# reuk/wayverb

Measured on AMD Instinct MI355X. Metric: Gnode-updates/s, fp64 box mesh, higher is better.
Workload: dtype f64

## Files before the change

include/wayverb_amd.h:

```cpp
#ifndef WAYVERB_AMD_H
#define WAYVERB_AMD_H

#include <stddef.h>
#include <stdint.h>

#ifdef __cplusplus
extern "C" {
#endif

enum {
    WV_OK = 0,
    WV_E_INVALID_ARGUMENT = -1,
    WV_E_INVALID_MESH = -2,
    WV_E_HIP = -3,
    WV_E_NO_DEVICE = -4,
    WV_E_COMM = -5,
    WV_E_STATE = -6
};


enum {
    WV_ID_NONE = 0,
    WV_ID_INSIDE = 1 << 0,
    WV_ID_NX = 1 << 1,
    WV_ID_PX = 1 << 2,
    WV_ID_NY = 1 << 3,
    WV_ID_PY = 1 << 4,
    WV_ID_NZ = 1 << 5,
    WV_ID_PZ = 1 << 6,
    WV_ID_REENTRANT = 1 << 7
};

enum {
    WV_FLAG_SUCCESS = 0,
    WV_FLAG_INF = 1 << 0,
    WV_FLAG_NAN = 1 << 1,
    WV_FLAG_OUTSIDE_RANGE = 1 << 2,
    WV_FLAG_OUTSIDE_MESH = 1 << 3,
    WV_FLAG_SUSPICIOUS_BOUNDARY = 1 << 4
};

typedef struct wv_condensed_node {
    int32_t boundary_type;
    uint32_t boundary_index;
} wv_condensed_node;

typedef struct wv_coefficients_canonical {
    double b[7];
    double a[7];
} wv_coefficients_canonical;

typedef struct wv_boundary_data {
    double filter_memory[6];
    uint32_t coefficient_index;
    uint32_t reserved_;
} wv_boundary_data;

typedef struct wv_mesh {
    int32_t nx, ny, nz;
    const wv_condensed_node* nodes;
    const wv_coefficients_canonical* coefficients;
    uint32_t num_coefficients;
    const uint32_t* boundary_indices_1;
    const uint32_t* boundary_indices_2;
    const uint32_t* boundary_indices_3;
    uint64_t num_boundary_1, num_boundary_2, num_boundary_3;
} wv_mesh;

enum { WV_PRECISION_F32 = 0,
       WV_PRECISION_F64 = 1   };

typedef struct wv_tuning {
    int32_t pair;
    int32_t pair_chunks;
    int32_t pair_inner_fix;
    int32_t pair_wide;
    int32_t pair_unit_waves;
    int32_t pair_unit_planes;
    int32_t pair_units_by_chunk;
    int32_t tile_lists;
    int32_t fuse_pre_post;
    int32_t graph;
    int32_t boundary_lds;
    int32_t boundary_order;
    int32_t boundary_xwall;
    int32_t stream_ry, stream_nwx, stream_nwy, stream_zchunks;
    int32_t slab_early;
    int32_t pair_split_rows;
    int32_t fuse_planes;
    int32_t whole_step;
    int32_t triple;
    int32_t triple_chunks;
    int32_t triple_lanes;
} wv_tuning;

typedef struct wv_options {
    int32_t struct_size;
    int32_t precision;
    int32_t device;
    int32_t ghost_lo, ghost_hi;
    int32_t flag_interval;
    int32_t stream_variant;
    int32_t all_tiles;
    int32_t nodes_on_device;
    int32_t comm_timeout_s;
    int32_t transport;
    int32_t reserved_[5];
    wv_tuning tuning;
} wv_options;

enum { WV_TRANSPORT_RCCL = 0, WV_TRANSPORT_IPC = 1 };

typedef struct wv_engine wv_engine;


int wv_create(const wv_mesh* mesh, const wv_options* options, wv_engine** out);
void wv_destroy(wv_engine* e);
const char* wv_last_error(void);
void wv_default_options(wv_options* options);

enum { WV_BUF_CURRENT = 0, WV_BUF_PREVIOUS = 1 };

int wv_read_value(wv_engine* e, int buffer, uint64_t index, double* value);
int wv_write_value(wv_engine* e, int buffer, uint64_t index, double value);
int wv_read_field(wv_engine* e, int buffer, void* dst, int elem_size);
int wv_write_field(wv_engine* e, int buffer, const void* src, int elem_size);
int wv_read_planes(wv_engine* e, int buffer, int32_t z_begin, int32_t z_count, void* dst, int elem_size);
int wv_write_planes(wv_engine* e, int buffer, int32_t z_begin, int32_t z_count, const void* src, int elem_size);
int wv_read_boundary_data(wv_engine* e, int dimensionality, wv_boundary_data* dst);
int wv_write_boundary_data(wv_engine* e, int dimensionality, const wv_boundary_data* src);
int wv_set_coefficients(wv_engine* e, const wv_coefficients_canonical* c, uint32_t n);
int wv_host_register(void* p, uint64_t bytes);
int wv_host_unregister(void* p);
int wv_device_buffer(wv_engine* e, int buffer, void** device_ptr);

int wv_checkpoint(wv_engine* e);
int wv_rollback(wv_engine* e);
int wv_drop_checkpoint(wv_engine* e);


int wv_step(wv_engine* e, int32_t* flag);
int wv_swap(wv_engine* e);

enum { WV_SOURCE_NONE = 0,
       WV_SOURCE_HARD = 1,
       WV_SOURCE_SOFT = 2   };

int wv_set_source(wv_engine* e, int kind, uint64_t node, const double* signal, uint64_t n);
int wv_set_receivers(wv_engine* e, const uint64_t* nodes, uint32_t n);
int wv_run(wv_engine* e, uint64_t n_steps, uint64_t* steps_done, int32_t* flag);
int wv_fetch_receivers(wv_engine* e, uint64_t first, uint64_t n, double* dst);
int wv_step_count(wv_engine* e, uint64_t* steps);

int wv_kernel_time_ms(wv_engine* e, double* mean_ms, uint64_t* launches);
int wv_enable_kernel_timing(wv_engine* e, int enable);
int wv_kernel_time_detail(wv_engine* e, double* mean_ms, uint64_t* launches, uint64_t* steps);
enum { WV_QUERY_PASSES = 0, WV_QUERY_XWALL_ENTRIES = 1, WV_QUERY_FIELDS = 2, WV_QUERY_MARCH_LIVE_PERMILLE = 3,
       WV_QUERY_SWEEP_LIVE_PERMILLE = 4, WV_QUERY_MARCH_ROUNDS = 5, WV_QUERY_HALO_WAIT_NS = 6, WV_QUERY_HALO_WAITS = 7,
       WV_QUERY_HALO_EXCHANGES = 8, WV_QUERY_HALO_BYTES_SENT = 9, WV_QUERY_EARLY_PASSES = 10,
       WV_QUERY_BOUNDARY1_NS = 11, WV_QUERY_BOUNDARY2_NS = 12, WV_QUERY_BOUNDARY_TIMED = 13,
       WV_QUERY_WHOLE_STEPS = 14 ,
       WV_QUERY_TRIPLE_PASSES = 15,
       WV_QUERY_TRIPLE_MARCH_NS = 16, WV_QUERY_TRIPLE_MARCH_TIMED = 17, WV_QUERY_BOUNDARY3_NS = 18, WV_QUERY_FIXUP3_NS = 19,
       WV_QUERY_TRIPLE_PARTS_TIMED = 20 };
int wv_query(wv_engine* e, int what, uint64_t* value);
int wv_synchronize(wv_engine* e);
int wv_set_stream_tuning(wv_engine* e, int variant, int rows_per_wave, int waves_x, int waves_y, int knob);

#define WV_UNIQUE_ID_BYTES 128
int wv_comm_use_library(const char* path);
int wv_comm_unique_id(void* id_bytes );
int wv_comm_init(wv_engine* e, const void* id_bytes, int rank, int nranks);
int wv_comm_destroy(wv_engine* e);
int wv_comm_init_local(wv_engine* const* engines, int32_t n);
int wv_run_group(wv_engine* const* engines, int32_t n, uint64_t n_steps, uint64_t* steps_done, int32_t* flag);

int wv_measure_triad(int32_t device, uint64_t n_doubles, int32_t iters, double* gb_per_s);

int wv_compressed_waveguide_run(int32_t device, uint64_t steps, int32_t source_kind, const float* input,
                                uint64_t n_input, float* output );
int wv_make_transparent(const float* input, uint64_t n, const float* response, uint32_t taps,
                        float* out );

int wv_filter_test_2(const float* input, float* output, double* memory,
                     const wv_coefficients_canonical* coeffs, uint32_t n_filters, uint32_t n_samples);
int wv_field_pitch(wv_engine* e, uint64_t* pitch_elements);

int wv_make_box_nodes(int32_t nx, int32_t ny, int32_t nz_global, int32_t z_begin, int32_t z_count,
                      int32_t number_from, int32_t number_to, wv_condensed_node* nodes,
                      uint64_t counts[3]);

int wv_classify_nodes(int32_t nx, int32_t ny, int32_t nz, const uint8_t* inside, wv_condensed_node* nodes,
                      uint64_t counts[3]);

int wv_voxelise(const float* vertices, uint32_t n_vertices, const uint32_t* triangles, uint32_t n_triangles,
                const float aabb_min[3], const float aabb_max[3], uint32_t side, uint32_t* out, uint64_t capacity,
                uint64_t* needed);
int wv_nodes_inside(int32_t nx, int32_t ny, int32_t nz, const float min_corner[3], float spacing,
                    const uint32_t* voxel_index, uint64_t n_voxel_words, const float aabb_min[3],
                    const float aabb_max[3], uint32_t side, const uint32_t* triangles, uint32_t n_triangles,
                    const float* vertices, uint32_t n_vertices, uint8_t* inside);

int wv_boundary_index_data(int32_t nx, int32_t ny, int32_t nz, const float min_corner[3], float spacing,
                           wv_condensed_node* nodes, const uint32_t* triangles, uint32_t n_triangles,
                           const float* vertices, uint32_t n_vertices, uint32_t* b1, uint64_t capacity_1,
                           uint32_t* b2, uint64_t capacity_2, uint32_t* b3, uint64_t capacity_3,
                           uint64_t counts[3]);

typedef struct wv_scene_mesh wv_scene_mesh;
int wv_scene_mesh_create(int32_t nx, int32_t ny, int32_t nz, const float min_corner[3], float spacing,
                         const uint32_t* voxel_index, uint64_t n_voxel_words, const float aabb_min[3],
                         const float aabb_max[3], uint32_t side, const uint32_t* triangles, uint32_t n_triangles,
                         const float* vertices, uint32_t n_vertices, int32_t device, wv_scene_mesh** out,
                         uint64_t counts[3]);
int wv_scene_mesh_fetch(const wv_scene_mesh* sm, wv_condensed_node* nodes, uint32_t* b1, uint32_t* b2, uint32_t* b3);
int wv_scene_mesh_create_engine(const wv_scene_mesh* sm, const wv_coefficients_canonical* coefficients,
                                uint32_t num_coefficients, const wv_options* options, wv_engine** out);
void wv_scene_mesh_destroy(wv_scene_mesh* sm);

int wv_arbitrary_magnitude_filter(const double* frequency, const double* amplitude, uint32_t n_points,
                                  double b[7], double a[7]);
int wv_is_stable(const double* a, uint32_t n, int32_t* stable);
int wv_band_centres(double sample_rate, double centres[8]);
int wv_reflectance_filter(const double absorption[8], double sample_rate, wv_coefficients_canonical* out);
int wv_impedance_coefficients(const wv_coefficients_canonical* reflectance, wv_coefficients_canonical* impedance);

typedef struct wv_directional_output {
    float intensity[3];
    float pressure;
} wv_directional_output;
typedef struct wv_waveguide_band {
    const wv_directional_output* directional;
    uint64_t n;
    double sample_rate;
    double valid_hz_min, valid_hz_max;
} wv_waveguide_band;
enum { WV_ATTENUATOR_NULL = 0,
       WV_ATTENUATOR_MICROPHONE = 1
        };
enum { WV_FILTER_LOPASS = 0, WV_FILTER_HIPASS = 1, WV_FILTER_BANDPASS = 2 };

int wv_attenuate(int32_t method, const float pointing[3], float shape, float acoustic_impedance,
                 const wv_directional_output* in, uint64_t n, float* out);
int wv_adjust_sampling_rate(const float* in, uint64_t n, double in_sample_rate, double out_sample_rate, float* out,
                            uint64_t capacity, uint64_t* n_out);
int wv_frequency_domain_filter(float* signal, uint64_t n, int32_t kind, double edge_lo, double edge_hi,
                               double width_factor, uint32_t steepness);
int wv_postprocess_waveguide(const wv_waveguide_band* bands, uint32_t n_bands, int32_t method, const float pointing[3],
                             float shape, float acoustic_impedance, double output_sample_rate, float* out,
                             uint64_t capacity, uint64_t* n_out);

typedef struct wv_hrtf_table {
    const double* energy;
    uint32_t az_num, el_num;
} wv_hrtf_table;
int wv_hrtf_attenuation(const wv_hrtf_table* table, const float pointing[3], const float up[3], int32_t channel,
                        const float incident[3], float bands[8]);
int wv_hrtf_ear_position(const float pointing[3], const float up[3], int32_t channel, float radius,
                         const float base_position[3], float ear[3]);
int wv_attenuate_hrtf(const wv_hrtf_table* table, const float pointing[3], const float up[3], int32_t channel,
                      float acoustic_impedance, const wv_directional_output* in, uint64_t n, float* out);
int wv_multiband_filter_and_mixdown(float* bands, uint64_t n, double sample_rate, float* out);
int wv_postprocess_waveguide_hrtf(const wv_waveguide_band* bands, uint32_t n_bands, const wv_hrtf_table* table,
                                  const float pointing[3], const float up[3], int32_t channel, float acoustic_impedance,
                                  double output_sample_rate, float* out, uint64_t capacity, uint64_t* n_out);

#ifdef __cplusplus
}
#endif
#endif
```

wayverb_amd/csrc/boundary_kernels.hip.h:

```cpp
#pragma once
#include "device_common.hip.h"

namespace wv {

__device__ __forceinline__ void filter_step_6(double in, double m[6], const double* __restrict__ cb,
                                              const double* __restrict__ ca) {
    const double out = (in * cb[0] + m[0]) / ca[0];
#pragma unroll
    for (int i = 0; i < 5; ++i) {
        const double b = cb[i + 1] == 0 ? 0 : cb[i + 1] * in;
        const double a = ca[i + 1] == 0 ? 0 : ca[i + 1] * out;
        m[i] = b - a + m[i + 1];
    }
    const double b = cb[6] == 0 ? 0 : cb[6] * in;
    const double a = ca[6] == 0 ? 0 : ca[6] * out;
    m[5] = b - a;
}

__global__ void __launch_bounds__(64) filter_test_2_kernel(const float* input, float* output, double* memory,
                                                           const double* coeffs, uint32_t n_filters,
                                                           uint32_t n_samples) {
    const uint32_t f = blockIdx.x * blockDim.x + threadIdx.x;
    if (f >= n_filters) return;
    double m[6], cb[7], ca[7];
// ... 287 lines not shown
    if (LEVEL == 2) {
        g2c = a.next[gn];
        h2c = a.next[gn + (h_off ? 0 : step)];
    }
    Real nb[3][2];
    bool off[3][2];
    off[0][0] = x - 1 < 0;
    off[0][1] = x + 1 >= a.nx;
    nb[0][0] = nb[0][1] = f_nb[pos_e];
    bool any_field = false;
#pragma unroll
    for (int k = 0; k < 4; ++k) {
        const int ax = 1 + (k >> 1), s = k & 1;
        const int c = pos[ax] + (s ? 1 : -1);
        off[ax][s] = c < 0 || c >= lim[ax];
        const bool mirrored = ref[k] != XW_FIELD;
        nb[ax][s] = own_nb[mirrored ? (ref[k] & ~XW_SAME_FACING) : pos_e];
        any_field = any_field || !mirrored;
    }
    const Real prev = own_prev[pos_e];
    double m[1][6];
    const double* cf[1];
    cf[0] = coeffs + (size_t)a.cidx[pos_e] * 14;
#pragma unroll
    for (int j = 0; j < 6; ++j) m[0][j] = __builtin_nontemporal_load(a.fmem + (size_t)j * a.n_slots + pos_e);
    Real f1 = 0, far1 = 0;
    Real fnb[3][2], fprev = 0;
    bool any_lateral_field = false;
    if (LEVEL == 1) {
        f1 = a.next[fn];
        far1 = a.next[fn + (far_off ? 0 : step)];
        far1 = far_off ? Real(0) : far1;
    } else {
        const Real own_at = own_nb[pos_e];
        Real far = LEVEL == 2 ? a.xw_g[pos_e] : *(gok ? a.xw_g2 + pos_e : a.cur + gn);
        far = (LEVEL == 3 && far_off) ? Real(0) : far;
        fnb[0][0] = step > 0 ? own_at : far;
        fnb[0][1] = step > 0 ? far : own_at;
#pragma unroll
        for (int k = 0; k < 4; ++k) {
            const int ax = 1 + (k >> 1), s = k & 1;
            const bool regular = ref[k] != XW_FIELD && (ref[k] & XW_SAME_FACING);
            const Real v = f_nb[regular ? (ref[k] & ~XW_SAME_FACING) : pos_e];
            fnb[ax][s] = off[ax][s] ? Real(0) : v;
            any_lateral_field = any_lateral_field || (!regular && !off[ax][s]);
        }
        fprev = LEVEL == 2 ? a.xw_f[pos_e] : a.xw_f1[pos_e];
    }
    Real gnb[3][2], gprev = 0;
    uint32_t g_from_field = 0;
    if (LEVEL == 3) {
        const Real f2 = nb[0][0], h2 = a.xw_h2[pos_e];
        gnb[0][0] = step > 0 ? f2 : h2;
        gnb[0][1] = step > 0 ? h2 : f2;
#pragma unroll
        for (int k = 0; k < 4; ++k) {
            const int ax = 1 + (k >> 1), s = k & 1;
            const bool regular = ref[k] != XW_FIELD && (ref[k] & XW_SAME_FACING);
            const uint32_t other = regular ? (ref[k] & ~XW_SAME_FACING) : pos_e;
            const bool copy = regular && a.xw_gok[other] != 0;
            const Real v = a.xw_g2[other];
            gnb[ax][s] = off[ax][s] ? Real(0) : v;
            if (!copy && !off[ax][s]) g_from_field |= 1u << k;
        }
        gprev = a.xw_g[pos_e];
        if (gok && g_from_field) {
#pragma unroll
            for (int k = 0; k < 4; ++k) {
                const int ax = 1 + (k >> 1), s = k & 1;
                if ((g_from_field >> k) & 1u) gnb[ax][s] = a.cur[gn + (s ? stride[ax] : -stride[ax])];
            }
        }
    }
    if (any_field) {
#pragma unroll
        for (int k = 0; k < 4; ++k) {
            const int ax = 1 + (k >> 1), s = k & 1;
            if (ref[k] == XW_FIELD) nb[ax][s] = a.cur[(int64_t)idx + (off[ax][s] ? 0 : (s ? stride[ax] : -stride[ax]))];
        }
    }
    if (LEVEL != 1 && any_lateral_field) {
#pragma unroll
        for (int k = 0; k < 4; ++k) {
            const int ax = 1 + (k >> 1), s = k & 1;
            const bool regular = ref[k] != XW_FIELD && (ref[k] & XW_SAME_FACING);
            if (!regular && !off[ax][s]) fnb[ax][s] = a.cur[fn + (s ? stride[ax] : -stride[ax])];
        }
    }

    const Real next = boundary_value<Real, 1>(a.courant, a.courant_sq, dirs, nb, off, prev, m, cf);
#pragma unroll
    for (int j = 0; j < 6; ++j) __builtin_nontemporal_store(m[0][j], a.fmem + (size_t)j * a.n_slots + pos_e);
    bad |= bad_bits(next);
    a.next[idx] = next;
    own_out[pos_e] = next;
    if (LEVEL == 1) {
        a.xw_f1[pos_e] = f1;
        a.xw_g[pos_e] = far1;
    } else {
        const Real sf = faced_value<Real>(fnb, fprev);
        bad |= bad_bits(sf);
        a.next[fn] = sf;
        (LEVEL == 2 ? a.xw_f2 : a.xw_f)[pos_e] = sf;
        if (LEVEL == 2) {
            a.xw_g2[pos_e] = g2c;
            a.xw_h2[pos_e] = h_off ? Real(0) : h2c;
        } else {
            const Real sg = faced_value<Real>(gnb, gprev);
            if (gok) {
                bad |= bad_bits(sg);
                a.next[gn] = sg;
            }
        }
    }
}

template <typename Real, bool FIX>
__device__ __forceinline__ void boundary_entry(const BoundaryArgs<Real>& a, const double* coeffs, uint32_t e, int& bad) {
    if (e < a.n1) {
        boundary_node<Real, 1, FIX>(a, coeffs, e, e, 0u, a.n1, bad);
    } else if (e < a.n1 + a.n2) {
        boundary_node<Real, 2, FIX>(a, coeffs, e - a.n1, e, a.n1, a.n2, bad);
    } else if (e < a.n1 + a.n2 + a.n3) {
        boundary_node<Real, 3, FIX>(a, coeffs, e - a.n1 - a.n2, e, a.n1 + 2u * a.n2, a.n3, bad);
    }
}

constexpr uint32_t kMaxLdsCoefficientSets = 256;

template <typename Real>
__device__ __forceinline__ void pre_post_body(const PrePostArgs<Real>& a, uint32_t t, uint32_t width);

template <typename Real, bool LDSC, bool FIX, int XW3 = 0>
__device__ __forceinline__ void boundary_body(const BoundaryArgs<Real>& a, const PrePostArgs<Real>& next, uint32_t block, uint32_t blocks) {
    __shared__ double s_coeffs[LDSC ? kMaxLdsCoefficientSets * 14 : 1];
    if (LDSC) {
        for (uint32_t w = threadIdx.x; w < a.n_coeffs * 14u; w += 256) s_coeffs[w] = a.coeffs[w];
        __syncthreads();
    }
    const double* coeffs = LDSC ? s_coeffs : a.coeffs;
    const uint32_t t = block * blockDim.x + threadIdx.x;
    int bad = 0;
    if (a.xw_n) {
        if (t < a.xw_pad) {
            if (t < a.xw_n) {
                if (XW3)
                    xwall3_node<Real, XW3 ? XW3 : 1>(a, coeffs, t, bad);
                else
                    xwall_node<Real, FIX ? 2 : 1>(a, coeffs, t, bad);
            }
        } else if (a.order) {
            if (t - a.xw_pad < a.n_order) boundary_entry<Real, FIX>(a, coeffs, a.order[t - a.xw_pad], bad);
        } else {
            boundary_entry<Real, FIX>(a, coeffs, a.xw_n + (t - a.xw_pad), bad);
        }
    } else if (a.order) {
        if (t < a.n_order) boundary_entry<Real, FIX>(a, coeffs, a.order[t], bad);
    } else {
        boundary_entry<Real, FIX>(a, coeffs, t, bad);
    }
    if (bad) atomicOr(a.flag, bad);
    if (next.fused && block == blocks - 1) pre_post_body<Real>(next, threadIdx.x, 256);
}

template <typename Real, bool LDSC, bool FIX = false, int XW3 = 0>
__global__ void __launch_bounds__(256) boundary_kernel(const BoundaryArgs<Real> a, const PrePostArgs<Real> next) {
    if (next.fused) {
        if (blockIdx.x == 0) {
            pre_post_body<Real>(next, threadIdx.x, 256);
            return;
        }
        PrePostArgs<Real> none{};
        boundary_body<Real, LDSC, FIX, XW3>(a, none, blockIdx.x - 1, gridDim.x - 1);
        return;
    }
    boundary_body<Real, LDSC, FIX, XW3>(a, next, blockIdx.x, gridDim.x);
}

struct XwCoverArgs {
    const uint32_t* bnode;
    const uint8_t* btype;
    uint32_t* covered;
    uint32_t xw_n;
    const uint8_t* pair_map;
    uint8_t* gok;
    int nx, ny, nz, pitch, cls_pitch;
};
__global__ void __launch_bounds__(256) xwall_cover_kernel(const XwCoverArgs a) {
    const uint32_t p = blockIdx.x * blockDim.x + threadIdx.x;
    if (p >= a.xw_n) return;
    const uint32_t idx = a.bnode[p];
    const int step = (a.btype[p] & 2u) ? 1 : -1;
    const uint32_t fn = idx + (uint32_t)step;
    atomicOr(a.covered + (fn >> 5), 1u << (fn & 31u));
    const int x = (int)(idx % (uint32_t)a.pitch);
    const uint32_t q = idx / (uint32_t)a.pitch;
    const int y = (int)(q % (uint32_t)a.ny), z = (int)(q / (uint32_t)a.ny);
    auto code_at = [&](int xx) -> uint32_t { return (a.pair_map[cls_byte_index(xx, y, z, a.ny, a.cls_pitch)] >> ((xx & 3) * 2)) & 3u; };
    const int xg = x + 2 * step, xh = x + 3 * step;
    bool ok = xg >= 0 && xg < a.nx && code_at(xg) == 1u;
    if (ok && xh >= 0 && xh < a.nx) ok = code_at(xh) != 2u && code_at(xh) != 3u;
    a.gok[p] = ok ? 1 : 0;
    if (ok) {
        const uint32_t gn = idx + (uint32_t)(2 * step);
        atomicOr(a.covered + (gn >> 5), 1u << (gn & 31u));
    }
}

struct XwEligibleArgs {
    const uint32_t* bnode;
    const uint8_t* btype;
    const uint8_t* cls;
    uint8_t* eligible;
    uint32_t n1;
    int nx, ny, nz, pitch, cls_pitch;
    int march_begin, march_end;
};

__global__ void __launch_bounds__(256) xwall_eligible_kernel(const XwEligibleArgs a) {
    const uint32_t e = blockIdx.x * blockDim.x + threadIdx.x;
    if (e >= a.n1) return;
    const uint32_t idx = a.bnode[e];
    const uint32_t dirs = a.btype[e] & 0x3Fu;
    bool ok = idx != INVALID_NODE && (dirs == 1u || dirs == 2u);
    if (ok) {
        const int x = (int)(idx % (uint32_t)a.pitch);
        const uint32_t q = idx / (uint32_t)a.pitch;
        const int y = (int)(q % (uint32_t)a.ny), z = (int)(q / (uint32_t)a.ny);
        const int step = dirs == 2u ? 1 : -1;
        auto cls_at = [&](int xx) -> uint32_t {
            return (a.cls[cls_byte_index(xx, y, z, a.ny, a.cls_pitch)] >> ((xx & 3) * 2)) & 3u;
        };
        ok = z >= a.march_begin && z < a.march_end && x + step >= 0 && x + step < a.nx && cls_at(x + step) == CLS_INSIDE;
        if (ok && x + 2 * step >= 0 && x + 2 * step < a.nx) ok = cls_at(x + 2 * step) != CLS_BOUNDARY;
    }
    a.eligible[e] = ok ? 1 : 0;
}

template <typename Real>
__global__ void __launch_bounds__(256) xwall_gather_kernel(const BoundaryArgs<Real> a) {
    const uint32_t p = blockIdx.x * blockDim.x + threadIdx.x;
    if (p >= a.xw_n) return;
    const uint32_t idx = a.bnode[p];
    const int64_t fn = (int64_t)idx + ((a.btype[p] & 2u) ? 1 : -1);
    a.xw_a[p] = a.prev[idx];
    a.xw_b[p] = a.cur[idx];
    a.xw_f[p] = a.cur[fn];
}

template <typename Real>
__device__ __forceinline__ void pre_post_body(const PrePostArgs<Real>& a, uint32_t t, uint32_t width) {
    if (t == 0 && a.flag) *a.flag = a.flag_init;
    if (t == 0 && a.flag2) *a.flag2 = a.flag_init;
    Real injected = 0;
    const bool has_source = a.source_kind != 0;
    if (has_source) {
        const Real s = (Real)a.signal[a.signal_pos + (a.signal_base ? *a.signal_base : 0ull)];
        injected = (a.source_kind == 1) ? s : (Real)(a.cur[a.source_node] + s);
    }
    for (uint32_t r = t; r < a.n_recv; r += width) {
        const uint64_t node = a.recv[r];
        Real v = 0;
        if (node != ~0ull) v = (has_source && node == a.source_node) ? injected : a.cur[node];
        a.recv_out[r] = v;
    }
    __syncthreads();
    if (t == 0 && has_source) a.cur[a.source_node] = injected;
    if (a.fix_n) {
        __threadfence();
        __syncthreads();
        const int64_t plane = (int64_t)a.pitch * a.ny;
        int bad = 0;
        for (uint32_t i = t; i < a.fix_n; i += width) {
            const uint32_t idx = a.fix_nodes[i];
            const int x = (int)(idx % (uint32_t)a.pitch);
            const uint32_t q = idx / (uint32_t)a.pitch;
            const int y = (int)(q % (uint32_t)a.ny);
            const int z = (int)(q / (uint32_t)a.ny);
            auto t1 = [&](int64_t at) { return __hip_atomic_load(a.cur + at, __ATOMIC_RELAXED, __HIP_MEMORY_SCOPE_AGENT); };
            Real s = 0;
            s += (x > 0) ? t1((int64_t)idx - 1) : Real(0);
            s += (x + 1 < a.nx) ? t1((int64_t)idx + 1) : Real(0);
            s += (y > 0) ? t1((int64_t)idx - a.pitch) : Real(0);
            s += (y + 1 < a.ny) ? t1((int64_t)idx + a.pitch) : Real(0);
            s += (z > 0) ? t1((int64_t)idx - plane) : Real(0);
            s += (z + 1 < a.nz) ? t1((int64_t)idx + plane) : Real(0);
            s = div3(s);
            s -= a.fix_cur[idx];
            bad |= bad_bits(s);
            a.fix_out2[idx] = s;
        }
        if (bad) atomicOr(a.fix_flag, bad);
    }
}

template <typename Real>
__global__ void __launch_bounds__(64) pre_post_kernel(const PrePostArgs<Real> a) {
    pre_post_body<Real>(a, threadIdx.x, 64);
}

struct NodeRec {
    int32_t boundary_type;
    uint32_t boundary_index;
};

struct SetupArgs {
    const NodeRec* nodes;
    int64_t first_row, rows;
    int nx, ny;
    int pitch;
    int cls_pitch;
    uint8_t* cls;
    uint32_t* bnode;
    uint8_t* btype;
    uint32_t n1, n2, n3;
    int* status;
    int z_begin, z_end;
};

__device__ __forceinline__ uint32_t classify(int32_t t, int* dim_out) {
    *dim_out = 0;
    if (t == 0) return CLS_NONE;
    const int bits = __popc((uint32_t)t);
    if (bits == 1 && (t & 1)) return CLS_INSIDE;
    if (bits == 1 && (t & 128)) return CLS_REENTRANT;
    *dim_out = bits;
    return CLS_BOUNDARY;
}

__global__ void __launch_bounds__(256) setup_classify_kernel(const SetupArgs a) {
    const int64_t n_bytes = a.rows * a.cls_pitch;
    for (int64_t i = (int64_t)blockIdx.x * blockDim.x + threadIdx.x; i < n_bytes;
         i += (int64_t)gridDim.x * blockDim.x) {
        const int64_t row = i / a.cls_pitch;
        const int xb = (int)(i % a.cls_pitch);
        const int64_t grow = a.first_row + row;
        const int z = (int)(grow / a.ny);
        uint32_t byte = 0;
        for (int j = 0; j < 4; ++j) {
            const int x = xb * 4 + j;
            if (x >= a.nx) break;
            const NodeRec rec = a.nodes[row * a.nx + x];
            const int32_t t = rec.boundary_type;
            int dim;
            const uint32_t c = classify(t, &dim);
            byte |= c << (2 * j);
            if (c == CLS_BOUNDARY) {
                const uint32_t dirs = ((uint32_t)t >> 1) & 0x3Fu;
                const bool only_dirs = ((uint32_t)t & ~0x7Eu) == 0;
                const bool axes_ok = ((dirs & 3u) != 3u) && (((dirs >> 2) & 3u) != 3u) && (((dirs >> 4) & 3u) != 3u);
                if (!only_dirs || !axes_ok || dim < 1 || dim > 3) {
                    atomicOr(a.status, 1);
                    continue;
                }
                if (z < a.z_begin || z >= a.z_end) continue;
                const uint32_t n_d = dim == 1 ? a.n1 : (dim == 2 ? a.n2 : a.n3);
                const uint32_t off = dim == 1 ? 0u : (dim == 2 ? a.n1 : a.n1 + a.n2);
                const uint32_t k = rec.boundary_index;
                if (k >= n_d) {
                    atomicOr(a.status, 2);
                    continue;
                }
                a.bnode[off + k] = (uint32_t)(grow * a.pitch + x);
                a.btype[off + k] = (uint8_t)dirs;
            }
        }
        a.cls[cls_byte_index(xb * 4, (int)(grow % a.ny), z, a.ny, a.cls_pitch)] = (uint8_t)byte;
    }
}

struct ValidateArgs {
    const uint32_t* bnode;
    const uint8_t* btype;
    const uint8_t* cls;
    uint32_t n_entries;
    int nx, ny, nz, pitch, cls_pitch;
    int* static_flag;
};

__global__ void __launch_bounds__(256) setup_validate_kernel(const ValidateArgs a) {
    const uint32_t e = blockIdx.x * blockDim.x + threadIdx.x;
    if (e >= a.n_entries) return;
    const uint32_t idx = a.bnode[e];
    if (idx == INVALID_NODE) return;
    const uint32_t dirs = a.btype[e] & 0x3Fu;
    const int pos[3] = {(int)(idx % (uint32_t)a.pitch), (int)((idx / (uint32_t)a.pitch) % (uint32_t)a.ny),
                        (int)(idx / ((uint32_t)a.pitch * (uint32_t)a.ny))};
    const int lim[3] = {a.nx, a.ny, a.nz};
    int flag = 0;
    int dim = __popc(dirs);
    for (int ax = 0; ax < 3; ++ax) {
        const bool has_n = (dirs >> (2 * ax)) & 1u, has_p = (dirs >> (2 * ax + 1)) & 1u;
        if (has_n || has_p) {
            const int c = pos[ax] + (has_p ? 1 : -1);
            if (c < 0 || c >= lim[ax]) flag |= FLAG_OUTSIDE_MESH;
        } else if (dim < 3) {
            for (int s = -1; s <= 1; s += 2) {
                int p[3] = {pos[0], pos[1], pos[2]};
                p[ax] += s;
                if (p[ax] < 0 || p[ax] >= lim[ax]) {
// ... 73 lines not shown
```

wayverb_amd/csrc/device_common.hip.h:

```cpp
#pragma once
#include <hip/hip_runtime.h>
#include <stdint.h>

namespace wv {

enum : uint32_t { CLS_NONE = 0, CLS_INSIDE = 1, CLS_BOUNDARY = 2, CLS_REENTRANT = 3 };

enum : int { FLAG_INF = 1, FLAG_NAN = 2, FLAG_OUTSIDE_RANGE = 4, FLAG_OUTSIDE_MESH = 8,
             FLAG_SUSPICIOUS = 16 };

constexpr uint32_t INVALID_NODE = 0xFFFFFFFFu;

__host__ __device__ inline int64_t cls_word_index(int x, int y, int z, int ny, int cls_pitch) {
    return ((int64_t)z * ((ny + 3) >> 2) + (y >> 2)) * cls_pitch + (x >> 2);
}
__host__ __device__ inline int64_t cls_byte_index(int x, int y, int z, int ny, int cls_pitch) {
    return cls_word_index(x, y, z, ny, cls_pitch) * 4 + (y & 3);
}

template <typename Real>
struct Vec16;
template <>
struct Vec16<double> {
    typedef double type __attribute__((ext_vector_type(2)));
    static constexpr int N = 2;
};
template <>
struct Vec16<float> {
    typedef float type __attribute__((ext_vector_type(4)));
    static constexpr int N = 4;
};

__device__ __forceinline__ float lane_from_below(float edge, float v) {
    return __int_as_float(__builtin_amdgcn_update_dpp(__float_as_int(edge), __float_as_int(v),
                                                      0x138 , 0xf, 0xf, false));
}
__device__ __forceinline__ float lane_from_above(float edge, float v) {
    return __int_as_float(__builtin_amdgcn_update_dpp(__float_as_int(edge), __float_as_int(v),
                                                      0x130 , 0xf, 0xf, false));
}
__device__ __forceinline__ double lane_from_below(double edge, double v) {
    const int lo = __builtin_amdgcn_update_dpp(__double2loint(edge), __double2loint(v), 0x138, 0xf, 0xf, false);
    const int hi = __builtin_amdgcn_update_dpp(__double2hiint(edge), __double2hiint(v), 0x138, 0xf, 0xf, false);
    return __hiloint2double(hi, lo);
}
__device__ __forceinline__ double lane_from_above(double edge, double v) {
    const int lo = __builtin_amdgcn_update_dpp(__double2loint(edge), __double2loint(v), 0x130, 0xf, 0xf, false);
    const int hi = __builtin_amdgcn_update_dpp(__double2hiint(edge), __double2hiint(v), 0x130, 0xf, 0xf, false);
    return __hiloint2double(hi, lo);
}

__device__ __forceinline__ float read_lane(float v, int src) {
    return __int_as_float(__builtin_amdgcn_readlane(__float_as_int(v), src));
}
__device__ __forceinline__ double read_lane(double v, int src) {
    const int lo = __builtin_amdgcn_readlane(__double2loint(v), src);
    const int hi = __builtin_amdgcn_readlane(__double2hiint(v), src);
    return __hiloint2double(hi, lo);
}

__device__ __forceinline__ double div3(double x) {
    constexpr double c = 0x1.5555555555555p-2;
    const double q0 = x * c;
    const double r = __builtin_fma(-3.0, q0, x);
    return __builtin_amdgcn_div_fixup(__builtin_fma(r, c, q0), 3.0, x);
}
__device__ __forceinline__ float div3(float x) {
    constexpr float c = 0x1.555556p-2f;
    const float q0 = x * c;
    const float r = __builtin_fmaf(-3.0f, q0, x);
    return __builtin_amdgcn_div_fixupf(__builtin_fmaf(r, c, q0), 3.0f, x);
}

__device__ __forceinline__ bool is_finite(float v) { return __builtin_amdgcn_classf(v, 0x1F8); }
__device__ __forceinline__ bool is_finite(double v) { return __builtin_amdgcn_class(v, 0x1F8); }

template <typename Real>
__device__ __forceinline__ int bad_bits(Real v) {
    return (isinf(v) ? FLAG_INF : 0) | (isnan(v) ? FLAG_NAN : 0);
}

template <typename Real>
struct BoundaryArgs {
    const Real* prev;
    Real* next;
    const Real* cur;
    int* flag;
    const uint32_t* bnode;
    const uint8_t* btype;
    double* fmem;
    const uint32_t* cidx;
    const double* coeffs;
    uint32_t n_coeffs;
    uint32_t n1, n2, n3;
    uint32_t n_slots;
    int nx, ny, nz;
    int pitch;
    int z_begin, z_end;
    Real courant, courant_sq;
    const uint32_t* order;
    uint32_t n_order;
    int fix_z0, fix_z1;
    uint32_t xw_n, xw_pad;
    const uint32_t* xw_nbr;
    Real *xw_a, *xw_b, *xw_f, *xw_f1, *xw_g;
    Real *xw_o2, *xw_f2;
    Real *xw_g2, *xw_h2;
    const uint8_t* xw_gok;
};

template <typename Real>
struct StreamArgs {
    const Real* prev;
    Real* next;
    const Real* cur;
    const uint8_t* cls;
    int* flag;
    int nx, ny, nz;
    int pitch;
    int cls_pitch;
    int z_begin, z_end;
    int z_skip_from, z_skip;
    int zc;
    int tiles_x, tiles_y, chunks_z;
    int total_tiles, tiles_per_xcd;
    int stripe_rows, tiles_y_stripe, passes;
    const uint64_t* tile_list;
    uint32_t list_start[9];
};

template <typename Real>
struct PrePostArgs {
    Real* cur;
    const double* signal;
    uint64_t signal_pos;
    const uint64_t* signal_base;
    uint64_t source_node;
    int source_kind;
    const uint64_t* recv;
    Real* recv_out;
    uint32_t n_recv;
    int* flag;
    int* flag2;
    int flag_init;
    int fused;
    const uint32_t* fix_nodes;
    uint32_t fix_n;
    const Real* fix_cur;
    Real* fix_out2;
    int* fix_flag;
    int nx, ny, nz, pitch;
};

struct StepDuty {
    uint64_t node;
    uint32_t block;
    uint32_t col;
    uint32_t kind;
    uint32_t pad_;
};
template <typename Real>
struct StepDuties {
    const StepDuty* list;
    uint32_t n;
    const double* signal;
    uint64_t signal_pos;
    const uint64_t* signal_base;
    Real* recv_out;
    const uint64_t* recv;
    uint32_t n_recv;
    int* next_flag;
    int flag_init;
};

}
```

wayverb_amd/csrc/engine.hip:

```cpp
#include "engine.hip.h"
#include "engine_setup.hip.h"
#include "engine_single.hip.h"
#include "engine_pair.hip.h"
#include "engine_triple.hip.h"
#include "engine_batch.hip.h"
#include "engine_io.hip.h"
#include "engine_slab.hip.h"

namespace {
thread_local std::string g_last_error;
thread_local hipError_t g_last_hip_error = hipSuccess;
}

namespace wv {
int fail_with(int code, const std::string& msg) {
    g_last_error = msg;
    return code;
}
void note_hip_error(hipError_t err) { g_last_hip_error = err; }
hipError_t last_hip_error() { return g_last_hip_error; }
}

using wv::DeviceGuard;
using wv::Engine;
using wv::fail;
using wv::ScopedDevice;

extern "C" {

const char* wv_last_error(void) { return g_last_error.c_str(); }

void wv_default_options(wv_options* o) {
    std::memset(o, 0, sizeof(*o));
    o->struct_size = (int32_t)sizeof(wv_options);
    o->precision = WV_PRECISION_F64;
    o->device = -1;
    o->flag_interval = 0;
    o->stream_variant = 2;
    wv_tuning& t = o->tuning;
    t.pair = -1;
    t.pair_chunks = 0;
    t.pair_inner_fix = 1;
    t.pair_wide = 1;
    t.pair_unit_waves = 1;
    t.pair_unit_planes = 32;
    t.pair_units_by_chunk = 1;
    t.tile_lists = 1;
    t.fuse_pre_post = 1;
    t.graph = 0;
    t.boundary_lds = 1;
    t.boundary_order = 1;
    t.boundary_xwall = 1;
    t.slab_early = -1;
    t.pair_split_rows = 0;
    t.fuse_planes = 1;
    t.whole_step = -1;
    t.triple = -1;
    t.triple_chunks = 0;
    t.triple_lanes = 0;
}

#ifdef WV_DEBUG_ENV
static void tuning_from_environment(wv_options* o) {
    struct Knob {
        const char* name;
        int32_t* field;
    };
    wv_tuning& t = o->tuning;
    const Knob knobs[] = {{"WV_PAIR", &t.pair}, {"WV_PAIR_CHUNKS", &t.pair_chunks}, {"WV_PAIR_INNER_FIX", &t.pair_inner_fix},
                          {"WV_PAIR_WIDE", &t.pair_wide}, {"WV_PAIR_UNIT_WAVES", &t.pair_unit_waves},
                          {"WV_PAIR_UNIT_PLANES", &t.pair_unit_planes}, {"WV_PAIR_UNITS_BY_CHUNK", &t.pair_units_by_chunk}, {"WV_TILE_LISTS", &t.tile_lists},
                          {"WV_FUSE_PRE_POST", &t.fuse_pre_post}, {"WV_GRAPH", &t.graph}, {"WV_BOUNDARY_LDS", &t.boundary_lds},
                          {"WV_BOUNDARY_ORDER", &t.boundary_order}, {"WV_BOUNDARY_XWALL", &t.boundary_xwall},
                          {"WV_SLAB_EARLY", &t.slab_early}, {"WV_PAIR_SPLIT_ROWS", &t.pair_split_rows}, {"WV_FUSE_PLANES", &t.fuse_planes}, {"WV_WHOLE_STEP", &t.whole_step}, {"WV_TRIPLE", &t.triple}, {"WV_TRIPLE_CHUNKS", &t.triple_chunks}, {"WV_TRIPLE_LANES", &t.triple_lanes},
                          {"WV_STREAM_VARIANT", &o->stream_variant},
                          {"WV_STREAM_RY", &t.stream_ry}, {"WV_STREAM_NWX", &t.stream_nwx}, {"WV_STREAM_NWY", &t.stream_nwy},
                          {"WV_STREAM_ZCHUNKS", &t.stream_zchunks}};
    for (const Knob& k : knobs)
        if (const char* v = std::getenv(k.name)) *k.field = std::atoi(v);
}
#endif

int wv_create(const wv_mesh* mesh, const wv_options* options, wv_engine** out) {
    if (!mesh || !out) return fail(WV_E_INVALID_ARGUMENT, "null argument");
    *out = nullptr;
    wv_options opt;
    wv_default_options(&opt);
    if (options) {
        const size_t n = std::min<size_t>(sizeof(opt), options->struct_size > 0 ? (size_t)options->struct_size : sizeof(opt));
        std::memcpy(&opt, options, n);
        opt.struct_size = (int32_t)sizeof(opt);
    }
#ifdef WV_DEBUG_ENV
    tuning_from_environment(&opt);
#endif
    std::unique_ptr<wv_engine> e;
    if (opt.precision == WV_PRECISION_F32) {
        e.reset(new Engine<float>());
    } else if (opt.precision == WV_PRECISION_F64) {
        e.reset(new Engine<double>());
    } else {
        return fail(WV_E_INVALID_ARGUMENT, "unknown precision");
    }
    const int rc = e->init(*mesh, opt);
    if (rc != WV_OK) return rc;
    *out = e.release();
    return WV_OK;
}

void wv_destroy(wv_engine* e) { delete e; }

#define WV_NEED(e) \
    if (!(e)) return fail(WV_E_INVALID_ARGUMENT, "null engine")

int wv_read_value(wv_engine* e, int buffer, uint64_t index, double* value) {
    WV_NEED(e);
    return e->read_value(buffer, index, value);
}
int wv_write_value(wv_engine* e, int buffer, uint64_t index, double value) {
    WV_NEED(e);
    return e->write_value(buffer, index, value);
}
int wv_read_field(wv_engine* e, int buffer, void* dst, int elem_size) {
    WV_NEED(e);
    return e->read_field(buffer, dst, elem_size);
}
int wv_write_field(wv_engine* e, int buffer, const void* src, int elem_size) {
    WV_NEED(e);
    return e->write_field(buffer, src, elem_size);
}
int wv_read_planes(wv_engine* e, int buffer, int32_t z_begin, int32_t z_count, void* dst, int elem_size) {
    WV_NEED(e);
    return e->read_planes(buffer, z_begin, z_count, dst, elem_size);
}
int wv_write_planes(wv_engine* e, int buffer, int32_t z_begin, int32_t z_count, const void* src, int elem_size) {
    WV_NEED(e);
    return e->write_planes(buffer, z_begin, z_count, src, elem_size);
}
int wv_read_boundary_data(wv_engine* e, int dim, wv_boundary_data* dst) {
    WV_NEED(e);
    return e->boundary_data(dim, dst, false);
}
int wv_write_boundary_data(wv_engine* e, int dim, const wv_boundary_data* src) {
    WV_NEED(e);
    return e->boundary_data(dim, const_cast<wv_boundary_data*>(src), true);
}
int wv_set_coefficients(wv_engine* e, const wv_coefficients_canonical* c, uint32_t n) {
    WV_NEED(e);
    return e->set_coefficients(c, n);
}
int wv_device_buffer(wv_engine* e, int buffer, void** p) {
    WV_NEED(e);
    return e->device_buffer(buffer, p);
}
int wv_host_register(void* p, uint64_t bytes) {
    if (!p || !bytes) return fail(WV_E_INVALID_ARGUMENT, "null argument");
    int count = 0;
    if (hipGetDeviceCount(&count) != hipSuccess || count == 0)
        return fail(WV_E_NO_DEVICE, "no HIP device visible; this engine has no CPU fallback");
    WV_HIP(hipHostRegister(p, (size_t)bytes, hipHostRegisterDefault));
    return WV_OK;
}
int wv_host_unregister(void* p) {
    if (!p) return fail(WV_E_INVALID_ARGUMENT, "null argument");
    WV_HIP(hipHostUnregister(p));
    return WV_OK;
}
int wv_checkpoint(wv_engine* e) {
    WV_NEED(e);
    return e->checkpoint(0);
}
int wv_rollback(wv_engine* e) {
    WV_NEED(e);
    return e->checkpoint(1);
}
int wv_drop_checkpoint(wv_engine* e) {
    WV_NEED(e);
    return e->checkpoint(2);
}
int wv_step(wv_engine* e, int32_t* flag) {
    WV_NEED(e);
    return e->step(flag);
}
int wv_swap(wv_engine* e) {
    WV_NEED(e);
    return e->swap();
}
int wv_set_source(wv_engine* e, int kind, uint64_t node, const double* signal, uint64_t n) {
    WV_NEED(e);
    return e->set_source(kind, node, signal, n);
}
int wv_set_receivers(wv_engine* e, const uint64_t* nodes, uint32_t n) {
    WV_NEED(e);
    return e->set_receivers(nodes, n);
}
int wv_run(wv_engine* e, uint64_t n_steps, uint64_t* done, int32_t* flag) {
    WV_NEED(e);
    return e->run(n_steps, done, flag);
}
int wv_fetch_receivers(wv_engine* e, uint64_t first, uint64_t n, double* dst) {
    WV_NEED(e);
    return e->fetch_receivers(first, n, dst);
}
int wv_step_count(wv_engine* e, uint64_t* steps) {
    WV_NEED(e);
    *steps = e->steps_done;
    return WV_OK;
}
int wv_kernel_time_ms(wv_engine* e, double* mean_ms, uint64_t* launches) {
    WV_NEED(e);
    return e->kernel_time(mean_ms, launches, nullptr);
}
int wv_kernel_time_detail(wv_engine* e, double* mean_ms, uint64_t* launches, uint64_t* steps) {
    WV_NEED(e);
    return e->kernel_time(mean_ms, launches, steps);
}
int wv_enable_kernel_timing(wv_engine* e, int enable) {
    WV_NEED(e);
    e->timing = enable != 0;
    return WV_OK;
}
int wv_query(wv_engine* e, int what, uint64_t* value) {
    WV_NEED(e);
    return e->query(what, value);
}
int wv_synchronize(wv_engine* e) {
    WV_NEED(e);
// ... 117 lines not shown
```

wayverb_amd/csrc/engine.hip.h:

```cpp
#pragma once
#include "engine_base.h"

#include "boundary_kernels.hip.h"
#include "pair_kernels.hip.h"
#include "stream_kernels.hip.h"
#include "plane_kernels.hip.h"
#include "triple_kernels.hip.h"

namespace wv {

template <typename Real>
class Engine final : public wv_engine {
public:
    ~Engine() override { release(); }
    int init(const wv_mesh& m, const wv_options& opt) override;
    int set_tuning(int variant, int ry, int nwx, int nwy, int zchunks) override;
    int build_plane_order();
    void plan_stream();
    template <int RY, int NWX, int NWY>
    void launch_shape(const wv::StreamArgs<Real>& a, unsigned grid);
    template <int RY>
    void launch_ry(const wv::StreamArgs<Real>& a, unsigned grid);
    int build_tile_lists(int z0, int z1);
    struct StreamLaunch {
        wv::StreamArgs<Real> args;
        unsigned grid = 0;
    };
    int launch_stream(Real* prev, const Real* cur, int* flag, int z0, int z1, bool timed, Real* out = nullptr, int zb0 = 0, int zb1 = 0,
                      StreamLaunch* plan_only = nullptr);
    int launch_faces(Real* prev, const Real* cur, int* flag, Real* out, int planes = 1);
    wv::BoundaryArgs<Real> boundary_args(Real* prev, const Real* cur, int* flag) const;
    struct BoundaryLaunch {
        wv::BoundaryArgs<Real> args;
        unsigned blocks = 0;
        bool lds = false;
    };
    int launch_boundary(Real* prev, const Real* cur, int* flag, int z0, int z1, const wv::PrePostArgs<Real>* next = nullptr, Real* out = nullptr, bool fix_inner = false,
                        bool levels = false, BoundaryLaunch* plan_only = nullptr, int xw3 = 0);
    wv::PrePostArgs<Real> pre_post_args(Real* cur, int slot, bool with_pre_post, uint64_t signal_pos, bool source_live) const;
    int enqueue_step(int slot, bool with_pre_post, uint64_t signal_pos, bool source_live, int fuse_next = 0);
    bool whole_step_ready();
    bool whole_step_sized() const;
    int launch_whole_step(Real* prev, const Real* cur, int slot, uint64_t signal_pos, bool source_live, bool serve_next);
    bool pair_eligible();
    int ensure_pair();
    int build_pair_units(int owned);
    static void parallel_sort(std::vector<uint64_t>& v);
    int enqueue_pair_a(int slot, uint64_t signal_pos, bool source_live, bool fuse_mid);
    int launch_fixup(uint32_t first, uint32_t n, const Real* t1, const Real* cur, Real* out2, int* flag2);
    int build_xwall();
    void xwall_args(wv::BoundaryArgs<Real>& b) const;
    int enqueue_pair_b(int slot, uint64_t signal_pos, bool source_live, int fuse_next);
    bool slab_early_now() const;
    int begin_halo_wait_timing();
    int end_halo_wait_timing(int token);
    int begin_part_timing(int part, bool always = false);
    int end_part_timing(int part, int token);
    int enqueue_batch_pair(uint64_t i, int part, int next_kind) override;
    int batch_pair_eligible(int* eligible) override;
    int batch_pair_prepare(int* ready, int* singles_first) override;
    int batch_pair_vetoed() override;
    int batch_triple_prepare(int* ready) override;
    int enqueue_batch_triple(uint64_t i, int part) override;
    uint64_t role_signature() const override {
        return (uint64_t)cur_ | (uint64_t)prv_ << 2 | (uint64_t)spare_[0] << 4 | (uint64_t)spare_[1] << 6 | steps_done << 8;
    }
    static constexpr int kWideLaneBytes = 16;
    int triple_lane_bytes() const;
    bool triple_eligible();
    int ensure_triple();
    int build_triple_units();
    int enqueue_triple(int slot, uint64_t signal_pos, bool source_live, int fuse_next);
    int enqueue_triple_slab(int slot, int part, uint64_t signal_pos, bool source_live);
    int launch_triple_march(int slot, const Real* A, const Real* B, Real* O1, Real* O2, Real* O3);
    int launch_triple_list(int slot, const Real* A, const Real* B, const Real* O1, const Real* O2, Real* O3, bool source_live);
    bool time_this_launch();
    int drain_timing();
    int step(int32_t* flag) override;
    int swap() override;
    int replay_batch(uint64_t batch, bool source_live, bool can_fuse);
    uint64_t plan_batch(uint64_t remaining) override;
    int enqueue_batch_step(uint64_t i, uint64_t batch, int next_kind) override;
    int collect_batch(uint64_t batch) override;
    const int* batch_flags() const override { return flags_host_; }
    int commit_batch(uint64_t batch, const int* flags, uint64_t* good_out, int32_t* flag_out) override;
    int run(uint64_t n_steps, uint64_t* done, int32_t* flag_out) override;
    int set_source(int kind, uint64_t node, const double* signal, uint64_t n) override;
    int set_receivers(const uint64_t* nodes, uint32_t n) override;
    bool io_nodes_plain();
    bool io_nodes(std::vector<uint64_t>* stored);
    bool io_nodes_unfaced();
    bool io_nodes_clear_of_x_walls();
    int fetch_receivers(uint64_t first, uint64_t n, double* dst) override;
    Real* buffer(int which) { return which == WV_BUF_CURRENT ? field_[cur_] : field_[prv_]; }
    hipError_t class_of(uint64_t x, uint64_t row, uint32_t* cls);
    uint64_t stored_index(uint64_t node) const;
    int read_value(int buffer_id, uint64_t index, double* v) override;
    int write_value(int buffer_id, uint64_t index, double v) override;
    template <typename Other>
    int copy_field(Real* stored, void* host, bool to_device, int z0, int planes);
    int read_field(int buffer_id, void* dst, int elem_size) override { return read_planes(buffer_id, 0, nz_, dst, elem_size); }
    int write_field(int buffer_id, const void* src, int elem_size) override {
        return write_planes(buffer_id, 0, nz_, src, elem_size);
    }
    int read_planes(int buffer_id, int z0, int planes, void* dst, int elem_size) override;
    int write_planes(int buffer_id, int z0, int planes, const void* src, int elem_size) override;
    int boundary_data(int dim, wv_boundary_data* host, bool to_device) override;
    int set_coefficients(const wv_coefficients_canonical* c, uint32_t n) override;
    int device_buffer(int buffer_id, void** p) override;
    int checkpoint(int op) override;
    int kernel_time(double* mean_ms, uint64_t* launches, uint64_t* steps) override;
    int synchronize() override;
    int query(int what, uint64_t* value) override;
    int comm_init(const void* id, int rank, int nranks) override;
    int comm_init_local(int rank, int nranks) override;
    int adopt_comm(std::unique_ptr<wv::SlabComm> c);
    wv::SlabComm* comm() override { return comm_.get(); }
    uint64_t field_pitch() const override { return (uint64_t)pitch_; }
    int comm_destroy() override;

private:
    void release();
    bool use_work_lists() const { return !opt_.all_tiles && opt_.tuning.tile_lists != 0; }

    wv_options opt_{};
    int nx_ = 0, ny_ = 0, nz_ = 0, z_begin_ = 0, z_end_ = 0, device_ = -1;
    uint64_t n_nodes_ = 0, stored_nodes_ = 0, field_bytes_ = 0;
    int pitch_ = 0;
    Real* field_[4] = {nullptr, nullptr, nullptr, nullptr};
    int cur_ = 1, prv_ = 0, spare_[2] = {2, 3};
    uint8_t* cls_ = nullptr;
    int cls_pitch_ = 0;
    uint32_t n1_ = 0, n2_ = 0, n3_ = 0, n_entries_ = 0, n_slots_ = 0, n_coeffs_ = 0;
    uint32_t* bnode_ = nullptr;
    uint64_t* tile_list_ = nullptr;
    uint32_t list_start_[9] = {0, 0, 0, 0, 0, 0, 0, 0, 0};
    uint32_t list_longest_ = 0;
    bool lists_built_ = false;
    int lists_z0_ = 0, lists_z1_ = 0;
    struct GraphKey {
        uint64_t batch;
        int cur;
        bool source_live, can_fuse;
        uint32_t n_recv;
        uint64_t source_node;
        int source_kind;
        uint64_t signal_ptr, recv_ptr;
        bool lists;
        uint64_t cur_ptr, prv_ptr;
        uint64_t io_generation;
        bool operator==(const GraphKey& o) const {
            return batch == o.batch && cur == o.cur && source_live == o.source_live && can_fuse == o.can_fuse &&
                   n_recv == o.n_recv && source_node == o.source_node && source_kind == o.source_kind &&
                   signal_ptr == o.signal_ptr && recv_ptr == o.recv_ptr && lists == o.lists && cur_ptr == o.cur_ptr &&
                   prv_ptr == o.prv_ptr && io_generation == o.io_generation;
        }
    };
    hipGraphExec_t graph_exec_ = nullptr;
    GraphKey graph_key_{};
    uint64_t* signal_base_dev_ = nullptr;
    bool graph_capturing_ = false;
    uint64_t graph_max_nodes_ = 64ull << 20;
    bool batch_flags_reset_ = false;
    bool pre_post_done_ = false;
    int pair_inner_ok_ = -1;
    uint64_t pair_min_nodes_ = 4ull << 20;
    bool pair_failed_ = false;
    uint8_t* pair_map_ = nullptr;
    uint32_t* pair_list_ = nullptr;
    uint32_t* pair_counter_ = nullptr;
    uint32_t* pair_units_ = nullptr;
    uint32_t pair_unit_start_[9] = {0, 0, 0, 0, 0, 0, 0, 0, 0};
    uint32_t pair_units_longest_ = 0;
    bool pair_sparse_ok_ = true;
    double tile_active_frac_ = 1.0;
    double pair_live_frac_ = 1.0;
    uint32_t pair_list_n_ = 0;
    int pair_z0_ = 0, pair_z1_ = 0;
    uint64_t pair_source_ = 0;
    int pair_nw_ = 1, pair_strips_ = 0, pair_zc_ = 0, pair_chunks_ = 1;
    uint64_t timed_steps_ = 0;
    bool batch_can_fuse_ = false, batch_source_live_ = false;
    bool io_plain_known_ = false, io_plain_ = false;
    bool io_unfaced_known_ = false, io_unfaced_ = false;
    bool io_xclear_known_ = false, io_xclear_ = false;
    bool duties_known_ = false, duties_ok_ = false;
    wv::StepDuty* duties_ = nullptr;
    uint32_t n_duties_ = 0;
    uint64_t whole_steps_ = 0;
    uint64_t graph_whole_steps_ = 0;
    uint64_t io_generation_ = 0;
    bool pair_list_early_ok_ = false;
    bool pair_unit_waves_ = false;
    int pair_windows_ = 0;
    uint8_t pair_win_[4][wv::kPairMaxWindows] = {};
    bool pair_mid_done_ = false, pair_list_done_ = false;
    int outside_dirty_ = 0;
    uint32_t* ref_to_pos_ = nullptr;
    uint8_t* btype_ = nullptr;
    double* fmem_ = nullptr;
    uint32_t* cidx_ = nullptr;
    uint32_t* zorder_ = nullptr;
    uint32_t* zorder_rest_ = nullptr;
    uint32_t* face_order_ = nullptr;
    uint32_t face_n_ = 0;
    uint32_t* early_order_ = nullptr;
    uint32_t early_n_ = 0;
    int pair_s0_ = 0, pair_s1_ = 0;
    bool pair_early_ = false;
    std::vector<hipEvent_t> halo_events_;
    int halo_ev_used_ = 0;
    unsigned halo_timing_calls_ = 0;
    double halo_wait_ms_ = 0;
    uint64_t halo_wait_n_ = 0, early_passes_ = 0;
    static constexpr int kParts = 5;
    std::vector<hipEvent_t> part_events_[kParts];
    int part_ev_used_[kParts] = {0, 0, 0, 0, 0};
    double part_ms_[kParts] = {0, 0, 0, 0, 0};
    uint64_t part_n_[kParts] = {0, 0, 0, 0, 0};
    bool pass_timed_ = false;
    unsigned part_timing_calls_ = 0;
    std::vector<uint32_t> plane_start_, plane_start_rest_;
    uint32_t n_xw_ = 0;
    uint32_t* xw_nbr_ = nullptr;
    Real* xw_val_ = nullptr;
    uint8_t* xw_gok_ = nullptr;
    bool xw_built_ = false;
    bool xw_active_ = false;
    bool xw_valid_ = false;
    uint64_t passes_taken_ = 0;
    Real* field1_ = nullptr;
    uint8_t* triple_map_ = nullptr;
    uint32_t* triple_list_ = nullptr;
    uint32_t triple_list_n_ = 0;
    int* suspect_ = nullptr;
    uint64_t triple_source_ = 0, triple_io_generation_ = ~0ull;
    bool triple_failed_ = false, triple_ready_ = false, triple_attr_set_ = false;
    uint32_t* triple_units_ = nullptr;
    uint32_t triple_unit_start_[9] = {0, 0, 0, 0, 0, 0, 0, 0, 0};
    uint32_t triple_units_longest_ = 0;
    double triple_live_frac_ = 1.0;
    bool triple_xw_ = false;
    uint64_t triple_min_nodes_ = sizeof(Real) == 8 ? (12ull << 20) : (24ull << 20);
    int triple_z0_ = 0, triple_z1_ = 0;
    int triple_nw_ = 1, triple_strips_ = 0, triple_zc_ = 0, triple_chunks_ = 1, triple_windows_ = 0;
    uint8_t triple_win_[4][wv::kTripleMaxWindows] = {};
    int triple_lb_ = 8;
    int triple_wide_from_ = 320;
    uint64_t triples_taken_ = 0;
    int* status_ = nullptr;
    int* static_flag_dev_ = nullptr;
    int static_flag_ = 0;
    double* coeffs_ = nullptr;
    int* flags_ = nullptr;
    int* flags_host_ = nullptr;
    void* scratch_ = nullptr;
    Real courant_ = 0, courant_sq_ = 0;
    hipStream_t stream_ = nullptr, comm_stream_ = nullptr;
    hipStream_t on_ = nullptr;
    hipStream_t st() const { return on_ ? on_ : stream_; }
    StreamPlan plan_;
    int tune_variant_ = -1, tune_ry_ = 0, tune_nwx_ = 0, tune_nwy_ = 0, tune_zchunks_ = 0;
    std::vector<hipEvent_t> events_;
    unsigned timing_launches_ = 0;
    int ev_used_ = 0;
    double time_ms_ = 0;
    uint64_t time_n_ = 0;
    int source_kind_ = WV_SOURCE_NONE;
    uint64_t source_node_ = 0, signal_len_ = 0, signal_pos_ = 0;
    double* signal_ = nullptr;
    uint64_t* recv_nodes_ = nullptr;
    Real* recv_out_ = nullptr;
    uint32_t n_recv_ = 0;
    uint64_t recv_first_step_ = 0;
    Real* recv_stage_ = nullptr;
    std::vector<double> recv_log_;
    std::unique_ptr<wv::SlabComm> comm_;
    struct Checkpoint {
        Real* field[2] = {nullptr, nullptr};
        double* fmem = nullptr;
        bool valid = false;
        uint64_t steps_done = 0, signal_pos = 0, recv_first_step = 0;
        size_t recv_log_size = 0;
        uint32_t n_recv = 0;
        int outside_dirty = 0;
    } ckpt_;
};

}
```

wayverb_amd/csrc/engine_batch.hip.h:

```cpp
#pragma once
#include "engine.hip.h"

namespace wv {

template <typename Real>
bool Engine<Real>::time_this_launch() {
    if (!timing || ev_used_ + 2 > (int)events_.size()) return false;
    const unsigned stride = stored_nodes_ < (128ull << 20) ? 8u : 1u;
    return (timing_launches_++ % stride) == 0;
}

template <typename Real>
int Engine<Real>::drain_timing() {
    for (int i = 0; i + 1 < ev_used_; i += 2) {
        float ms = 0;
        WV_HIP(hipEventElapsedTime(&ms, events_[i], events_[i + 1]));
        time_ms_ += ms;
        ++time_n_;
    }
    ev_used_ = 0;
    for (int i = 0; i + 1 < halo_ev_used_; i += 2) {
        float ms = 0;
        WV_HIP(hipEventElapsedTime(&ms, halo_events_[i], halo_events_[i + 1]));
        halo_wait_ms_ += ms;
        ++halo_wait_n_;
    }
    halo_ev_used_ = 0;
    for (int p = 0; p < kParts; ++p) {
        for (int i = 0; i + 1 < part_ev_used_[p]; i += 2) {
            float ms = 0;
            WV_HIP(hipEventElapsedTime(&ms, part_events_[p][i], part_events_[p][i + 1]));
            part_ms_[p] += ms;
            ++part_n_[p];
        }
        part_ev_used_[p] = 0;
    }
    return WV_OK;
}

template <typename Real>
int Engine<Real>::begin_part_timing(int part, bool always) {
    if (!timing || !(pass_timed_ || always)) return -1;
    auto& ev = part_events_[part];
    if (ev.empty()) {
        ev.resize(2 * 512);
        for (auto& e : ev)
            if (hipEventCreate(&e) != hipSuccess) {
                (void)hipGetLastError();
                e = nullptr;
            }
    }
    const int at = part_ev_used_[part];
    if (at + 2 > (int)ev.size() || !ev[at] || !ev[at + 1]) return -1;
    if (hipEventRecord(ev[at], stream_) != hipSuccess) {
        (void)hipGetLastError();
        return -1;
    }
    return at;
}

template <typename Real>
int Engine<Real>::end_part_timing(int part, int token) {
    if (token < 0) return WV_OK;
    WV_HIP(hipEventRecord(part_events_[part][token + 1], stream_));
    part_ev_used_[part] = token + 2;
    return WV_OK;
}

template <typename Real>
int Engine<Real>::begin_halo_wait_timing() {
    if (!timing || !comm_ || (halo_timing_calls_++ & 3u) != 0) return -1;
    if (halo_events_.empty()) {
        halo_events_.resize(2 * 160);
        for (auto& e : halo_events_)
            if (hipEventCreate(&e) != hipSuccess) {
                (void)hipGetLastError();
                e = nullptr;
            }
    }
    if (halo_ev_used_ + 2 > (int)halo_events_.size() || !halo_events_[halo_ev_used_] || !halo_events_[halo_ev_used_ + 1]) return -1;
    if (hipEventRecord(halo_events_[halo_ev_used_], stream_) != hipSuccess) {
        (void)hipGetLastError();
        return -1;
    }
    return halo_ev_used_;
}

template <typename Real>
int Engine<Real>::end_halo_wait_timing(int token) {
    if (token < 0) return WV_OK;
    WV_HIP(hipEventRecord(halo_events_[token + 1], stream_));
    halo_ev_used_ = token + 2;
    return WV_OK;
}

template <typename Real>
int Engine<Real>::step(int32_t* flag) {
    DeviceGuard guard(device_);
    pre_post_done_ = false;
    batch_flags_reset_ = false;
    int rc = enqueue_step(0, false, 0, false);
    if (rc) return rc;
    WV_HIP(hipMemcpyAsync(flags_host_, flags_, sizeof(int), hipMemcpyDeviceToHost, stream_));
    WV_HIP(hipStreamSynchronize(stream_));
    if ((rc = drain_timing())) return rc;
    if (flag) *flag = flags_host_[0];
    return WV_OK;
}

template <typename Real>
int Engine<Real>::swap() {
    std::swap(cur_, prv_);
    xw_valid_ = false;
    ++steps_done;
    if (n_recv_) recv_log_.insert(recv_log_.end(), n_recv_, std::numeric_limits<double>::quiet_NaN());
    return WV_OK;
}

template <typename Real>
uint64_t Engine<Real>::plan_batch(uint64_t remaining) {
    DeviceGuard guard(device_);
    const uint64_t interval = opt_.flag_interval > 0 ? (uint64_t)opt_.flag_interval : (uint64_t)kRing;
    uint64_t batch = std::min<uint64_t>(std::min<uint64_t>(interval, kRing), remaining);
    if (source_kind_ != WV_SOURCE_NONE) {
        const uint64_t left = signal_len_ - std::min(signal_len_, signal_pos_);
        batch = std::min(batch, left);
    }
    batch_can_fuse_ = !comm_ && io_nodes_plain() && opt_.tuning.fuse_pre_post != 0;
    (void)whole_step_ready();
    batch_source_live_ = source_kind_ != WV_SOURCE_NONE;
    pre_post_done_ = pair_mid_done_ = pair_list_done_ = false;
    batch_flags_reset_ = false;
    if (comm_ && batch) {
        static_assert(sizeof(int) == 4, "flag words are 32 bit");
        if (hipMemsetD32Async((hipDeviceptr_t)flags_, static_flag_, (size_t)batch, stream_) == hipSuccess)
            batch_flags_reset_ = true;
        else
            (void)hipGetLastError();
    }
    return batch;
}

template <typename Real>
int Engine<Real>::enqueue_batch_step(uint64_t i, uint64_t batch, int next_kind) {
    DeviceGuard guard(device_);
    const int rc = enqueue_step((int)i, true, signal_pos_ + i, batch_source_live_,
                                batch_can_fuse_ && i + 1 < batch ? next_kind : 0);
    if (rc) return rc;
    std::swap(cur_, prv_);
    return WV_OK;
}

template <typename Real>
int Engine<Real>::collect_batch(uint64_t batch) {
    DeviceGuard guard(device_);
    std::string cerr;
    if (comm_ && !comm_->join_halo(stream_, &cerr)) return fail(WV_E_COMM, cerr);
    if (comm_ && !comm_->or_flags(stream_, flags_, (int)batch, &cerr)) return fail(WV_E_COMM, cerr);
    WV_HIP(hipMemcpyAsync(flags_host_, flags_, batch * sizeof(int), hipMemcpyDeviceToHost, stream_));
    if (n_recv_) {
        WV_HIP(hipMemcpyAsync(recv_stage_, recv_out_, (size_t)batch * n_recv_ * sizeof(Real), hipMemcpyDeviceToHost, stream_));
    }
    if (comm_ && !comm_->is_local()) {
        if (!comm_->sync(stream_, "the batch of steps " + std::to_string(steps_done) + " .. " + std::to_string(steps_done + batch - 1), &cerr))
            return fail(WV_E_COMM, cerr);
    } else {
        WV_HIP(hipStreamSynchronize(stream_));
    }
    if (comm_ && comm_->is_local()) WV_HIP(hipStreamSynchronize(comm_stream_));
    return drain_timing();
}

template <typename Real>
int Engine<Real>::commit_batch(uint64_t batch, const int* flags, uint64_t* good_out, int32_t* flag_out) {
    uint64_t good = batch;
    int32_t flag = 0;
    for (uint64_t i = 0; i < batch; ++i) {
        if (flags[i]) {
            good = i;
            flag = flags[i];
            break;
        }
    }
    if (n_recv_)
        for (size_t i = 0; i < (size_t)good * n_recv_; ++i) recv_log_.push_back((double)recv_stage_[i]);
    steps_done += good;
    signal_pos_ += good;
    if (flag && good < batch && ((batch - good) & 1)) std::swap(cur_, prv_);
    if (flag) xw_valid_ = false;
    *good_out = good;
    *flag_out = flag;
    return WV_OK;
}

template <typename Real>
int Engine<Real>::run(uint64_t n_steps, uint64_t* done, int32_t* flag_out) {
    DeviceGuard guard(device_);
    if (comm_ && comm_->is_local() && comm_->nranks() > 1)
        return fail(WV_E_STATE, "slabs joined by wv_comm_init_local are stepped together: use wv_run_group");
    uint64_t completed = 0;
    int32_t flag = 0;
    const bool chain = comm_ && !comm_->is_local();
    std::string cerr;
    while (completed < n_steps && flag == 0) {
        uint64_t batch = plan_batch(n_steps - completed);
        int eligible = 0, rc = batch_pair_eligible(&eligible);
        if (rc) return rc;
        if (chain) {
            uint64_t words[2] = {batch, (uint64_t)eligible};
            if (!comm_->agree_min(stream_, words, 2, &cerr)) return fail(WV_E_COMM, cerr);
            batch = words[0];
            eligible = (int)words[1];
        }
        if (batch == 0) break;
        const bool use_graph = opt_.tuning.graph != 0 && !comm_ && !timing && (batch % 2) == 0 && batch >= 16 &&
                               stored_nodes_ <= graph_max_nodes_ && outside_dirty_ == 0;
        if (use_graph) {
            if ((rc = replay_batch(batch, batch_source_live_, batch_can_fuse_))) return rc;
        } else {
            int singles_first = -1;
            if (eligible) {
                int ready = 0, mine = 0;
                const int prepared = batch_pair_prepare(&ready, &mine);
                if (prepared && !chain) return prepared;
                if (chain) {
                    uint64_t words[3] = {(uint64_t)(prepared ? 0 : ready), (uint64_t)(prepared ? 2 : 2 - mine), prepared ? 0ull : 1ull};
                    if (!comm_->agree_min(stream_, words, 3, &cerr)) return fail(WV_E_COMM, cerr);
                    if (prepared) return prepared;
                    if (words[2] == 0)
                        return fail(WV_E_COMM, "another rank of the chain failed while preparing two-step passes (its wv_last_error says why)");
                    ready = (int)words[0];
                    mine = 2 - (int)words[1];
                }
                if (ready) singles_first = mine;
            }
            if (singles_first < 0 && (rc = batch_pair_vetoed())) return rc;
            const bool pairs = singles_first >= 0;
            bool triples = false;
            if (pairs && batch >= (uint64_t)singles_first + 3) {
                int mine = 0;
                const int prepared = batch_triple_prepare(&mine);
                if (prepared && !chain) return prepared;
                if (chain) {
                    uint64_t words[2] = {(uint64_t)(prepared ? 0 : mine), prepared ? 0ull : 1ull};
                    if (!comm_->agree_min(stream_, words, 2, &cerr)) return fail(WV_E_COMM, cerr);
                    if (prepared) return prepared;
                    if (words[1] == 0)
                        return fail(WV_E_COMM, "another rank of the chain failed while preparing three-step passes (its wv_last_error says why)");
                    mine = (int)words[0];
                }
                triples = mine != 0;
                if (triples && !batch_flags_reset_) {
                    WV_HIP(hipMemsetD32Async((hipDeviceptr_t)flags_, static_flag_, (size_t)batch, stream_));
                    batch_flags_reset_ = true;
                }
            }
            auto triple_at = [&](uint64_t i) { return triples && i >= (uint64_t)singles_first && i + 3 <= batch; };
            auto pair_at = [&](uint64_t i) { return pairs && !triple_at(i) && i >= (uint64_t)singles_first && i + 2 <= batch; };
            auto kind_at = [&](uint64_t i) { return i >= batch ? 0 : (pair_at(i) ? 2 : 1); };
            for (uint64_t i = 0; i < batch;) {
                if (triple_at(i)) {
                    if (comm_) {
                        for (int part = 0; part < 3; ++part)
                            if ((rc = enqueue_batch_triple(i, part))) return rc;
                    } else if ((rc = enqueue_triple((int)i, signal_pos_ + i, batch_source_live_, kind_at(i + 3)))) {
                        return rc;
                    }
                    i += 3;
                } else if (pair_at(i)) {
                    if ((rc = enqueue_batch_pair(i, 0, 0))) return rc;
                    if ((rc = enqueue_batch_pair(i, 1, kind_at(i + 2)))) return rc;
                    i += 2;
                } else {
                    if ((rc = enqueue_batch_step(i, batch, kind_at(i + 1)))) return rc;
                    i += 1;
                }
            }
        }
        if ((rc = collect_batch(batch))) return rc;
        uint64_t good = 0;
        if ((rc = commit_batch(batch, flags_host_, &good, &flag))) return rc;
        completed += good;
    }
    if (done) *done = completed;
    if (flag_out) *flag_out = flag;
    return WV_OK;
}

template <typename Real>
int Engine<Real>::kernel_time(double* mean_ms, uint64_t* launches, uint64_t* steps) {
    DeviceGuard guard(device_);
    if (mean_ms) *mean_ms = time_n_ ? time_ms_ / (double)time_n_ : 0.0;
    if (launches) *launches = time_n_;
    if (steps) *steps = timed_steps_;
    time_ms_ = 0;
    time_n_ = 0;
    timed_steps_ = 0;
    timing_launches_ = 0;
    halo_wait_ms_ = 0;
    halo_wait_n_ = 0;
    halo_timing_calls_ = 0;
    for (int p = 0; p < kParts; ++p) {
        part_ms_[p] = 0;
        part_n_[p] = 0;
    }
    part_timing_calls_ = 0;
    return WV_OK;
}

template <typename Real>
int Engine<Real>::query(int what, uint64_t* value) {
    if (!value) return fail(WV_E_INVALID_ARGUMENT, "null argument");
    switch (what) {
        case WV_QUERY_PASSES: *value = passes_taken_; return WV_OK;
        case WV_QUERY_XWALL_ENTRIES: *value = xw_active_ ? n_xw_ : 0; return WV_OK;
        case WV_QUERY_FIELDS: {
            uint64_t n = 0;
            for (int i = 0; i < 4; ++i) n += field_[i] != nullptr;
            n += field1_ != nullptr;
            *value = n;
            return WV_OK;
        }
        case WV_QUERY_MARCH_LIVE_PERMILLE:
            *value = (triple_units_ && triple_ready_) ? (uint64_t)(triple_live_frac_ * 1000.0 + 0.5) : pair_units_ ? (uint64_t)(pair_live_frac_ * 1000.0 + 0.5) : 1000;
            return WV_OK;
        case WV_QUERY_MARCH_ROUNDS: {
            if (!pair_map_ || pair_nw_ < 1) {
                *value = 0;
                return WV_OK;
            }
            const uint64_t slots = 256ull * (uint64_t)std::max(1, wv::kPairMaxWaves / pair_nw_);
            const uint64_t wgs = pair_units_ ? 8ull * pair_units_longest_
                                             : 8ull * (uint64_t)((pair_strips_ + 7) / 8) * (uint64_t)pair_chunks_ * (uint64_t)std::max(1, pair_windows_);
            *value = (wgs + slots - 1) / slots;
            return WV_OK;
        }
        case WV_QUERY_SWEEP_LIVE_PERMILLE: *value = tile_list_ ? (uint64_t)(tile_active_frac_ * 1000.0 + 0.5) : 1000; return WV_OK;
        case WV_QUERY_HALO_WAIT_NS: *value = (uint64_t)(halo_wait_ms_ * 1e6 + 0.5); return WV_OK;
        case WV_QUERY_HALO_WAITS: *value = halo_wait_n_; return WV_OK;
        case WV_QUERY_HALO_EXCHANGES: *value = comm_ ? comm_->exchanges() : 0; return WV_OK;
        case WV_QUERY_HALO_BYTES_SENT: *value = comm_ ? comm_->planes_sent() * (uint64_t)comm_->plane_bytes() : 0; return WV_OK;
        case WV_QUERY_EARLY_PASSES: *value = early_passes_; return WV_OK;
        case WV_QUERY_BOUNDARY1_NS: *value = (uint64_t)(part_ms_[0] * 1e6 + 0.5); return WV_OK;
        case WV_QUERY_BOUNDARY2_NS: *value = (uint64_t)(part_ms_[1] * 1e6 + 0.5); return WV_OK;
        case WV_QUERY_BOUNDARY_TIMED: *value = std::min(part_n_[0], part_n_[1]); return WV_OK;
        case WV_QUERY_WHOLE_STEPS: *value = whole_steps_; return WV_OK;
        case WV_QUERY_TRIPLE_PASSES: *value = triples_taken_; return WV_OK;
        case WV_QUERY_BOUNDARY3_NS: *value = (uint64_t)(part_ms_[2] * 1e6 + 0.5); return WV_OK;
        case WV_QUERY_FIXUP3_NS: *value = (uint64_t)(part_ms_[3] * 1e6 + 0.5); return WV_OK;
        case WV_QUERY_TRIPLE_PARTS_TIMED: *value = std::min(part_n_[2], part_n_[3]); return WV_OK;
        case WV_QUERY_TRIPLE_MARCH_NS: *value = (uint64_t)(part_ms_[4] * 1e6 + 0.5); return WV_OK;
        case WV_QUERY_TRIPLE_MARCH_TIMED: *value = part_n_[4]; return WV_OK;
        default: return fail(WV_E_INVALID_ARGUMENT, "unknown query");
    }
}

template <typename Real>
int Engine<Real>::synchronize() {
    DeviceGuard guard(device_);
    WV_HIP(hipStreamSynchronize(stream_));
    WV_HIP(hipStreamSynchronize(comm_stream_));
    return WV_OK;
}

}
```

wayverb_amd/csrc/engine_setup.hip.h:

```cpp
#pragma once
#include "engine.hip.h"

namespace wv {

template <typename Real>
int Engine<Real>::init(const wv_mesh& m, const wv_options& opt) {
    opt_ = opt;
    nx_ = m.nx;
    ny_ = m.ny;
    nz_ = m.nz;
    if (nx_ < 1 || ny_ < 1 || nz_ < 1) return fail(WV_E_INVALID_ARGUMENT, "mesh dimensions must be positive");
    n_nodes_ = (uint64_t)nx_ * ny_ * nz_;
    constexpr int kTile = 64 * (16 / (int)sizeof(Real));
    pitch_ = (nx_ + kTile - 1) / kTile * kTile;
    stored_nodes_ = (uint64_t)pitch_ * ny_ * nz_;
    if (stored_nodes_ >= 0xFFFFFFFEull)
        return fail(WV_E_INVALID_ARGUMENT,
                    "more than 2^32-2 stored nodes in one engine: decompose into z-slabs (32-bit local node indices)");
    if (!m.nodes || (!m.coefficients && m.num_coefficients))
        return fail(WV_E_INVALID_ARGUMENT, "mesh arrays missing");
    z_begin_ = opt.ghost_lo ? 1 : 0;
    z_end_ = opt.ghost_hi ? nz_ - 1 : nz_;
    if (z_end_ <= z_begin_) return fail(WV_E_INVALID_ARGUMENT, "slab has no owned planes");

    int count = 0;
    if (hipGetDeviceCount(&count) != hipSuccess || count == 0)
        return fail(WV_E_NO_DEVICE, "no HIP device visible; this engine has no CPU fallback");
    if (opt.device >= count) return fail(WV_E_INVALID_ARGUMENT, "no such HIP device");
    DeviceGuard guard(opt.device);
    WV_HIP(hipGetDevice(&device_));
    WV_HIP(hipStreamCreateWithFlags(&stream_, hipStreamNonBlocking));
    WV_HIP(hipStreamCreateWithFlags(&comm_stream_, hipStreamNonBlocking));

    field_bytes_ = stored_nodes_ * sizeof(Real);
    for (int i = 0; i < 2; ++i) {
        WV_HIP(hipMalloc((void**)&field_[i], field_bytes_ + 256));
        WV_HIP(hipMemsetAsync(field_[i], 0, field_bytes_ + 256, stream_));
    }
    prv_ = 0;
    cur_ = 1;

    cls_pitch_ = pitch_ / 4;
    const uint64_t cls_bytes = (uint64_t)cls_pitch_ * 4u * (uint64_t)((ny_ + 3) / 4) * nz_;
    WV_HIP(hipMalloc((void**)&cls_, cls_bytes + 16));
    WV_HIP(hipMemsetAsync(cls_, 0, cls_bytes + 16, stream_));
    n1_ = (uint32_t)m.num_boundary_1;
    n2_ = (uint32_t)m.num_boundary_2;
    n3_ = (uint32_t)m.num_boundary_3;
    if (m.num_boundary_1 + m.num_boundary_2 + m.num_boundary_3 >= 0xFFFFFFFFull)
        return fail(WV_E_INVALID_ARGUMENT, "too many boundary nodes");
    n_entries_ = n1_ + n2_ + n3_;
    n_slots_ = n1_ + 2u * n2_ + 3u * n3_;
    const size_t ne = std::max<size_t>(n_entries_, 1), ns = std::max<size_t>(n_slots_, 1);
    WV_HIP(hipMalloc((void**)&bnode_, ne * sizeof(uint32_t)));
    WV_HIP(hipMemsetAsync(bnode_, 0xFF, ne * sizeof(uint32_t), stream_));
    WV_HIP(hipMalloc((void**)&btype_, ne));
    WV_HIP(hipMemsetAsync(btype_, 0, ne, stream_));
    WV_HIP(hipMalloc((void**)&fmem_, ns * 6 * sizeof(double)));
    WV_HIP(hipMemsetAsync(fmem_, 0, ns * 6 * sizeof(double), stream_));
    WV_HIP(hipMalloc((void**)&cidx_, ns * sizeof(uint32_t)));
    WV_HIP(hipMalloc((void**)&status_, 4 * sizeof(int)));
    WV_HIP(hipMemsetAsync(status_, 0, 4 * sizeof(int), stream_));
    static_flag_dev_ = status_ + 1;

    {
        const bool resident = opt.nodes_on_device != 0;
        const int64_t rows_total = (int64_t)ny_ * nz_;
        const int64_t rows_per_chunk = resident ? rows_total : std::max<int64_t>(1, (int64_t)(32 << 20) / nx_);
        ScopedDevice stage_mem;
        if (!resident) WV_HIP(hipMalloc(&stage_mem.p, (size_t)rows_per_chunk * nx_ * sizeof(wv::NodeRec)));
        const wv::NodeRec* stage = resident ? reinterpret_cast<const wv::NodeRec*>(m.nodes)
                                            : static_cast<const wv::NodeRec*>(stage_mem.p);
        for (int64_t row = 0; row < rows_total; row += rows_per_chunk) {
            const int64_t rows = std::min(rows_per_chunk, rows_total - row);
            const int64_t first = row * nx_, cnt = rows * nx_;
            if (!resident)
                WV_HIP(hipMemcpyAsync(stage_mem.p, m.nodes + first, (size_t)cnt * sizeof(wv::NodeRec),
                                      hipMemcpyHostToDevice, stream_));
            wv::SetupArgs a{};
            a.nodes = stage;
            a.first_row = row;
            a.rows = rows;
            a.nx = nx_;
            a.ny = ny_;
            a.pitch = pitch_;
            a.cls_pitch = cls_pitch_;
            a.cls = cls_;
            a.bnode = bnode_;
            a.btype = btype_;
            a.n1 = n1_;
            a.n2 = n2_;
            a.n3 = n3_;
            a.status = status_;
            a.z_begin = z_begin_;
            a.z_end = z_end_;
            const int64_t n_bytes = rows * cls_pitch_;
            const unsigned grid = (unsigned)std::min<int64_t>((n_bytes + 255) / 256, 65536);
            hipLaunchKernelGGL(wv::setup_classify_kernel, dim3(grid), dim3(256), 0, stream_, a);
            WV_HIP(hipGetLastError());
            WV_HIP(hipStreamSynchronize(stream_));
        }
    }
    if (n_entries_) {
        wv::ValidateArgs v{};
        v.bnode = bnode_;
        v.btype = btype_;
        v.cls = cls_;
        v.n_entries = n_entries_;
        v.nx = nx_;
        v.ny = ny_;
        v.nz = nz_;
        v.pitch = pitch_;
        v.cls_pitch = cls_pitch_;
        v.static_flag = static_flag_dev_;
        hipLaunchKernelGGL(wv::setup_validate_kernel, dim3((n_entries_ + 255) / 256), dim3(256), 0, stream_, v);
        WV_HIP(hipGetLastError());
    }
    int status_host[4] = {0, 0, 0, 0};
    WV_HIP(hipMemcpyAsync(status_host, status_, sizeof(status_host), hipMemcpyDeviceToHost, stream_));
    WV_HIP(hipStreamSynchronize(stream_));
    if (status_host[0] & 1)
        return fail(WV_E_INVALID_MESH,
                    "node with an invalid boundary_type (boundary bits must be 1-3 direction bits on distinct axes)");
    if (status_host[0] & 2) return fail(WV_E_INVALID_MESH, "boundary_index exceeds the boundary array length");
    static_flag_ = status_host[1];

    std::vector<uint32_t> ref_to_pos(ne);
    for (uint32_t e = 0; e < n_entries_; ++e) ref_to_pos[e] = e;
    WV_HIP(hipMalloc((void**)&ref_to_pos_, ne * sizeof(uint32_t)));
    if (n_entries_ && opt_.tuning.boundary_order != 0) {
        std::vector<uint32_t> bnode(n_entries_);
        std::vector<uint8_t> btype(n_entries_);
        WV_HIP(hipMemcpy(bnode.data(), bnode_, (size_t)n_entries_ * sizeof(uint32_t), hipMemcpyDeviceToHost));
        WV_HIP(hipMemcpy(btype.data(), btype_, (size_t)n_entries_, hipMemcpyDeviceToHost));
        const uint32_t nd[3] = {n1_, n2_, n3_};
        std::vector<uint8_t> eligible(std::max<uint32_t>(n1_, 1), 0);
        if (n1_ && opt_.tuning.boundary_xwall != 0) {
            ScopedDevice flags_mem;
            WV_HIP(hipMalloc(&flags_mem.p, n1_));
            wv::XwEligibleArgs x{};
            x.bnode = bnode_;
            x.btype = btype_;
            x.cls = cls_;
            x.eligible = static_cast<uint8_t*>(flags_mem.p);
            x.n1 = n1_;
            x.nx = nx_;
            x.ny = ny_;
            x.nz = nz_;
            x.pitch = pitch_;
            x.cls_pitch = cls_pitch_;
            const int off = opt_.tuning.slab_early != 0 ? 2 : 1;
            x.march_begin = z_begin_ + (opt_.ghost_lo ? off : 0);
            x.march_end = z_end_ - (opt_.ghost_hi ? off : 0);
            hipLaunchKernelGGL(wv::xwall_eligible_kernel, dim3((n1_ + 255) / 256), dim3(256), 0, stream_, x);
            WV_HIP(hipGetLastError());
            WV_HIP(hipMemcpyAsync(eligible.data(), flags_mem.p, n1_, hipMemcpyDeviceToHost, stream_));
            WV_HIP(hipStreamSynchronize(stream_));
            for (uint32_t k = 0; k < n1_; ++k) n_xw_ += eligible[k];
            if (n_xw_ >= 0x7FFFFFFFu) n_xw_ = 0;
        }
        const uint64_t bricks_x = ((uint64_t)pitch_ + 63) / 64, bricks_y = ((uint64_t)ny_ + 7) / 8;
        std::vector<std::pair<uint64_t, uint32_t>> keyed(n_entries_);
        std::vector<uint32_t> by_pos(n_entries_);
        uint32_t off = 0;
        for (int d = 0; d < 3; ++d) {
            for (uint32_t k = 0; k < nd[d]; ++k) {
                const uint32_t idx = bnode[off + k];
                uint64_t kk = ~0ull >> 8;
                if (idx != wv::INVALID_NODE) {
                    const uint64_t x = idx % (uint32_t)pitch_, q = idx / (uint32_t)pitch_;
                    const uint64_t y = q % (uint32_t)ny_, z = q / (uint32_t)ny_;
                    const uint64_t brick = ((z >> 3) * bricks_y + (y >> 3)) * bricks_x + (x >> 6);
                    kk = (brick << 12) | ((z & 7) << 9) | ((y & 7) << 6) | (x & 63);
                }
                if (!(d == 0 && n_xw_ && eligible[k])) kk |= 1ull << 57;
                keyed[off + k] = {kk, off + k};
            }
            std::sort(keyed.begin() + off, keyed.begin() + off + nd[d]);
            for (uint32_t k = 0; k < nd[d]; ++k) by_pos[off + k] = keyed[off + k].second;
            off += nd[d];
        }
        std::vector<uint32_t> bnode2(n_entries_);
        std::vector<uint8_t> btype2(n_entries_);
        for (uint32_t pos = 0; pos < n_entries_; ++pos) {
            bnode2[pos] = bnode[by_pos[pos]];
            btype2[pos] = btype[by_pos[pos]];
            ref_to_pos[by_pos[pos]] = pos;
        }
        WV_HIP(hipMemcpy(bnode_, bnode2.data(), (size_t)n_entries_ * sizeof(uint32_t), hipMemcpyHostToDevice));
        WV_HIP(hipMemcpy(btype_, btype2.data(), (size_t)n_entries_, hipMemcpyHostToDevice));
    }
    WV_HIP(hipMemcpy(ref_to_pos_, ref_to_pos.data(), ne * sizeof(uint32_t), hipMemcpyHostToDevice));

    {
        std::vector<uint32_t> cidx(ns, 0u);
        const uint32_t* src[3] = {m.boundary_indices_1, m.boundary_indices_2, m.boundary_indices_3};
        const uint32_t nd[3] = {n1_, n2_, n3_};
        uint32_t base = 0, entry_off = 0;
        for (int d = 1; d <= 3; ++d) {
            if (nd[d - 1] && !src[d - 1]) return fail(WV_E_INVALID_ARGUMENT, "boundary index array missing");
            for (uint32_t k = 0; k < nd[d - 1]; ++k)
                for (int i = 0; i < d; ++i) {
                    const uint32_t c = src[d - 1][(size_t)k * d + i];
                    if (c >= m.num_coefficients)
                        return fail(WV_E_INVALID_MESH, "coefficient index exceeds the coefficient array length");
                    cidx[base + (uint32_t)i * nd[d - 1] + (ref_to_pos[entry_off + k] - entry_off)] = c;
                }
            base += (uint32_t)d * nd[d - 1];
            entry_off += nd[d - 1];
        }
        WV_HIP(hipMemcpy(cidx_, cidx.data(), ns * sizeof(uint32_t), hipMemcpyHostToDevice));
    }
    n_coeffs_ = m.num_coefficients;
    WV_HIP(hipMalloc((void**)&coeffs_, std::max<size_t>(n_coeffs_, 1) * sizeof(wv_coefficients_canonical)));
    if (n_coeffs_)
        WV_HIP(hipMemcpy(coeffs_, m.coefficients, n_coeffs_ * sizeof(wv_coefficients_canonical),
                         hipMemcpyHostToDevice));

    WV_HIP(hipMalloc((void**)&flags_, (kRing + 1) * sizeof(int)));
    WV_HIP(hipHostMalloc((void**)&flags_host_, kRing * sizeof(int), hipHostMallocDefault));
    WV_HIP(hipMalloc((void**)&scratch_, 64));

    courant_ = (Real)1 / (Real)std::sqrt((Real)3);
    courant_sq_ = (Real)1 / (Real)3;

    plan_stream();
    const int n_ev = 2 * kRing;
    events_.resize(n_ev);
    for (auto& e : events_) WV_HIP(hipEventCreate(&e));
    return WV_OK;
}

template <typename Real>
int Engine<Real>::set_tuning(int variant, int ry, int nwx, int nwy, int zchunks) {
    if (variant < 0 || variant > 3) return fail(WV_E_INVALID_ARGUMENT, "unknown stream variant");
    tune_variant_ = variant;
    tune_ry_ = ry;
    tune_nwx_ = nwx;
    tune_nwy_ = nwy;
    tune_zchunks_ = zchunks;
    plan_stream();
    return WV_OK;
}

template <typename Real>
int Engine<Real>::build_plane_order() {
    if (zorder_ || !n_entries_) return WV_OK;
    std::vector<uint32_t> bnode(n_entries_);
    WV_HIP(hipMemcpy(bnode.data(), bnode_, (size_t)n_entries_ * sizeof(uint32_t), hipMemcpyDeviceToHost));
    const uint32_t plane = (uint32_t)pitch_ * (uint32_t)ny_;
    plane_start_.assign((size_t)nz_ + 1, 0);
    for (uint32_t e = 0; e < n_entries_; ++e)
        if (bnode[e] != wv::INVALID_NODE) ++plane_start_[bnode[e] / plane + 1];
    for (int z = 0; z < nz_; ++z) plane_start_[z + 1] += plane_start_[z];
    std::vector<uint32_t> order(std::max<uint32_t>(plane_start_[nz_], 1)), cursor(plane_start_.begin(), plane_start_.end() - 1);
    for (uint32_t e = 0; e < n_entries_; ++e)
        if (bnode[e] != wv::INVALID_NODE) order[cursor[bnode[e] / plane]++] = e;
    plane_start_rest_.assign((size_t)nz_ + 1, 0);
    for (uint32_t e = n_xw_; e < n_entries_; ++e)
        if (bnode[e] != wv::INVALID_NODE) ++plane_start_rest_[bnode[e] / plane + 1];
    for (int z = 0; z < nz_; ++z) plane_start_rest_[z + 1] += plane_start_rest_[z];
    std::vector<uint32_t> rest(std::max<uint32_t>(plane_start_rest_[nz_], 1));
    cursor.assign(plane_start_rest_.begin(), plane_start_rest_.end() - 1);
    for (uint32_t e = n_xw_; e < n_entries_; ++e)
        if (bnode[e] != wv::INVALID_NODE) rest[cursor[bnode[e] / plane]++] = e;
    std::vector<uint32_t> face;
    {
        const int lo = opt_.ghost_lo ? 1 : 0, hi = opt_.ghost_hi ? 1 : 0;
        const int zi0 = std::min(z_begin_ + lo, z_end_), zi1 = std::max(z_end_ - hi, zi0);
        face.assign(order.begin() + plane_start_[z_begin_], order.begin() + plane_start_[zi0]);
        face.insert(face.end(), order.begin() + plane_start_[zi1], order.begin() + plane_start_[z_end_]);
        face_n_ = (uint32_t)face.size();
        if (face.empty()) face.push_back(0);
    }
    std::vector<uint32_t> early;
    {
        const int lo = opt_.ghost_lo ? 2 : 0, hi = opt_.ghost_hi ? 2 : 0;
        const int zi0 = std::min(z_begin_ + lo, z_end_), zi1 = std::max(z_end_ - hi, zi0);
        early.assign(order.begin() + plane_start_[z_begin_], order.begin() + plane_start_[zi0]);
        early.insert(early.end(), order.begin() + plane_start_[zi1], order.begin() + plane_start_[z_end_]);
        early_n_ = (uint32_t)early.size();
        if (early.empty()) early.push_back(0);
    }
    uint32_t* staged = nullptr;
    WV_HIP(hipMalloc((void**)&staged, (order.size() + rest.size() + face.size() + early.size()) * sizeof(uint32_t)));
    if (hipMemcpy(staged, order.data(), order.size() * sizeof(uint32_t), hipMemcpyHostToDevice) != hipSuccess ||
        hipMemcpy(staged + order.size(), rest.data(), rest.size() * sizeof(uint32_t), hipMemcpyHostToDevice) != hipSuccess ||
        hipMemcpy(staged + order.size() + rest.size(), face.data(), face.size() * sizeof(uint32_t), hipMemcpyHostToDevice) != hipSuccess ||
        hipMemcpy(staged + order.size() + rest.size() + face.size(), early.data(), early.size() * sizeof(uint32_t), hipMemcpyHostToDevice) !=
            hipSuccess) {
        (void)hipFree(staged);
        return fail(WV_E_HIP, "copying the plane order of the boundary entries to the device failed");
    }
    zorder_ = staged;
    zorder_rest_ = staged + order.size();
    face_order_ = zorder_rest_ + rest.size();
    early_order_ = face_order_ + face.size();
    return WV_OK;
}

template <typename Real>
void Engine<Real>::plan_stream() {
    lists_built_ = false;
    duties_known_ = false;
    if (graph_exec_) {
        (void)hipStreamSynchronize(stream_);
        (void)hipGraphExecDestroy(graph_exec_);
        graph_exec_ = nullptr;
    }
    StreamPlan& p = plan_;
    constexpr int VX = 16 / (int)sizeof(Real);
    constexpr int WX = 64 * VX;
    p.variant = tune_variant_ >= 0 ? tune_variant_ : opt_.stream_variant;
    if (p.variant < 0 || p.variant > 3) p.variant = 2;
    p.ry = tune_ry_ > 0 ? tune_ry_ : (opt_.tuning.stream_ry > 0 ? opt_.tuning.stream_ry : 4);
    p.nwx = tune_nwx_ > 0 ? tune_nwx_ : (opt_.tuning.stream_nwx > 0 ? opt_.tuning.stream_nwx : 1);
    p.nwy = tune_nwy_ > 0 ? tune_nwy_ : (opt_.tuning.stream_nwy > 0 ? opt_.tuning.stream_nwy : 4);
    if (p.ry != 2 && p.ry != 4) p.ry = 4;
    {
        const int key = p.nwx * 10 + p.nwy;
        const int ok[] = {11, 14, 18, 22, 24, 41, 42, 81};
        bool found = false;
        for (int k : ok) found = found || k == key;
        if (!found) {
            p.nwx = 1;
            p.nwy = 4;
        }
    }
    p.tiles_x = (pitch_ + WX * p.nwx - 1) / (WX * p.nwx);
    p.tiles_y = (ny_ + p.ry * p.nwy - 1) / (p.ry * p.nwy);
    p.block = 64u * (unsigned)(p.nwx * p.nwy);
    const int owned = z_end_ - z_begin_;
    const int64_t knob = tune_zchunks_ > 0 ? tune_zchunks_ : opt_.tuning.stream_zchunks;
    if (p.variant == 2 || p.variant == 3) {
        const int tile_rows = p.ry * p.nwy;
        int64_t rows = knob > 0 ? knob : (int64_t)(1600 * 1024) / (3ll * pitch_ * (int64_t)sizeof(Real));
        if (knob > 0) {
            rows = std::max<int64_t>(tile_rows, rows / tile_rows * tile_rows);
        } else {
            const int64_t budget = std::max<int64_t>(rows, tile_rows);
            double best = -1.0;
            for (int64_t r = tile_rows; r <= budget; r += tile_rows) {
                const int64_t stripes = (ny_ + r - 1) / r, rounds = (stripes + 7) / 8;
                const double used = (double)ny_ / (double)(rounds * 8 * r);
                if (used >= best - 1e-12) {
                    best = used;
                    rows = r;
                }
            }
        }
        rows = std::max<int64_t>(rows, 1);
        p.stripe_rows = (int)rows;
        p.tiles_y_stripe = (p.stripe_rows + tile_rows - 1) / tile_rows;
        const int stripes = (ny_ + p.stripe_rows - 1) / p.stripe_rows;
        p.passes = (stripes + 7) / 8;
        return;
    }
    if (p.variant == 1) {
        p.block = 256;
        p.grid = (unsigned)std::min<uint64_t>((n_nodes_ + 255) / 256, 256ull * 64);
        return;
    }
    const int64_t wave_tiles = (int64_t)p.tiles_x * p.tiles_y * p.nwx * p.nwy;
    int64_t want = knob;
    if (want <= 0) want = (65536 + wave_tiles - 1) / wave_tiles;
    want = std::max<int64_t>(1, std::min<int64_t>(want, owned));
    p.zc = (int)((owned + want - 1) / want);
}

template <typename Real>
int Engine<Real>::build_tile_lists(int z0, int z1) {
    if (lists_built_) return WV_OK;
    lists_built_ = true;
    lists_z0_ = z0;
    lists_z1_ = z1;
    if (tile_list_) {
        (void)hipFree(tile_list_);
        tile_list_ = nullptr;
    }
    if ((plan_.variant != 2 && plan_.variant != 3) || !use_work_lists()) return WV_OK;
    const int wave_cols = 64 * (16 / (int)sizeof(Real));
    const int wtiles_x = plan_.tiles_x * plan_.nwx;
    const int wtiles_y = (ny_ + plan_.ry - 1) / plan_.ry;
    const int tile_rows = plan_.ry * plan_.nwy;
    const int tiles_y = (ny_ + tile_rows - 1) / tile_rows;
    const int64_t n_tiles = (int64_t)nz_ * wtiles_y * wtiles_x;
    ScopedDevice act_mem;
    WV_HIP(hipMalloc(&act_mem.p, (size_t)n_tiles));
    wv::TileActivityArgs t{};
    t.cls = cls_;
    t.active = static_cast<uint8_t*>(act_mem.p);
    t.ny = ny_;
    t.nz = nz_;
    t.pitch = pitch_;
    t.cls_pitch = cls_pitch_;
    t.tile_rows = plan_.ry;
    t.tile_cols = wave_cols;
    t.tiles_x = wtiles_x;
    t.tiles_y = wtiles_y;
    hipLaunchKernelGGL(wv::tile_activity_kernel, dim3((unsigned)((n_tiles + 255) / 256)), dim3(256), 0, stream_, t);
    WV_HIP(hipGetLastError());
    std::vector<uint8_t> active((size_t)n_tiles);
    WV_HIP(hipMemcpyAsync(active.data(), act_mem.p, (size_t)n_tiles, hipMemcpyDeviceToHost, stream_));
    WV_HIP(hipStreamSynchronize(stream_));

    const int stripes = (ny_ + plan_.stripe_rows - 1) / plan_.stripe_rows;
    const int tys = plan_.tiles_y_stripe;
    auto wave_mask = [&](int z, int ty, int tx) -> uint32_t {
        uint32_t m = 0;
        for (int wy = 0; wy < plan_.nwy; ++wy) {
            const int wty = ty * plan_.nwy + wy;
            if (wty >= wtiles_y) break;
            for (int wx = 0; wx < plan_.nwx; ++wx) {
                const int wtx = tx * plan_.nwx + wx;
                if (wtx < wtiles_x && active[((size_t)z * wtiles_y + wty) * wtiles_x + wtx]) m |= 1u << (wy * plan_.nwx + wx);
            }
        }
        return m;
    };
    std::vector<uint64_t> per_stripe((size_t)stripes, 0);
    uint64_t total_active = 0, total = 0;
    for (int z = z0; z < z1; ++z)
        for (int ty = 0; ty < tiles_y; ++ty)
            for (int tx = 0; tx < plan_.tiles_x; ++tx) {
                const uint64_t on = (uint64_t)__builtin_popcount(wave_mask(z, ty, tx));
                per_stripe[(size_t)(ty / tys)] += on;
                total_active += on;
                total += (uint64_t)(plan_.nwx * plan_.nwy);
            }
    tile_active_frac_ = total ? (double)total_active / (double)total : 1.0;
    if (total_active * 100 >= total * 92 || stripes >= (1 << 16) || nz_ >= (1 << 20) ||
        (int64_t)plan_.tiles_x * tys >= (1 << 20) || plan_.nwx * plan_.nwy > 8)
        return WV_OK;

    std::vector<int> order((size_t)stripes);
    for (int i = 0; i < stripes; ++i) order[(size_t)i] = i;
    std::stable_sort(order.begin(), order.end(), [&](int a, int b) { return per_stripe[(size_t)a] > per_stripe[(size_t)b]; });
    std::vector<std::vector<int>> mine(8);
    uint64_t load[8] = {0, 0, 0, 0, 0, 0, 0, 0};
    for (int sidx : order) {
        int best = 0;
        for (int k = 1; k < 8; ++k)
            if (load[k] < load[best]) best = k;
        mine[(size_t)best].push_back(sidx);
        load[best] += per_stripe[(size_t)sidx];
    }
    std::vector<uint64_t> list;
    list.reserve((size_t)total_active / 2 + 16);
    list_longest_ = 0;
    for (int k = 0; k < 8; ++k) {
        list_start_[k] = (uint32_t)list.size();
        for (int sidx : mine[(size_t)k])
            for (int z = z0; z < z1; ++z)
                for (int tyl = 0; tyl < tys; ++tyl) {
                    const int ty = sidx * tys + tyl;
                    if (ty >= tiles_y) break;
                    for (int tx = 0; tx < plan_.tiles_x; ++tx) {
                        const uint32_t m = wave_mask(z, ty, tx);
                        if (m)
                            list.push_back(((uint64_t)sidx << 48) | ((uint64_t)m << 40) | ((uint64_t)z << 20) |
                                           (uint64_t)(tyl * plan_.tiles_x + tx));
                    }
                }
        list_longest_ = std::max<uint32_t>(list_longest_, (uint32_t)list.size() - list_start_[k]);
    }
    list_start_[8] = (uint32_t)list.size();
    if (list.empty()) return WV_OK;
    uint64_t* staged = nullptr;
    WV_HIP(hipMalloc((void**)&staged, list.size() * sizeof(uint64_t)));
    if (hipMemcpy(staged, list.data(), list.size() * sizeof(uint64_t), hipMemcpyHostToDevice) != hipSuccess) {
        (void)hipFree(staged);
        return fail(WV_E_HIP, "copying the tile work list to the device failed");
    }
    tile_list_ = staged;
    return WV_OK;
}

template <typename Real>
void Engine<Real>::release() {
    DeviceGuard guard(device_);
    if (comm_ && comm_->dead()) {
        comm_.release();
        return;
    }
    comm_.reset();
    if (stream_) (void)hipStreamSynchronize(stream_);
    for (auto& e : events_) (void)hipEventDestroy(e);
    events_.clear();
    for (auto& e : halo_events_)
        if (e) (void)hipEventDestroy(e);
    halo_events_.clear();
    for (auto& ev : part_events_) {
        for (auto& e : ev)
            if (e) (void)hipEventDestroy(e);
        ev.clear();
    }
    for (int i = 0; i < 4; ++i)
        if (field_[i]) (void)hipFree(field_[i]);
    if (graph_exec_) (void)hipGraphExecDestroy(graph_exec_);
    for (auto& f : ckpt_.field)
        if (f) (void)hipFree(f);
    if (ckpt_.fmem) (void)hipFree(ckpt_.fmem);
    void* ptrs[] = {field1_, triple_map_, triple_list_, triple_units_, suspect_, pair_units_, pair_map_, pair_list_, pair_counter_, signal_base_dev_, tile_list_, xw_nbr_, xw_val_, xw_gok_, ref_to_pos_, cls_,   bnode_,      btype_,    fmem_,  cidx_,
                    status_,          coeffs_,    flags_,      scratch_, signal_, recv_nodes_, recv_out_, zorder_};
    for (void* p : ptrs)
        if (p) (void)hipFree(p);
    if (flags_host_) (void)hipHostFree(flags_host_);
    if (recv_stage_) (void)hipHostFree(recv_stage_);
    if (duties_) (void)hipFree(duties_);
    if (stream_) (void)hipStreamDestroy(stream_);
    if (comm_stream_) (void)hipStreamDestroy(comm_stream_);
}

}
```

wayverb_amd/csrc/engine_single.hip.h:

```cpp
#pragma once
#include "engine.hip.h"

namespace wv {

template <typename Real>
template <int RY, int NWX, int NWY>
void Engine<Real>::launch_shape(const wv::StreamArgs<Real>& a, unsigned grid) {
    if (plan_.variant == 2) {
        hipLaunchKernelGGL((wv::stream_sweep_kernel<Real, RY, NWX, NWY>), dim3(grid), dim3(64 * NWX * NWY), 0,
                           st(), a);
    } else if (plan_.variant == 3) {
        hipLaunchKernelGGL((wv::stream_sweep_nolds_kernel<Real, RY, NWX, NWY>), dim3(grid), dim3(64 * NWX * NWY), 0,
                           st(), a);
    } else {
        hipLaunchKernelGGL((wv::stream_march_kernel<Real, RY, NWX, NWY>), dim3(grid), dim3(64 * NWX * NWY), 0,
                           st(), a);
    }
}

template <typename Real>
template <int RY>
void Engine<Real>::launch_ry(const wv::StreamArgs<Real>& a, unsigned grid) {
    switch (plan_.nwx * 10 + plan_.nwy) {
        case 11: launch_shape<RY, 1, 1>(a, grid); break;
        case 22: launch_shape<RY, 2, 2>(a, grid); break;
        case 41: launch_shape<RY, 4, 1>(a, grid); break;
        case 42: launch_shape<RY, 4, 2>(a, grid); break;
        case 81: launch_shape<RY, 8, 1>(a, grid); break;
        case 18: launch_shape<RY, 1, 8>(a, grid); break;
        case 24: launch_shape<RY, 2, 4>(a, grid); break;
        default: launch_shape<RY, 1, 4>(a, grid); break;
    }
}

template <typename Real>
int Engine<Real>::launch_stream(Real* prev, const Real* cur, int* flag, int z0, int z1, bool timed, Real* out, int zb0, int zb1,
                                StreamLaunch* plan_only) {
    if (zb0 < zb1 && z0 >= z1) return launch_stream(prev, cur, flag, zb0, zb1, timed, out, 0, 0, plan_only);
    if (zb0 < zb1 && plan_.variant != 2 && plan_.variant != 3) {
        const int rc = launch_stream(prev, cur, flag, z0, z1, timed, out);
        return rc ? rc : launch_stream(prev, cur, flag, zb0, zb1, false, out);
    }
    if (z0 >= z1) return WV_OK;
    const int second = zb0 < zb1 ? zb1 - zb0 : 0;
    wv::StreamArgs<Real> a{};
    a.prev = prev;
    a.next = out ? out : prev;
    a.cur = cur;
    a.cls = cls_;
    a.flag = flag;
    a.nx = nx_;
    a.ny = ny_;
    a.nz = nz_;
    a.pitch = pitch_;
    a.cls_pitch = cls_pitch_;
    a.z_begin = z0;
    a.z_end = z1 + second;
    a.z_skip_from = second ? z1 : std::numeric_limits<int>::max();
    a.z_skip = second ? zb0 - z1 : 0;
    a.tiles_x = plan_.tiles_x;
    a.tiles_y = plan_.tiles_y;
    unsigned grid = plan_.grid;
    if (plan_.variant == 2 || plan_.variant == 3) {
        a.stripe_rows = plan_.stripe_rows;
        a.tiles_y_stripe = plan_.tiles_y_stripe;
        a.passes = plan_.passes;
        grid = 8u * (unsigned)plan_.passes * (unsigned)(z1 - z0 + second) * (unsigned)(a.tiles_x * a.tiles_y_stripe);
        if (!second && (int64_t)(z1 - z0) * 2 > (int64_t)(z_end_ - z_begin_) && outside_dirty_ == 0) {
            int rc = build_tile_lists(z0, z1);
            if (rc) return rc;
            if (tile_list_ && z0 == lists_z0_ && z1 == lists_z1_) {
                a.tile_list = tile_list_;
                for (int k = 0; k < 9; ++k) a.list_start[k] = list_start_[k];
                grid = 8u * list_longest_;
            }
        }
    } else if (plan_.variant == 0) {
        a.zc = std::min(plan_.zc, z1 - z0);
        a.chunks_z = (z1 - z0 + a.zc - 1) / a.zc;
        a.total_tiles = a.tiles_x * a.tiles_y * a.chunks_z;
        a.tiles_per_xcd = (a.total_tiles + 7) / 8;
        grid = (unsigned)a.tiles_per_xcd * 8u;
    }
    if (plan_only) {
        plan_only->args = a;
        plan_only->grid = grid;
        return WV_OK;
    }
    timed = timed && !on_ && time_this_launch();
    if (timed) WV_HIP(hipEventRecord(events_[ev_used_], stream_));
    if (plan_.variant == 1) {
        hipLaunchKernelGGL(wv::stream_naive_kernel<Real>, dim3(grid), dim3(plan_.block), 0, st(), a);
    } else if (plan_.ry == 2) {
        launch_ry<2>(a, grid);
    } else {
        launch_ry<4>(a, grid);
    }
    if (timed) {
        WV_HIP(hipEventRecord(events_[ev_used_ + 1], stream_));
        ev_used_ += 2;
        timed_steps_ += 1;
    }
    return WV_OK;
}

template <typename Real>
wv::BoundaryArgs<Real> Engine<Real>::boundary_args(Real* prev, const Real* cur, int* flag) const {
    wv::BoundaryArgs<Real> b{};
    b.prev = prev;
    b.next = prev;
    b.cur = cur;
    b.flag = flag;
    b.bnode = bnode_;
    b.btype = btype_;
    b.fmem = fmem_;
    b.cidx = cidx_;
    b.coeffs = coeffs_;
    b.n_coeffs = n_coeffs_;
    b.n1 = n1_;
    b.n2 = n2_;
    b.n3 = n3_;
    b.n_slots = n_slots_;
    b.nx = nx_;
    b.ny = ny_;
    b.nz = nz_;
    b.pitch = pitch_;
    b.z_begin = z_begin_;
    b.z_end = z_end_;
    b.courant = courant_;
    b.courant_sq = courant_sq_;
    return b;
}

template <typename Real>
int Engine<Real>::launch_boundary(Real* prev, const Real* cur, int* flag, int z0, int z1, const wv::PrePostArgs<Real>* next, Real* out, bool fix_inner,
                                  bool levels, BoundaryLaunch* plan_only, int xw3) {
    const bool faces = z0 == z1 && (z0 == -1 || z0 == -2);
    if (!n_entries_ || (z0 >= z1 && !faces)) return WV_OK;
    wv::BoundaryArgs<Real> b = boundary_args(prev, cur, flag);
    if (out) b.next = out;
    b.fix_z0 = z0;
    b.fix_z1 = z1;
    wv::PrePostArgs<Real> nx{};
    if (next) {
        nx = *next;
        nx.fused = 1;
    }
    const bool xw = out && xw_active_ && (levels || xw3);
    uint32_t n = n_entries_ - (xw ? n_xw_ : 0u);
    if (faces) {
        const int rc = build_plane_order();
        if (rc != WV_OK) return rc;
        b.order = z0 == -1 ? face_order_ : early_order_;
        b.n_order = n = z0 == -1 ? face_n_ : early_n_;
        if (!n) return WV_OK;
    } else if (z0 > z_begin_ || z1 < z_end_) {
        const int rc = build_plane_order();
        if (rc != WV_OK) return rc;
        const uint32_t* order = xw ? zorder_rest_ : zorder_;
        const std::vector<uint32_t>& start = xw ? plane_start_rest_ : plane_start_;
        b.order = order + start[z0];
        b.n_order = start[z1] - start[z0];
        n = b.n_order;
        if (!n && !xw) return WV_OK;
    }
    if (xw) {
        xwall_args(b);
        n += b.xw_pad;
    }
    const bool lds = n_coeffs_ <= wv::kMaxLdsCoefficientSets && opt_.tuning.boundary_lds != 0;
    if (plan_only) {
        plan_only->args = b;
        plan_only->blocks = (n + 255) / 256;
        plan_only->lds = lds;
        return WV_OK;
    }
    const dim3 grid((n + 255) / 256 + (nx.fused ? 1u : 0u)), block(256);
    if (xw && xw3) {
        if (lds && xw3 == 1)
            hipLaunchKernelGGL((wv::boundary_kernel<Real, true, false, 1>), grid, block, 0, st(), b, nx);
        else if (lds && xw3 == 2 && fix_inner)
            hipLaunchKernelGGL((wv::boundary_kernel<Real, true, true, 2>), grid, block, 0, st(), b, nx);
        else if (lds && xw3 == 3)
            hipLaunchKernelGGL((wv::boundary_kernel<Real, true, false, 3>), grid, block, 0, st(), b, nx);
        else if (xw3 == 1)
            hipLaunchKernelGGL((wv::boundary_kernel<Real, false, false, 1>), grid, block, 0, st(), b, nx);
        else if (xw3 == 2 && fix_inner)
            hipLaunchKernelGGL((wv::boundary_kernel<Real, false, true, 2>), grid, block, 0, st(), b, nx);
        else if (xw3 == 3)
            hipLaunchKernelGGL((wv::boundary_kernel<Real, false, false, 3>), grid, block, 0, st(), b, nx);
        else
            return fail(WV_E_STATE, "launch_boundary: a three-step pass's second level on compact copies without its entries finishing the nodes they face");
    } else if (lds && fix_inner)
        hipLaunchKernelGGL((wv::boundary_kernel<Real, true, true>), grid, block, 0, st(), b, nx);
    else if (lds)
        hipLaunchKernelGGL((wv::boundary_kernel<Real, true, false>), grid, block, 0, st(), b, nx);
    else if (fix_inner)
        hipLaunchKernelGGL((wv::boundary_kernel<Real, false, true>), grid, block, 0, st(), b, nx);
    else
        hipLaunchKernelGGL((wv::boundary_kernel<Real, false, false>), grid, block, 0, st(), b, nx);
    return WV_OK;
}

template <typename Real>
int Engine<Real>::launch_faces(Real* prev, const Real* cur, int* flag, Real* out, int planes) {
    const int lo = opt_.ghost_lo ? planes : 0, hi = opt_.ghost_hi ? planes : 0;
    const int zi0 = std::min(z_begin_ + lo, z_end_), zi1 = std::max(z_end_ - hi, zi0);
    if (opt_.tuning.fuse_planes != 0 && plan_.variant == 2 && plan_.ry == 4 && plan_.nwx == 1 && plan_.nwy == 4 && n_entries_) {
        StreamLaunch sw;
        BoundaryLaunch bd;
        int rc = launch_stream(prev, cur, flag, z_begin_, zi0, false, out, zi1, z_end_, &sw);
        if (rc) return rc;
        if ((rc = launch_boundary(prev, cur, flag, -planes, -planes, nullptr, out, false, false, &bd))) return rc;
        if (sw.grid && bd.blocks) {
            const dim3 grid(sw.grid + bd.blocks), block(256);
            if (bd.lds)
                hipLaunchKernelGGL((wv::plane_step_kernel<Real, true>), grid, block, 0, st(), sw.args, bd.args, (uint32_t)sw.grid);
            else
                hipLaunchKernelGGL((wv::plane_step_kernel<Real, false>), grid, block, 0, st(), sw.args, bd.args, (uint32_t)sw.grid);
            return WV_OK;
        }
    }
    int rc = launch_stream(prev, cur, flag, z_begin_, zi0, false, out, zi1, z_end_);
    if (rc) return rc;
    return launch_boundary(prev, cur, flag, -planes, -planes, nullptr, out);
}

template <typename Real>
wv::PrePostArgs<Real> Engine<Real>::pre_post_args(Real* cur, int slot, bool with_pre_post, uint64_t signal_pos, bool source_live) const {
    const bool io = with_pre_post && (n_recv_ || source_live);
    wv::PrePostArgs<Real> pp{};
    pp.cur = cur;
    pp.signal = signal_;
    pp.signal_pos = signal_pos;
    pp.signal_base = graph_capturing_ ? signal_base_dev_ : nullptr;
    pp.source_node = source_node_;
    pp.source_kind = io && source_live ? source_kind_ : 0;
    pp.recv = recv_nodes_;
    pp.recv_out = recv_out_ ? recv_out_ + (size_t)slot * std::max<uint32_t>(n_recv_, 1) : nullptr;
    pp.n_recv = io ? n_recv_ : 0;
    pp.flag = flags_ + slot;
    pp.flag_init = static_flag_;
    return pp;
}

constexpr uint64_t kWholeStepMaxBytes = 160ull << 20;

template <typename Real>
bool Engine<Real>::whole_step_sized() const {
    return 2ull * stored_nodes_ * sizeof(Real) <= kWholeStepMaxBytes;
}

template <typename Real>
bool Engine<Real>::whole_step_ready() {
    if (opt_.tuning.whole_step == 0 || comm_ || opt_.ghost_lo || opt_.ghost_hi) return false;
    if (plan_.variant != 2 || plan_.ry != 4 || plan_.nwx != 1 || plan_.nwy != 4) return false;
    if (opt_.tuning.whole_step < 0 && !whole_step_sized()) return false;
    if (duties_known_) return duties_ok_;
    duties_known_ = true;
    duties_ok_ = false;
    if (n_recv_ > 63) return false;
    std::vector<uint64_t> recv(n_recv_);
    if (n_recv_ && hipMemcpy(recv.data(), recv_nodes_, (size_t)n_recv_ * sizeof(uint64_t), hipMemcpyDeviceToHost) != hipSuccess) {
        (void)hipGetLastError();
        return false;
    }
    constexpr int WX = 64 * (16 / (int)sizeof(Real));
    const int nzr = z_end_ - z_begin_;
    const int per_plane = plan_.tiles_x * plan_.tiles_y_stripe;
    auto duty = [&](uint64_t idx, uint32_t col, uint32_t kind, wv::StepDuty* out) -> bool {
        const int x = (int)(idx % (uint64_t)pitch_);
        const uint64_t row = idx / (uint64_t)pitch_;
        const int y = (int)(row % (uint64_t)ny_), z = (int)(row / (uint64_t)ny_);
        uint32_t cls = 0;
        if (z < z_begin_ || z >= z_end_ || class_of((uint64_t)x, row, &cls) != hipSuccess) {
            (void)hipGetLastError();
            return false;
        }
        if (!(cls & 1u)) return false;
        const int stripe = y / plan_.stripe_rows;
        const int tl = ((y - stripe * plan_.stripe_rows) / 16) * plan_.tiles_x + x / WX;
        const uint32_t j = (uint32_t)(((stripe / 8) * nzr + (z - z_begin_)) * per_plane + tl);
        *out = wv::StepDuty{idx, j * 8u + (uint32_t)(stripe % 8), col, kind, 0u};
        return true;
    };
    std::vector<wv::StepDuty> list;
    wv::StepDuty q{};
    if (source_kind_ != WV_SOURCE_NONE) {
        if (!duty(source_node_, 0u, source_kind_ == WV_SOURCE_HARD ? 1u : 2u, &q)) return false;
        list.push_back(q);
    }
    for (uint32_t c = 0; c < n_recv_; ++c) {
        if (recv[c] == ~0ull) continue;
        if (!duty(recv[c], c, 0u, &q)) return false;
        list.push_back(q);
    }
    if (!duties_ && hipMalloc((void**)&duties_, 64 * sizeof(wv::StepDuty)) != hipSuccess) {
        (void)hipGetLastError();
        duties_ = nullptr;
        return false;
    }
    if (hipStreamSynchronize(stream_) != hipSuccess) return false;
    if (!list.empty() && hipMemcpy(duties_, list.data(), list.size() * sizeof(wv::StepDuty), hipMemcpyHostToDevice) != hipSuccess) {
        (void)hipGetLastError();
        return false;
    }
    n_duties_ = (uint32_t)list.size();
    duties_ok_ = true;
    return true;
}

template <typename Real>
int Engine<Real>::launch_whole_step(Real* prev, const Real* cur, int slot, uint64_t signal_pos, bool source_live, bool serve_next) {
    int* flag = flags_ + slot;
    StreamLaunch sw;
    BoundaryLaunch bd;
    int rc = launch_stream(prev, cur, flag, z_begin_, z_end_, false, nullptr, 0, 0, &sw);
    if (rc) return rc;
// ... 135 lines not shown
```

wayverb_amd/csrc/engine_triple.hip.h:

```cpp
#pragma once
#include "engine.hip.h"
#include "triple_kernels.hip.h"

namespace wv {

template <typename Real>
bool Engine<Real>::triple_eligible() {
    if (opt_.tuning.triple == 0 || triple_failed_) return false;
    const bool slab = opt_.ghost_lo || opt_.ghost_hi;
    if (slab != (comm_ != nullptr)) return false;
    if (slab) {
        if (z_end_ - z_begin_ < (opt_.ghost_lo ? 2 : 0) + (opt_.ghost_hi ? 2 : 0) + 2) return false;
    }
    if (!pair_eligible()) return false;
    const int lb = triple_lane_bytes();
    const int WX = 64 * (lb / (int)sizeof(Real));
    uint8_t win[4][wv::kTripleMaxWindows];
    int widest = 0;
    if (wv::triple_windows(pitch_ / WX, win, &widest, false, wv::triple_max_waves(lb)) < 0) return false;
    if (opt_.tuning.triple < 0 && stored_nodes_ < triple_min_nodes_) return false;
    return true;
}

template <typename Real>
int Engine<Real>::triple_lane_bytes() const {
    if (opt_.tuning.triple_lanes == 8 || opt_.tuning.triple_lanes == 16) return opt_.tuning.triple_lanes;
    if (sizeof(Real) == 4) return (pitch_ > 512 && pitch_ <= 768) ? 16 : 8;
    if (pitch_ < triple_wide_from_) return 8;
    return (pitch_ >= 512 && pitch_ < 768) ? 8 : 16;
}

template <typename Real>
int Engine<Real>::ensure_triple() {
    int rc = ensure_pair();
    if (rc) return rc;
    triple_z0_ = z_begin_ + (opt_.ghost_lo ? 2 : 0);
    triple_z1_ = z_end_ - (opt_.ghost_hi ? 2 : 0);
    if (pair_failed_ || (!pair_sparse_ok_ && opt_.tuning.triple < 0)) {
        triple_ready_ = false;
        return WV_OK;
    }
    const uint64_t src = source_kind_ != WV_SOURCE_NONE ? source_node_ : ~0ull;
    if (!field1_) {
        if (hipMalloc((void**)&field1_, field_bytes_ + 256) != hipSuccess) {
            (void)hipGetLastError();
            field1_ = nullptr;
            triple_failed_ = true;
            triple_ready_ = false;
            return WV_OK;
        }
        WV_HIP(hipMemsetAsync(field1_, 0, field_bytes_ + 256, stream_));
    }
    if (!suspect_) {
        WV_HIP(hipMalloc((void**)&suspect_, kRing * sizeof(int)));
        WV_HIP(hipMemsetAsync(suspect_, 0, kRing * sizeof(int), stream_));
    }
    const bool xw = xw_active_ && pair_inner_ok_ > 0 && opt_.tuning.boundary_xwall != 2 && !(comm_ && opt_.tuning.slab_early == 0);
    if (triple_map_ && triple_source_ == src && triple_io_generation_ == io_generation_ && triple_xw_ == xw) {
        triple_ready_ = !(pair_units_ && !triple_units_);
        return WV_OK;
    }
    const uint64_t cls_bytes = (uint64_t)cls_pitch_ * 4u * (uint64_t)((ny_ + 3) / 4) * nz_;
    if (!triple_map_) {
        WV_HIP(hipMalloc((void**)&triple_map_, cls_bytes + 16));
        WV_HIP(hipMemsetAsync(triple_map_, 0, cls_bytes + 16, stream_));
    }
    const int64_t n_bytes = (int64_t)cls_pitch_ * ny_ * nz_;
    const unsigned blocks = (unsigned)((n_bytes + 255) / 256);
    ScopedDevice counts;
    WV_HIP(hipMalloc(&counts.p, (size_t)blocks * sizeof(uint32_t)));
    wv::TripleMapArgs m{};
    m.pair_map = pair_map_;
    m.map = triple_map_;
    m.block_count = static_cast<uint32_t*>(counts.p);
    m.ny = ny_;
    m.nz = nz_;
    m.pitch = pitch_;
    m.cls_pitch = cls_pitch_;
    m.z_begin = triple_z0_;
    m.z_end = triple_z1_;
    ScopedDevice covered;
    if (xw) {
        const size_t words = (size_t)((stored_nodes_ + 31) / 32) + 1;
        WV_HIP(hipMalloc(&covered.p, words * sizeof(uint32_t)));
        WV_HIP(hipMemsetAsync(covered.p, 0, words * sizeof(uint32_t), stream_));
        wv::XwCoverArgs c{};
        c.bnode = bnode_;
        c.btype = btype_;
        c.covered = static_cast<uint32_t*>(covered.p);
        c.xw_n = n_xw_;
        c.pair_map = pair_map_;
        c.gok = xw_gok_;
        c.nx = nx_;
        c.ny = ny_;
        c.nz = nz_;
        c.pitch = pitch_;
        c.cls_pitch = cls_pitch_;
        hipLaunchKernelGGL(wv::xwall_cover_kernel, dim3((n_xw_ + 255) / 256), dim3(256), 0, stream_, c);
        WV_HIP(hipGetLastError());
        m.covered = c.covered;
    }
    triple_xw_ = xw;
    hipLaunchKernelGGL(wv::triple_map_kernel, dim3(blocks), dim3(256), 0, stream_, m);
    WV_HIP(hipGetLastError());
    std::vector<uint32_t> per_block(blocks);
    WV_HIP(hipMemcpyAsync(per_block.data(), counts.p, (size_t)blocks * sizeof(uint32_t), hipMemcpyDeviceToHost, stream_));
    WV_HIP(hipStreamSynchronize(stream_));
    uint64_t total = 0;
    for (unsigned b = 0; b < blocks; ++b) {
        const uint32_t c = per_block[b];
        per_block[b] = (uint32_t)total;
        total += c;
    }
    if (triple_list_) {
        (void)hipFree(triple_list_);
        triple_list_ = nullptr;
    }
    triple_list_n_ = 0;
    if (total >= (1ull << 32)) {
        triple_ready_ = false;
        return WV_OK;
    }
    if (total) {
        WV_HIP(hipMalloc((void**)&triple_list_, (size_t)total * sizeof(uint32_t)));
        WV_HIP(hipMemcpyAsync(counts.p, per_block.data(), (size_t)blocks * sizeof(uint32_t), hipMemcpyHostToDevice, stream_));
        m.list = triple_list_;
        hipLaunchKernelGGL(wv::triple_map_kernel, dim3(blocks), dim3(256), 0, stream_, m);
        WV_HIP(hipGetLastError());
        triple_list_n_ = (uint32_t)total;
    }
    WV_HIP(hipStreamSynchronize(stream_));
    if (n_recv_ || src != ~0ull) {
        wv::TripleMarkArgs k{};
        k.map = triple_map_;
        k.recv = recv_nodes_;
        k.n_recv = n_recv_;
        k.source_node = src;
        k.ny = ny_;
        k.pitch = pitch_;
        k.cls_pitch = cls_pitch_;
        hipLaunchKernelGGL(wv::triple_mark_kernel, dim3((n_recv_ + 1 + 255) / 256), dim3(256), 0, stream_, k);
        WV_HIP(hipGetLastError());
    }
    triple_source_ = src;
    triple_io_generation_ = io_generation_;
    const int lb = triple_lb_ = triple_lane_bytes();
    const int WX = 64 * (lb / (int)sizeof(Real));
    int widest = 0;
    triple_windows_ = wv::triple_windows(pitch_ / WX, triple_win_, &widest, false, wv::triple_max_waves(lb));
    if (triple_windows_ < 0) {
        triple_ready_ = false;
        return WV_OK;
    }
    triple_nw_ = widest;
    triple_strips_ = (ny_ + wv::kTripleRows - 1) / wv::kTripleRows;
    const size_t lds = wv::triple_lds_bytes(triple_nw_, false, lb);
    const int by_lds = std::max<int>(1, (int)((160u * 1024u) / lds));
    const int by_waves = std::max(1, (lb == 16 ? 8 : 12) / triple_nw_);
    const int64_t slots = 256ll * std::min(by_lds, by_waves);
    const int owned = triple_z1_ - triple_z0_;
    int chunks = opt_.tuning.triple_chunks;
    if (chunks <= 0) {
        const int64_t want_rounds = ((opt_.ghost_lo || opt_.ghost_hi) && comm_ && comm_->peers_elsewhere()) ? 2 : 1;
        double best[2] = {0, 0};
        int at[2] = {0, 0};
        for (int c = 1; c <= std::max(1, owned / 12) && c <= 256; ++c) {
            const int64_t wgs = (int64_t)triple_strips_ * c * std::max(1, triple_windows_);
            const int64_t rounds = (wgs + slots - 1) / slots;
            const double zc = (double)((owned + c - 1) / c);
            const double cost = (double)(rounds * slots) / (double)wgs * (zc + 4.0) / zc;
            for (int k = 0; k < 2; ++k)
                if ((k == 0 || rounds >= want_rounds) && (at[k] == 0 || cost < best[k] - 1e-9)) {
                    best[k] = cost;
                    at[k] = c;
                }
        }
        chunks = (at[1] && best[1] <= 1.06 * best[0]) ? at[1] : std::max(1, at[0]);
    }
    chunks = std::max(1, std::min(chunks, std::max(1, owned / 4)));
    triple_zc_ = (owned + chunks - 1) / chunks;
    triple_chunks_ = (owned + triple_zc_ - 1) / triple_zc_;
    if (triple_units_) {
        (void)hipFree(triple_units_);
        triple_units_ = nullptr;
    }
    if (pair_units_ && (rc = build_triple_units())) return rc;
    if (pair_units_ && !triple_units_) {
        triple_ready_ = false;
        return WV_OK;
    }
    if (!triple_attr_set_) {
        WV_HIP(hipFuncSetAttribute(reinterpret_cast<const void*>(&wv::triple_march_kernel<Real, 0, false, 8>),
                                   hipFuncAttributeMaxDynamicSharedMemorySize, 160 * 1024));
        WV_HIP(hipFuncSetAttribute(reinterpret_cast<const void*>(&wv::triple_march_kernel<Real, 0, false, kWideLaneBytes>),
                                   hipFuncAttributeMaxDynamicSharedMemorySize, 160 * 1024));
        triple_attr_set_ = true;
    }
    triple_ready_ = true;
    return WV_OK;
}

template <typename Real>
int Engine<Real>::build_triple_units() {
    const int owned = triple_z1_ - triple_z0_;
    const int z_lo = triple_z0_, z_hi = triple_z1_, extra_lo = triple_z0_ > z_begin_ ? 1 : 0, extra_hi = triple_z1_ < z_end_ ? 1 : 0;
    const int lb = triple_lb_;
    const int WX = 64 * (lb / (int)sizeof(Real));
    const int row_waves = pitch_ / WX;
    if (triple_windows_ || triple_strips_ >= (1 << 14) || row_waves > 16) return WV_OK;
    const int64_t n_cells = (int64_t)nz_ * triple_strips_;
    ScopedDevice act_mem, raw_mem;
    WV_HIP(hipMalloc(&act_mem.p, (size_t)n_cells));
    WV_HIP(hipMalloc(&raw_mem.p, (size_t)n_cells * sizeof(uint16_t)));
    wv::TileActivityArgs t{};
    t.cls = cls_;
    t.active = static_cast<uint8_t*>(act_mem.p);
    t.ny = ny_;
    t.nz = nz_;
    t.pitch = pitch_;
    t.cls_pitch = cls_pitch_;
    t.tile_rows = wv::kTripleRows;
    t.tile_cols = pitch_;
    t.tiles_x = 1;
    t.tiles_y = triple_strips_;
    hipLaunchKernelGGL(wv::tile_activity_kernel, dim3((unsigned)((n_cells + 255) / 256)), dim3(256), 0, stream_, t);
    WV_HIP(hipGetLastError());
    static_assert(wv::kTripleRows == wv::kPairRows, "pair_wave_activity_kernel counts strips of kPairRows rows");
    wv::WaveActivityArgs w{};
    w.cls = cls_;
    w.raw16 = static_cast<uint16_t*>(raw_mem.p);
    w.ny = ny_;
    w.nz = nz_;
    w.pitch = pitch_;
    w.cls_pitch = cls_pitch_;
    w.strips = triple_strips_;
    w.nw = row_waves;
    w.wave_cols = WX;
    hipLaunchKernelGGL(wv::pair_wave_activity_kernel, dim3((unsigned)((n_cells + 255) / 256)), dim3(256), 0, stream_, w);
    WV_HIP(hipGetLastError());
    std::vector<uint8_t> active((size_t)n_cells);
    std::vector<uint16_t> raw((size_t)n_cells);
    WV_HIP(hipMemcpyAsync(active.data(), act_mem.p, (size_t)n_cells, hipMemcpyDeviceToHost, stream_));
    WV_HIP(hipMemcpyAsync(raw.data(), raw_mem.p, (size_t)n_cells * sizeof(uint16_t), hipMemcpyDeviceToHost, stream_));
    WV_HIP(hipStreamSynchronize(stream_));
    const int per_cu = std::max(1, (lb == 16 ? 8 : 12) / std::max(1, triple_nw_));
    const int64_t slots_per_xcd = 32ll * per_cu;
    auto units_of = [&](int height, std::vector<uint32_t>* per_strip) -> uint64_t {
        const int n_chunks = (owned + height - 1) / height;
        uint64_t units = 0;
        for (int sidx = 0; sidx < triple_strips_; ++sidx)
            for (int c = 0; c < n_chunks; ++c) {
                const int zb = z_lo + c * height, ze = std::min(zb + height, z_hi);
                bool any = false;
// ... 19 lines not shown
    };
    int zc;
    if (opt_.tuning.triple_chunks > 0) {
        zc = std::max(4, (owned + opt_.tuning.triple_chunks - 1) / opt_.tuning.triple_chunks);
    } else {
        const int base = std::max(8, std::min(owned, opt_.tuning.pair_unit_planes + 8));
        zc = base;
        double best = rounds_cost(zc);
        for (int height = base * 3 / 4; height <= base * 5 / 4; ++height) {
            if (height < 8 || height > owned) continue;
            const double cost = rounds_cost(height);
            if (cost > 0 && cost < best * 0.97) {
                best = cost;
                zc = height;
            }
        }
    }
    const int chunks = (owned + zc - 1) / zc;
    if (chunks >= (1 << 9)) return WV_OK;
    std::vector<std::vector<uint32_t>> of_strip((size_t)triple_strips_);
    uint64_t total = 0, live_waves = 0;
    for (int sidx = 0; sidx < triple_strips_; ++sidx)
        for (int c = 0; c < chunks; ++c) {
            const int zb = z_lo + c * zc, ze = std::min(zb + zc, z_hi);
            bool any = false;
            for (int z = zb - (zb == z_lo ? extra_lo : 0); z < ze + (ze == z_hi ? extra_hi : 0) && !any; ++z) any = active[(size_t)z * triple_strips_ + sidx] != 0;
            if (!any) continue;
            uint32_t bits = 0;
            for (int z = std::max(0, zb - 3); z < std::min(nz_, ze + 3); ++z)
                for (int ss = std::max(0, sidx - 1); ss <= std::min(triple_strips_ - 1, sidx + 1); ++ss) bits |= raw[(size_t)z * triple_strips_ + ss];
            const uint32_t lo = std::min((uint32_t)__builtin_ctz(bits | (1u << 31)), (uint32_t)row_waves - 1u);
            const uint32_t hi = std::min(32u - (uint32_t)__builtin_clz(bits | 1u), (uint32_t)row_waves);
            const uint32_t span = hi > lo ? hi - lo : 1u;
            of_strip[(size_t)sidx].push_back(wv::triple_unit_entry((uint32_t)sidx, (uint32_t)c, lo, span));
            live_waves += span;
            ++total;
        }
    if (!total) return WV_OK;
    triple_live_frac_ = (double)live_waves / ((double)triple_strips_ * chunks * row_waves);
    std::vector<uint32_t> list;
    list.reserve((size_t)total);
    triple_units_longest_ = 0;
    int sidx = 0;
    for (int k = 0; k < 8; ++k) {
        triple_unit_start_[k] = (uint32_t)list.size();
        const uint64_t want = total * (uint64_t)(k + 1) / 8;
        const size_t first = list.size();
        while (sidx < triple_strips_ && (list.size() < want || k == 7)) {
            list.insert(list.end(), of_strip[(size_t)sidx].begin(), of_strip[(size_t)sidx].end());
            ++sidx;
        }
        std::stable_sort(list.begin() + (std::ptrdiff_t)first, list.end(), [](uint32_t a, uint32_t b) { return ((a >> 14) & 0x1FFu) < ((b >> 14) & 0x1FFu); });
        triple_units_longest_ = std::max<uint32_t>(triple_units_longest_, (uint32_t)list.size() - triple_unit_start_[k]);
    }
    triple_unit_start_[8] = (uint32_t)list.size();
    uint32_t* staged = nullptr;
    WV_HIP(hipMalloc((void**)&staged, list.size() * sizeof(uint32_t)));
    if (hipMemcpy(staged, list.data(), list.size() * sizeof(uint32_t), hipMemcpyHostToDevice) != hipSuccess) {
        (void)hipFree(staged);
        return fail(WV_E_HIP, "copying the three-step march's unit list to the device failed");
    }
    triple_units_ = staged;
    triple_zc_ = zc;
    triple_chunks_ = chunks;
    return WV_OK;
}

template <typename Real>
int Engine<Real>::launch_triple_march(int slot, const Real* A, const Real* B, Real* O1, Real* O2, Real* O3) {
    int rc;
    wv::TripleArgs<Real> a{};
    a.prev = A;
    a.cur = B;
    a.out1 = O1;
    a.out2 = O2;
    a.out3 = O3;
    a.map = triple_map_;
    a.suspect = suspect_ + slot;
    a.ny = ny_;
    a.nz = nz_;
    a.pitch = pitch_;
    a.cls_pitch = cls_pitch_;
    a.z_begin = triple_z0_;
    a.z_end = triple_z1_;
    a.z2_lo = triple_z0_ > z_begin_ ? 1 : 0;
    a.z2_hi = triple_z1_ < z_end_ ? 1 : 0;
    a.nw = triple_nw_;
    a.zc = triple_zc_;
    a.chunks = triple_chunks_;
    a.strips = triple_strips_;
    a.strips_per_xcd = (triple_strips_ + 7) / 8;
    a.windows = triple_windows_;
    for (int k = 0; k < triple_windows_; ++k) {
        a.win_first |= (uint64_t)triple_win_[0][k] << (8 * k);
        a.win_count |= (uint64_t)triple_win_[1][k] << (8 * k);
        a.win_store_lo |= (uint64_t)triple_win_[2][k] << (8 * k);
        a.win_store_hi |= (uint64_t)triple_win_[3][k] << (8 * k);
    }
    unsigned grid = 8u * (unsigned)a.strips_per_xcd * (unsigned)triple_chunks_ * (unsigned)std::max(1, triple_windows_);
    if (triple_units_) {
        a.unit_list = triple_units_;
        for (int k = 0; k < 9; ++k) a.list_start[k] = triple_unit_start_[k];
        grid = 8u * triple_units_longest_;
    }
    const bool timed = timing && time_this_launch();
    const int token = timed ? begin_part_timing(4, true) : -1;
    if (triple_lb_ == 8)
        hipLaunchKernelGGL((wv::triple_march_kernel<Real, 0, false, 8>), dim3(grid), dim3(64u * (unsigned)triple_nw_),
                           wv::triple_lds_bytes(triple_nw_, false, 8), stream_, a);
    else
        hipLaunchKernelGGL((wv::triple_march_kernel<Real, 0, false, kWideLaneBytes>), dim3(grid), dim3(64u * (unsigned)triple_nw_),
                           wv::triple_lds_bytes(triple_nw_, false, kWideLaneBytes), stream_, a);
    if ((rc = end_part_timing(4, token))) return rc;
    pass_timed_ = timed && (part_timing_calls_++ & 7u) == 0;
    return WV_OK;
}

template <typename Real>
int Engine<Real>::launch_triple_list(int slot, const Real* A, const Real* B, const Real* O1, const Real* O2, Real* O3, bool source_live) {
    wv::PairFixupArgs<Real> f{};
    f.nodes = triple_list_;
    f.n = triple_list_n_;
    f.t1 = O2;
    f.cur = O1;
    f.out2 = O3;
    f.flag2 = flags_ + slot + 2;
    f.nx = nx_;
    f.ny = ny_;
    f.nz = nz_;
    f.pitch = pitch_;
    wv::TripleFlagsArgs<Real> g{};
    g.prev = A;
    g.cur = B;
    g.out2 = O2;
    g.out3 = O3;
    g.pair_map = pair_map_;
    g.suspect = suspect_ + slot;
    g.flag1 = flags_ + slot;
    g.flag2 = flags_ + slot + 1;
    g.flag3 = flags_ + slot + 2;
    g.source_node = source_live ? source_node_ : ~0ull;
    g.nx = nx_;
    g.ny = ny_;
    g.nz = nz_;
    g.pitch = pitch_;
    g.cls_pitch = cls_pitch_;
    g.z_begin = triple_z0_;
    g.z_end = triple_z1_;
    hipLaunchKernelGGL(wv::triple_list_kernel<Real>, dim3(std::max(1u, (triple_list_n_ + 255) / 256)), dim3(256), 0, stream_, f, g);
    return WV_OK;
}

template <typename Real>
int Engine<Real>::enqueue_triple(int slot, uint64_t signal_pos, bool source_live, int fuse_next) {
    DeviceGuard guard(device_);
    Real* A = field_[prv_];
    Real* B = field_[cur_];
    Real* O1 = field1_;
    Real* O2 = field_[spare_[0]];
    Real* O3 = field_[spare_[1]];
    int* flag1 = flags_ + slot;
    int* flag2 = flags_ + slot + 1;
    int* flag3 = flags_ + slot + 2;
    int rc;
    const bool io = n_recv_ || source_live;
    const bool fuse = batch_can_fuse_ && n_entries_ != 0;
    if (!pre_post_done_ && io) {
        wv::PrePostArgs<Real> pp = pre_post_args(B, slot, true, signal_pos, source_live);
        pp.flag = nullptr;
        hipLaunchKernelGGL(wv::pre_post_kernel<Real>, dim3(1), dim3(64), 0, stream_, pp);
    }
    pre_post_done_ = false;
    if ((rc = launch_triple_march(slot, A, B, O1, O2, O3))) return rc;
    bool list2_done = false;
    const bool xw = triple_xw_ && xw_active_;
    if (xw && !xw_valid_) {
        wv::BoundaryArgs<Real> g = boundary_args(A, B, flag1);
        xwall_args(g);
        hipLaunchKernelGGL(wv::xwall_gather_kernel<Real>, dim3(g.xw_pad / 256), dim3(256), 0, stream_, g);
    }
    xw_valid_ = xw;
    int token = begin_part_timing(0);
    if (fuse && io) {
        wv::PrePostArgs<Real> nx = pre_post_args(O1, slot + 1, true, signal_pos + 1, source_live);
        nx.flag = nullptr;
        if (pair_list_early_ok_ && pair_list_n_) {
            nx.fix_nodes = pair_list_;
            nx.fix_n = pair_list_n_;
            nx.fix_cur = B;
            nx.fix_out2 = O2;
            nx.fix_flag = flag2;
            nx.nx = nx_;
            nx.ny = ny_;
            nx.nz = nz_;
            nx.pitch = pitch_;
            list2_done = true;
        }
        if ((rc = launch_boundary(A, B, flag1, z_begin_, z_end_, &nx, O1, false, false, nullptr, xw ? 1 : 0))) return rc;
    } else {
        if ((rc = launch_boundary(A, B, flag1, z_begin_, z_end_, nullptr, O1, false, false, nullptr, xw ? 1 : 0))) return rc;
        if (io) {
            wv::PrePostArgs<Real> pp = pre_post_args(O1, slot + 1, true, signal_pos + 1, source_live);
            pp.flag = nullptr;
            hipLaunchKernelGGL(wv::pre_post_kernel<Real>, dim3(1), dim3(64), 0, stream_, pp);
        }
    }
    if ((rc = end_part_timing(0, token))) return rc;
    if (!list2_done && (rc = launch_fixup(0, pair_list_n_, O1, B, O2, flag2))) return rc;
    token = begin_part_timing(1);
    if (fuse && io && io_nodes_unfaced()) {
        wv::PrePostArgs<Real> nx = pre_post_args(O2, slot + 2, true, signal_pos + 2, source_live);
        nx.flag = nullptr;
        if ((rc = launch_boundary(B, O1, flag2, z_begin_, z_end_, &nx, O2, pair_inner_ok_ > 0, false, nullptr, xw ? 2 : 0))) return rc;
    } else {
        if ((rc = launch_boundary(B, O1, flag2, z_begin_, z_end_, nullptr, O2, pair_inner_ok_ > 0, false, nullptr, xw ? 2 : 0))) return rc;
        if (io) {
            wv::PrePostArgs<Real> pp = pre_post_args(O2, slot + 2, true, signal_pos + 2, source_live);
            pp.flag = nullptr;
            hipLaunchKernelGGL(wv::pre_post_kernel<Real>, dim3(1), dim3(64), 0, stream_, pp);
        }
    }
    if ((rc = end_part_timing(1, token))) return rc;
    token = begin_part_timing(3);
    if ((rc = launch_triple_list(slot, A, B, O1, O2, O3, source_live))) return rc;
    if ((rc = end_part_timing(3, token))) return rc;
    token = begin_part_timing(2);
    if (fuse && fuse_next && (!xw || io_nodes_clear_of_x_walls())) {
        wv::PrePostArgs<Real> nx = pre_post_args(O3, slot + 3, true, signal_pos + 3, source_live);
        if (fuse_next == 2) nx.flag2 = flags_ + slot + 4;
        if ((rc = launch_boundary(O1, O2, flag3, z_begin_, z_end_, &nx, O3, false, false, nullptr, xw ? 3 : 0))) return rc;
        pre_post_done_ = true;
    } else if ((rc = launch_boundary(O1, O2, flag3, z_begin_, z_end_, nullptr, O3, false, false, nullptr, xw ? 3 : 0))) {
        return rc;
    }
    if ((rc = end_part_timing(2, token))) return rc;
    pass_timed_ = false;
    WV_HIP(hipGetLastError());
    ++triples_taken_;
    const int a_idx = prv_, b_idx = cur_;
    prv_ = spare_[0];
    cur_ = spare_[1];
    spare_[0] = a_idx;
    spare_[1] = b_idx;
    return WV_OK;
}

template <typename Real>
int Engine<Real>::enqueue_triple_slab(int slot, int part, uint64_t signal_pos, bool source_live) {
    DeviceGuard guard(device_);
    Real* A = field_[prv_];
    Real* B = field_[cur_];
    Real* O1 = field1_;
    Real* O2 = field_[spare_[0]];
    Real* O3 = field_[spare_[1]];
    int* flag1 = flags_ + slot;
    int* flag2 = flags_ + slot + 1;
    int* flag3 = flags_ + slot + 2;
    int rc;
    std::string cerr;
    const bool io = n_recv_ || source_live;
    const bool xw = triple_xw_ && xw_active_;
    const size_t plane = (size_t)pitch_ * ny_;
    const int z0 = triple_z0_, z1 = triple_z1_;
    const int n0 = z0 - (opt_.ghost_lo ? 1 : 0), n1 = z1 + (opt_.ghost_hi ? 1 : 0);
    auto pre_post = [&](Real* field, int step) {
        if (!io) return;
        wv::PrePostArgs<Real> pp = pre_post_args(field, slot + step, true, signal_pos + (uint64_t)step, source_live);
        pp.flag = nullptr;
        hipLaunchKernelGGL(wv::pre_post_kernel<Real>, dim3(1), dim3(64), 0, stream_, pp);
    };
    auto wait_for = [&](int field) -> int {
        const int token = begin_halo_wait_timing();
        if (!comm_->wait_ghosts(stream_, field, &cerr)) return fail(WV_E_COMM, cerr);
        return end_halo_wait_timing(token);
    };
    auto copy_plane = [&](Real* dst, const Real* src, int z) -> int {
        WV_HIP(hipMemcpyAsync(dst + (size_t)z * plane, src + (size_t)z * plane, plane * sizeof(Real), hipMemcpyDeviceToDevice, stream_));
        return WV_OK;
    };
    if (!batch_flags_reset_) return fail(WV_E_STATE, "a slab's three-step pass without the batch's flag words reset");
    if (part == 0) {
        if ((rc = wait_for(cur_))) return rc;
        pre_post(B, 0);
        pre_post_done_ = false;
        if ((rc = launch_faces(A, B, flag1, O1, 2))) return rc;
        WV_HIP(hipGetLastError());
        if (opt_.ghost_lo && (rc = copy_plane(O3, O1, z_begin_))) return rc;
        if (opt_.ghost_hi && (rc = copy_plane(O3, O1, z_end_ - 1))) return rc;
        const bool ahead = opt_.tuning.slab_early == 2;
        if (ahead && !comm_->exchange_faces(stream_, spare_[1], &cerr)) return fail(WV_E_COMM, cerr);
        if (!comm_->bulk_begin(stream_, &cerr)) return fail(WV_E_COMM, cerr);
        if ((rc = launch_triple_march(slot, A, B, O1, O2, O3))) return rc;
        if (!comm_->bulk_end(stream_, &cerr)) return fail(WV_E_COMM, cerr);
        if (!ahead && !comm_->exchange_faces(stream_, spare_[1], &cerr)) return fail(WV_E_COMM, cerr);
        if (xw && !xw_valid_) {
            wv::BoundaryArgs<Real> g = boundary_args(A, B, flag1);
            xwall_args(g);
            hipLaunchKernelGGL(wv::xwall_gather_kernel<Real>, dim3(g.xw_pad / 256), dim3(256), 0, stream_, g);
        }
        xw_valid_ = xw;
        const int token = begin_part_timing(0);
        if ((rc = launch_boundary(A, B, flag1, z0, z1, nullptr, O1, false, false, nullptr, xw ? 1 : 0))) return rc;
        if ((rc = end_part_timing(0, token))) return rc;
    } else if (part == 1) {
        if ((rc = wait_for(spare_[1]))) return rc;
        if (opt_.ghost_lo && (rc = copy_plane(O1, O3, 0))) return rc;
        if (opt_.ghost_hi && (rc = copy_plane(O1, O3, nz_ - 1))) return rc;
        pre_post(O1, 1);
        if ((rc = launch_faces(B, O1, flag2, O2, 1))) return rc;
        WV_HIP(hipGetLastError());
        if (!comm_->exchange_faces(stream_, spare_[0], &cerr)) return fail(WV_E_COMM, cerr);
        if ((rc = launch_fixup(0, pair_list_n_, O1, B, O2, flag2))) return rc;
        const int token = begin_part_timing(1);
        if ((rc = launch_boundary(B, O1, flag2, n0, n1, nullptr, O2, pair_inner_ok_ > 0, false, nullptr, xw ? 2 : 0))) return rc;
        if ((rc = end_part_timing(1, token))) return rc;
    } else {
        if ((rc = wait_for(spare_[0]))) return rc;
        pre_post(O2, 2);
        if ((rc = launch_faces(O1, O2, flag3, O3, 2))) return rc;
        WV_HIP(hipGetLastError());
        if (!comm_->exchange_faces(stream_, spare_[1], &cerr)) return fail(WV_E_COMM, cerr);
        int token = begin_part_timing(3);
        if ((rc = launch_triple_list(slot, A, B, O1, O2, O3, source_live))) return rc;
        if ((rc = end_part_timing(3, token))) return rc;
        token = begin_part_timing(2);
        if ((rc = launch_boundary(O1, O2, flag3, z0, z1, nullptr, O3, false, false, nullptr, xw ? 3 : 0))) return rc;
        if ((rc = end_part_timing(2, token))) return rc;
        pass_timed_ = false;
        WV_HIP(hipGetLastError());
        if (!comm_->step_done(stream_, &cerr)) return fail(WV_E_COMM, cerr);
        ++triples_taken_;
        const int a_idx = prv_, b_idx = cur_;
        prv_ = spare_[0];
        cur_ = spare_[1];
        spare_[0] = a_idx;
        spare_[1] = b_idx;
    }
    return WV_OK;
}

template <typename Real>
int Engine<Real>::batch_triple_prepare(int* ready) {
    DeviceGuard guard(device_);
    *ready = 0;
    if (!triple_eligible()) return WV_OK;
    const int rc = ensure_triple();
    if (rc == WV_E_HIP && wv::last_hip_error() == hipErrorOutOfMemory) {
        (void)hipGetLastError();
        triple_failed_ = true;
        return WV_OK;
    }
    if (rc) return rc;
    *ready = triple_ready_ ? 1 : 0;
    if (*ready && suspect_) WV_HIP(hipMemsetAsync(suspect_, 0, kRing * sizeof(int), stream_));
    return WV_OK;
}

template <typename Real>
int Engine<Real>::enqueue_batch_triple(uint64_t i, int part) {
    if (comm_) return enqueue_triple_slab((int)i, part, signal_pos_ + i, batch_source_live_);
    return part == 0 ? enqueue_triple((int)i, signal_pos_ + i, batch_source_live_, 0) : WV_OK;
}

}
```

wayverb_amd/engine.py:

```python
import ctypes as C
import os

import numpy as np

from . import mesh as M

_HERE = os.path.dirname(os.path.abspath(__file__))
_LIB_PATH = os.path.join(_HERE, "libwayverb_amd.so")

WV_OK = 0
PRECISION_F32 = 0
PRECISION_F64 = 1
BUF_CURRENT = 0
BUF_PREVIOUS = 1
SOURCE_NONE, SOURCE_HARD, SOURCE_SOFT = 0, 1, 2
NO_NODE = 0xFFFFFFFFFFFFFFFF
UNIQUE_ID_BYTES = 128

EXPORTS = [
    "wv_create", "wv_destroy", "wv_last_error", "wv_default_options", "wv_read_value", "wv_write_value",
    "wv_read_field", "wv_write_field", "wv_read_planes", "wv_write_planes", "wv_read_boundary_data", "wv_write_boundary_data",
    "wv_set_coefficients", "wv_device_buffer", "wv_step", "wv_swap", "wv_set_source",
    "wv_set_receivers", "wv_run", "wv_fetch_receivers", "wv_step_count", "wv_kernel_time_ms",
    "wv_enable_kernel_timing", "wv_kernel_time_detail", "wv_query", "wv_measure_triad", "wv_synchronize", "wv_comm_unique_id", "wv_comm_init",
    "wv_comm_destroy", "wv_comm_use_library", "wv_comm_init_local", "wv_run_group", "wv_make_box_nodes", "wv_set_stream_tuning", "wv_filter_test_2", "wv_field_pitch", "wv_classify_nodes", "wv_voxelise", "wv_nodes_inside",
    "wv_boundary_index_data", "wv_arbitrary_magnitude_filter", "wv_is_stable", "wv_band_centres",
    "wv_reflectance_filter", "wv_impedance_coefficients", "wv_attenuate", "wv_adjust_sampling_rate",
    "wv_frequency_domain_filter", "wv_postprocess_waveguide", "wv_hrtf_attenuation", "wv_hrtf_ear_position",
    "wv_attenuate_hrtf", "wv_multiband_filter_and_mixdown", "wv_postprocess_waveguide_hrtf", "wv_scene_mesh_create", "wv_scene_mesh_fetch",
    "wv_scene_mesh_create_engine", "wv_scene_mesh_destroy", "wv_checkpoint", "wv_rollback", "wv_drop_checkpoint", "wv_host_register", "wv_host_unregister",
    "wv_compressed_waveguide_run", "wv_make_transparent",
]


class WvMesh(C.Structure):
    _fields_ = [("nx", C.c_int32), ("ny", C.c_int32), ("nz", C.c_int32),
                ("nodes", C.c_void_p), ("coefficients", C.c_void_p), ("num_coefficients", C.c_uint32),
                ("boundary_indices_1", C.c_void_p), ("boundary_indices_2", C.c_void_p),
                ("boundary_indices_3", C.c_void_p),
                ("num_boundary_1", C.c_uint64), ("num_boundary_2", C.c_uint64), ("num_boundary_3", C.c_uint64)]


TUNING_FIELDS = ("pair", "pair_chunks", "pair_inner_fix", "pair_wide", "pair_unit_waves", "pair_unit_planes", "pair_units_by_chunk", "tile_lists",
                 "fuse_pre_post", "graph", "boundary_lds", "boundary_order", "boundary_xwall",
                 "stream_ry", "stream_nwx", "stream_nwy", "stream_zchunks", "slab_early", "pair_split_rows", "fuse_planes", "whole_step", "triple",
                 "triple_chunks", "triple_lanes")


class WvTuning(C.Structure):
    _fields_ = [(name, C.c_int32) for name in TUNING_FIELDS]


class WvOptions(C.Structure):
    _fields_ = [("struct_size", C.c_int32), ("precision", C.c_int32), ("device", C.c_int32),
                ("ghost_lo", C.c_int32), ("ghost_hi", C.c_int32), ("flag_interval", C.c_int32),
                ("stream_variant", C.c_int32), ("all_tiles", C.c_int32), ("nodes_on_device", C.c_int32), ("comm_timeout_s", C.c_int32), ("transport", C.c_int32), ("reserved_", C.c_int32 * 5),
                ("tuning", WvTuning)]


default_tuning = {}


def tuning_from_env(environ=None):
    environ = os.environ if environ is None else environ
    out = {}
    for name in TUNING_FIELDS + ("stream_variant",):
        v = environ.get("WV_" + name.upper())
        if v is not None:
            out[name] = int(v)
    return out


def apply_tuning(opt, tuning=None):
    merged = dict(default_tuning)
    merged.update(tuning or {})
    for name, value in merged.items():
        if name == "stream_variant":
            opt.stream_variant = int(value)
        elif name in TUNING_FIELDS:
            setattr(opt.tuning, name, int(value))
        else:
            raise ValueError("unknown tuning field %r" % name)


class WaveguideError(RuntimeError):
    pass


class ValueIsInf(WaveguideError):
    """core::exceptions::value_is_inf (src/core/include/core/exceptions.h:28-30)"""


class ValueIsNan(WaveguideError):
    """core::exceptions::value_is_nan (exceptions.h:24-26)"""


_lib = None


def load_library():
    global _lib
    if _lib is not None:
        return _lib
    if not os.path.exists(_LIB_PATH):
        raise WaveguideError(
            "%s not built: run `python -m wayverb_amd.build` (there is no CPU fallback)" % _LIB_PATH)
    if os.environ.get("WV_NO_TORCH_PRELOAD") != "1":
        try:
            import torch
        except Exception:
            pass
    lib = C.CDLL(_LIB_PATH, mode=C.RTLD_GLOBAL)
    lib.wv_last_error.restype = C.c_char_p
    lib.wv_create.argtypes = [C.POINTER(WvMesh), C.POINTER(WvOptions), C.POINTER(C.c_void_p)]
    lib.wv_destroy.argtypes = [C.c_void_p]
    lib.wv_destroy.restype = None
    lib.wv_default_options.argtypes = [C.POINTER(WvOptions)]
    lib.wv_default_options.restype = None
    lib.wv_read_value.argtypes = [C.c_void_p, C.c_int, C.c_uint64, C.POINTER(C.c_double)]
    lib.wv_write_value.argtypes = [C.c_void_p, C.c_int, C.c_uint64, C.c_double]
    lib.wv_read_field.argtypes = [C.c_void_p, C.c_int, C.c_void_p, C.c_int]
    lib.wv_write_field.argtypes = [C.c_void_p, C.c_int, C.c_void_p, C.c_int]
    lib.wv_read_planes.argtypes = [C.c_void_p, C.c_int, C.c_int32, C.c_int32, C.c_void_p, C.c_int]
    lib.wv_write_planes.argtypes = [C.c_void_p, C.c_int, C.c_int32, C.c_int32, C.c_void_p, C.c_int]
    lib.wv_read_boundary_data.argtypes = [C.c_void_p, C.c_int, C.c_void_p]
    lib.wv_write_boundary_data.argtypes = [C.c_void_p, C.c_int, C.c_void_p]
    lib.wv_set_coefficients.argtypes = [C.c_void_p, C.c_void_p, C.c_uint32]
    lib.wv_device_buffer.argtypes = [C.c_void_p, C.c_int, C.POINTER(C.c_void_p)]
    lib.wv_step.argtypes = [C.c_void_p, C.POINTER(C.c_int32)]
    lib.wv_checkpoint.argtypes = [C.c_void_p]
    lib.wv_rollback.argtypes = [C.c_void_p]
    lib.wv_drop_checkpoint.argtypes = [C.c_void_p]
    lib.wv_swap.argtypes = [C.c_void_p]
    lib.wv_set_source.argtypes = [C.c_void_p, C.c_int, C.c_uint64, C.c_void_p, C.c_uint64]
    lib.wv_set_receivers.argtypes = [C.c_void_p, C.c_void_p, C.c_uint32]
    lib.wv_run.argtypes = [C.c_void_p, C.c_uint64, C.POINTER(C.c_uint64), C.POINTER(C.c_int32)]
    lib.wv_fetch_receivers.argtypes = [C.c_void_p, C.c_uint64, C.c_uint64, C.c_void_p]
    lib.wv_step_count.argtypes = [C.c_void_p, C.POINTER(C.c_uint64)]
    lib.wv_kernel_time_ms.argtypes = [C.c_void_p, C.POINTER(C.c_double), C.POINTER(C.c_uint64)]
    lib.wv_enable_kernel_timing.argtypes = [C.c_void_p, C.c_int]
    lib.wv_kernel_time_detail.argtypes = [C.c_void_p, C.POINTER(C.c_double), C.POINTER(C.c_uint64), C.POINTER(C.c_uint64)]
    lib.wv_synchronize.argtypes = [C.c_void_p]
    lib.wv_set_stream_tuning.argtypes = [C.c_void_p, C.c_int, C.c_int, C.c_int, C.c_int, C.c_int]
    lib.wv_filter_test_2.argtypes = [C.c_void_p, C.c_void_p, C.c_void_p, C.c_void_p, C.c_uint32, C.c_uint32]
    lib.wv_field_pitch.argtypes = [C.c_void_p, C.POINTER(C.c_uint64)]
    lib.wv_classify_nodes.argtypes = [C.c_int32, C.c_int32, C.c_int32, C.c_void_p, C.c_void_p, C.POINTER(C.c_uint64)]
    lib.wv_comm_unique_id.argtypes = [C.c_void_p]
    lib.wv_comm_init.argtypes = [C.c_void_p, C.c_void_p, C.c_int, C.c_int]
    lib.wv_comm_destroy.argtypes = [C.c_void_p]
    lib.wv_comm_init_local.argtypes = [C.POINTER(C.c_void_p), C.c_int32]
    lib.wv_run_group.argtypes = [C.POINTER(C.c_void_p), C.c_int32, C.c_uint64, C.POINTER(C.c_uint64), C.POINTER(C.c_int32)]
    lib.wv_make_box_nodes.argtypes = [C.c_int32] * 7 + [C.c_void_p, C.POINTER(C.c_uint64)]
    _lib = lib
    return lib


def _check(rc):
    if rc != WV_OK:
        raise WaveguideError("wayverb_amd error %d: %s" % (rc, load_library().wv_last_error().decode()))


def raise_for_flag(flag):
    if flag & M.ERR_INF:
        raise ValueIsInf("Pressure value is inf, check filter coefficients.")
    if flag & M.ERR_NAN:
        raise ValueIsNan("Pressure value is nan, check filter coefficients.")
    if flag & M.ERR_OUTSIDE_MESH:
        raise WaveguideError("Tried to read non-existant node.")
    if flag & M.ERR_SUSPICIOUS_BOUNDARY:
        raise WaveguideError("Suspicious boundary read.")


def make_box_nodes(nx, ny, nz_global, z_begin=0, z_count=None, number_from=None, number_to=None):
    lib = load_library()
    if z_count is None:
        z_count = nz_global - z_begin
    if number_from is None:
        number_from = z_begin
    if number_to is None:
        number_to = z_begin + z_count
    nodes = np.empty(z_count * ny * nx, dtype=M.condensed_node_dtype)
    counts = (C.c_uint64 * 3)()
    _check(lib.wv_make_box_nodes(nx, ny, nz_global, z_begin, z_count, number_from, number_to,
                                 nodes.ctypes.data_as(C.c_void_p), counts))
    return nodes, tuple(int(c) for c in counts)


def classify_nodes(inside_mask):
    lib = load_library()
    mask = np.ascontiguousarray(inside_mask, dtype=np.uint8)
    nz, ny, nx = mask.shape
    nodes = np.zeros(nx * ny * nz, dtype=M.condensed_node_dtype)
    counts = (C.c_uint64 * 3)()
    _check(lib.wv_classify_nodes(nx, ny, nz, mask.ctypes.data_as(C.c_void_p), nodes.ctypes.data_as(C.c_void_p), counts))
    return nodes, tuple(int(c) for c in counts)


def voxelise(vertices, triangles, aabb, side=32):
    lib = load_library()
# ... 102 lines not shown
        opt.all_tiles = 1 if all_tiles else 0
        opt.transport = {"rccl": 0, "ipc": 1}[transport]
        opt.comm_timeout_s = int(comm_timeout_s)
        apply_tuning(opt, tuning)
        handle = C.c_void_p()
        _check(self.lib.wv_create(C.byref(wm), C.byref(opt), C.byref(handle)))
        self.h = handle
        self.n_recv = 0

    @classmethod
    def from_handle(cls, handle, mesh, precision):
        eng = cls.__new__(cls)
        eng.lib = load_library()
        eng.mesh = mesh
        eng.precision = precision
        eng.dtype = np.float32 if precision == "f32" else np.float64
        eng.h = handle
        eng.n_recv = 0
        return eng

    def close(self):
        if getattr(self, "h", None):
            self.lib.wv_destroy(self.h)
            self.h = None

    def __del__(self):
        try:
            self.close()
        except Exception:
            pass

    def read_value(self, index, buffer=BUF_CURRENT):
        v = C.c_double()
        _check(self.lib.wv_read_value(self.h, buffer, index, C.byref(v)))
        return v.value

    def write_value(self, index, value, buffer=BUF_CURRENT):
        _check(self.lib.wv_write_value(self.h, buffer, index, float(value)))

    def read_field(self, buffer=BUF_CURRENT, dtype=None):
        dtype = np.dtype(dtype or self.dtype)
        out = np.empty(self.mesh.num_nodes, dtype=dtype)
        _check(self.lib.wv_read_field(self.h, buffer, out.ctypes.data_as(C.c_void_p), dtype.itemsize))
        return out

    def write_field(self, values, buffer=BUF_CURRENT):
        values = np.ascontiguousarray(values)
        assert values.shape == (self.mesh.num_nodes,) and values.dtype in (np.float32, np.float64)
        _check(self.lib.wv_write_field(self.h, buffer, values.ctypes.data_as(C.c_void_p), values.dtype.itemsize))

    def read_planes(self, z_begin, z_count, buffer=BUF_CURRENT, dtype=None):
        dtype = np.dtype(dtype or self.dtype)
        nx, ny, _ = self.mesh.dims
        out = np.empty((z_count, ny, nx), dtype=dtype)
        _check(self.lib.wv_read_planes(self.h, buffer, z_begin, z_count, out.ctypes.data_as(C.c_void_p), dtype.itemsize))
        return out

    def write_planes(self, z_begin, values, buffer=BUF_CURRENT):
        values = np.ascontiguousarray(values)
        nx, ny, _ = self.mesh.dims
        assert values.shape[1:] == (ny, nx) and values.dtype in (np.float32, np.float64)
        _check(self.lib.wv_write_planes(self.h, buffer, z_begin, values.shape[0], values.ctypes.data_as(C.c_void_p),
                                        values.dtype.itemsize))

    def read_boundary_data(self, d):
        out = np.zeros((self.mesh.bidx[d - 1].shape[0], d), dtype=M.boundary_data_dtype)
        if out.size:
            _check(self.lib.wv_read_boundary_data(self.h, d, out.ctypes.data_as(C.c_void_p)))
        return out

    def write_boundary_data(self, d, data):
        data = np.ascontiguousarray(data, dtype=M.boundary_data_dtype)
        if data.size:
            _check(self.lib.wv_write_boundary_data(self.h, d, data.ctypes.data_as(C.c_void_p)))

    def set_coefficients(self, coeffs):
        coeffs = np.ascontiguousarray(coeffs, dtype=M.coefficients_dtype)
        _check(self.lib.wv_set_coefficients(self.h, coeffs.ctypes.data_as(C.c_void_p), coeffs.shape[0]))

    def device_buffer(self, buffer=BUF_CURRENT):
        p = C.c_void_p()
        _check(self.lib.wv_device_buffer(self.h, buffer, C.byref(p)))
        return p.value

    def checkpoint(self):
        _check(self.lib.wv_checkpoint(self.h))

    def rollback(self):
        _check(self.lib.wv_rollback(self.h))

    def drop_checkpoint(self):
        _check(self.lib.wv_drop_checkpoint(self.h))

    def step(self):
        flag = C.c_int32()
        _check(self.lib.wv_step(self.h, C.byref(flag)))
        return flag.value

    def swap(self):
        _check(self.lib.wv_swap(self.h))

    def set_source(self, kind, node=0, signal=None):
        if kind == SOURCE_NONE:
            _check(self.lib.wv_set_source(self.h, kind, 0, None, 0))
            return
        sig = np.ascontiguousarray(signal, dtype=np.float64)
        _check(self.lib.wv_set_source(self.h, kind, int(node), sig.ctypes.data_as(C.c_void_p), sig.shape[0]))

    def set_receivers(self, nodes):
        nodes = np.ascontiguousarray(nodes, dtype=np.uint64)
        self.n_recv = nodes.shape[0]
        _check(self.lib.wv_set_receivers(self.h, nodes.ctypes.data_as(C.c_void_p) if self.n_recv else None,
                                         self.n_recv))

    def run_steps(self, n_steps):
        done = C.c_uint64()
        flag = C.c_int32()
        _check(self.lib.wv_run(self.h, int(n_steps), C.byref(done), C.byref(flag)))
        return done.value, flag.value

    def fetch_receivers(self, first, n):
        out = np.zeros((n, self.n_recv), dtype=np.float64)
        if out.size:
            _check(self.lib.wv_fetch_receivers(self.h, first, n, out.ctypes.data_as(C.c_void_p)))
        return out

    def step_count(self):
        s = C.c_uint64()
        _check(self.lib.wv_step_count(self.h, C.byref(s)))
        return s.value

    def enable_kernel_timing(self, on=True):
        _check(self.lib.wv_enable_kernel_timing(self.h, int(on)))

    def kernel_time_ms(self):
        ms = C.c_double()
        n = C.c_uint64()
        _check(self.lib.wv_kernel_time_ms(self.h, C.byref(ms), C.byref(n)))
        return ms.value, n.value

    def kernel_time_detail(self):
        ms = C.c_double()
        n = C.c_uint64()
        steps = C.c_uint64()
        _check(self.lib.wv_kernel_time_detail(self.h, C.byref(ms), C.byref(n), C.byref(steps)))
        return ms.value, n.value, steps.value

    QUERY_PASSES, QUERY_XWALL_ENTRIES, QUERY_FIELDS, QUERY_MARCH_LIVE_PERMILLE, QUERY_SWEEP_LIVE_PERMILLE, QUERY_MARCH_ROUNDS = 0, 1, 2, 3, 4, 5
    QUERY_HALO_WAIT_NS, QUERY_HALO_WAITS, QUERY_HALO_EXCHANGES, QUERY_HALO_BYTES_SENT, QUERY_EARLY_PASSES = 6, 7, 8, 9, 10
    QUERY_BOUNDARY1_NS, QUERY_BOUNDARY2_NS, QUERY_BOUNDARY_TIMED = 11, 12, 13
    QUERY_WHOLE_STEPS = 14
    QUERY_TRIPLE_PASSES = 15
    QUERY_TRIPLE_MARCH_NS, QUERY_TRIPLE_MARCH_TIMED, QUERY_BOUNDARY3_NS, QUERY_FIXUP3_NS, QUERY_TRIPLE_PARTS_TIMED = 16, 17, 18, 19, 20

    def query(self, what):
        self.lib.wv_query.argtypes = [C.c_void_p, C.c_int, C.POINTER(C.c_uint64)]
        v = C.c_uint64()
        _check(self.lib.wv_query(self.h, what, C.byref(v)))
        return v.value

    def synchronize(self):
        _check(self.lib.wv_synchronize(self.h))

    def set_stream_tuning(self, variant=2, rows_per_wave=0, waves_x=0, waves_y=0, knob=0):
        _check(self.lib.wv_set_stream_tuning(self.h, variant, rows_per_wave, waves_x, waves_y, knob))

    @staticmethod
    def comm_unique_id():
        buf = (C.c_uint8 * UNIQUE_ID_BYTES)()
        _check(load_library().wv_comm_unique_id(buf))
        return bytes(buf)

    @staticmethod
    def comm_use_library(path):
        lib = load_library()
        lib.wv_comm_use_library.argtypes = [C.c_char_p]
        _check(lib.wv_comm_use_library(path.encode() if path else None))

    def comm_init(self, id_bytes, rank, nranks):
        buf = (C.c_uint8 * UNIQUE_ID_BYTES).from_buffer_copy(id_bytes)
        _check(self.lib.wv_comm_init(self.h, buf, rank, nranks))


class LocalSlabGroup:

    def __init__(self, engines):
        self.engines = list(engines)
        self.lib = load_library()
        self._handles = (C.c_void_p * len(self.engines))(*[e.h for e in self.engines])
        _check(self.lib.wv_comm_init_local(self._handles, len(self.engines)))

    def run_steps(self, n_steps):
        done = C.c_uint64()
        flag = C.c_int32()
        _check(self.lib.wv_run_group(self._handles, len(self.engines), int(n_steps), C.byref(done), C.byref(flag)))
        return done.value, flag.value

    def close(self):
        for e in self.engines:
            if e.h:
                self.lib.wv_comm_destroy(e.h)
        for e in self.engines:
            e.close()


def run(engine, pre, post, keep_going=lambda: True):
    step = 0
    while pre(engine, step) and keep_going():
        flag = engine.step()
        raise_for_flag(flag)
        post(engine, step)
        engine.swap()
        step += 1
    return step


def run_fast(engine, source_kind, source_node, signal, receivers, keep_going=lambda: True, chunk=1024):
    n = len(signal)
    engine.set_source(source_kind, source_node, signal)
    engine.set_receivers(receivers)
    first = engine.step_count()
    done_total = 0
    while done_total < n and keep_going():
        done, flag = engine.run_steps(min(chunk, n - done_total))
        done_total += done
        raise_for_flag(flag)
        if done == 0:
            break
    return done_total, engine.fetch_receivers(first, done_total)


def run_fast_slabs(mesh, slabs, source_kind, source_node, signal, receivers, precision="f64", devices=None,
                   keep_going=lambda: True, chunk=1024, tuning=None):
    from .slab import SlabLayout, place_source_and_receivers, slab_mesh
    devices = list(devices) if devices else [-1]
    engines, owners = [], []
    try:
        for r in range(slabs):
            L = SlabLayout(mesh.dims, r, slabs)
            eng = Engine(slab_mesh(mesh, L), precision=precision, device=devices[r % len(devices)],
                         ghost_lo=L.ghost_lo, ghost_hi=L.ghost_hi, tuning=tuning)
            engines.append(eng)
            src_local, mine = place_source_and_receivers(L, source_node, receivers)
            if src_local is not None:
                eng.set_source(source_kind, src_local, signal)
            eng.set_receivers([idx for _, idx in mine])
            owners.append([pos for pos, _ in mine])
        group = LocalSlabGroup(engines)
    except Exception:
        for e in engines:
            e.close()
        raise
    try:
        n = len(signal)
        done_total = 0
        while done_total < n and keep_going():
            done, flag = group.run_steps(min(chunk, n - done_total))
            done_total += done
            raise_for_flag(flag)
            if done == 0:
                break
        out = np.zeros((done_total, len(receivers)))
        for eng, cols in zip(engines, owners):
            if cols:
                out[:, cols] = eng.fetch_receivers(0, done_total)
        return done_total, out
    finally:
        group.close()


class _ResidentMesh:

    def __init__(self, dims, counts):
        self.dims = dims
        self.num_nodes = dims[0] * dims[1] * dims[2]
        self.bidx = [np.broadcast_to(np.uint32(0), (counts[d], d + 1)) for d in range(3)]
        self.nodes = None


class SceneMesh:

    def __init__(self, dims, min_corner, spacing, voxel_index, aabb, side, triangles, vertices, device=-1):
        self.lib = load_library()
        L = self.lib
        L.wv_scene_mesh_create.argtypes = [C.c_int32, C.c_int32, C.c_int32, C.c_void_p, C.c_float, C.c_void_p, C.c_uint64,
                                           C.c_void_p, C.c_void_p, C.c_uint32, C.c_void_p, C.c_uint32, C.c_void_p,
                                           C.c_uint32, C.c_int32, C.POINTER(C.c_void_p), C.POINTER(C.c_uint64)]
        L.wv_scene_mesh_fetch.argtypes = [C.c_void_p] * 5
        L.wv_scene_mesh_create_engine.argtypes = [C.c_void_p, C.c_void_p, C.c_uint32, C.POINTER(WvOptions),
                                                  C.POINTER(C.c_void_p)]
        L.wv_scene_mesh_destroy.argtypes = [C.c_void_p]
        L.wv_scene_mesh_destroy.restype = None
        self.dims = tuple(int(d) for d in dims)
        nx, ny, nz = self.dims
        v = np.ascontiguousarray(vertices, dtype=np.float32)
        t = np.ascontiguousarray(triangles, dtype=np.uint32)
        vox = np.ascontiguousarray(voxel_index, dtype=np.uint32)
        mc = np.ascontiguousarray(min_corner, dtype=np.float32)
        a0 = np.ascontiguousarray(aabb[0], dtype=np.float32)
        a1 = np.ascontiguousarray(aabb[1], dtype=np.float32)
        p = lambda a: a.ctypes.data_as(C.c_void_p)
        counts = (C.c_uint64 * 3)()
        h = C.c_void_p()
        _check(L.wv_scene_mesh_create(nx, ny, nz, p(mc), float(spacing), p(vox), vox.shape[0], p(a0), p(a1), int(side),
                                      p(t), t.shape[0], p(v), v.shape[0], int(device), C.byref(h), counts))
        self.h = h
# ... 37 lines not shown
```

Before: 442.0.

## Add sheet kernel fusing three timesteps for planar y/z boundary walls

```diff
diff --git a/include/wayverb_amd.h b/include/wayverb_amd.h
--- a/include/wayverb_amd.h
+++ b/include/wayverb_amd.h
@@ -92,6 +92,7 @@
     int32_t triple;
     int32_t triple_chunks;
     int32_t triple_lanes;
+    int32_t triple_sheets;
 } wv_tuning;
 
 typedef struct wv_options {
@@ -162,7 +163,7 @@
        WV_QUERY_WHOLE_STEPS = 14 ,
        WV_QUERY_TRIPLE_PASSES = 15,
        WV_QUERY_TRIPLE_MARCH_NS = 16, WV_QUERY_TRIPLE_MARCH_TIMED = 17, WV_QUERY_BOUNDARY3_NS = 18, WV_QUERY_FIXUP3_NS = 19,
-       WV_QUERY_TRIPLE_PARTS_TIMED = 20 };
+       WV_QUERY_TRIPLE_PARTS_TIMED = 20, WV_QUERY_SHEET_ENTRIES = 21 };
 int wv_query(wv_engine* e, int what, uint64_t* value);
 int wv_synchronize(wv_engine* e);
 int wv_set_stream_tuning(wv_engine* e, int variant, int rows_per_wave, int waves_x, int waves_y, int knob);
diff --git a/wayverb_amd/csrc/boundary_kernels.hip.h b/wayverb_amd/csrc/boundary_kernels.hip.h
--- a/wayverb_amd/csrc/boundary_kernels.hip.h
+++ b/wayverb_amd/csrc/boundary_kernels.hip.h
@@ -463,12 +463,13 @@
         } else if (a.order) {
             if (t - a.xw_pad < a.n_order) boundary_entry<Real, FIX>(a, coeffs, a.order[t - a.xw_pad], bad);
         } else {
-            boundary_entry<Real, FIX>(a, coeffs, a.xw_n + (t - a.xw_pad), bad);
+            const uint32_t e = a.xw_n + (t - a.xw_pad);
+            boundary_entry<Real, FIX>(a, coeffs, e >= a.sh_first ? e + a.sh_n : e, bad);
         }
     } else if (a.order) {
         if (t < a.n_order) boundary_entry<Real, FIX>(a, coeffs, a.order[t], bad);
     } else {
-        boundary_entry<Real, FIX>(a, coeffs, t, bad);
+        boundary_entry<Real, FIX>(a, coeffs, t >= a.sh_first ? t + a.sh_n : t, bad);
     }
     if (bad) atomicOr(a.flag, bad);
     if (next.fused && block == blocks - 1) pre_post_body<Real>(next, threadIdx.x, 256);
@@ -557,6 +558,270 @@
     a.xw_a[p] = a.prev[idx];
     a.xw_b[p] = a.cur[idx];
     a.xw_f[p] = a.cur[fn];
+}
+
+struct SheetTask {
+    uint32_t node0;
+    uint32_t table;
+    int32_t x0;
+    int32_t row0, row1;
+    int32_t trow0;
+    uint32_t dirs;
+};
+
+template <typename Real>
+struct SheetArgs {
+    const Real *prev, *cur;
+    Real *o1, *o2, *o3;
+    int *flag1, *flag2, *flag3;
+    const SheetTask* tasks;
+    uint32_t n_tasks;
+    const uint32_t* table;
+    uint32_t first, n;
+    const double* home;
+    const double* q_in;
+    double* q_out;
+    uint64_t q_in_stride, q_out_stride;
+    uint32_t q_in_sub, q_out_sub;
+    uint32_t n_slots;
+    const uint32_t* cidx;
+    const double* coeffs;
+    uint32_t n_coeffs;
+    int ny, pitch;
+    Real courant, courant_sq;
+};
+
+template <typename Real, uint32_t DIRS>
+__device__ __forceinline__ void sheet_body(const SheetArgs<Real>& a, const double* coeffs, const SheetTask& tk) {
+    const int lane = (int)(threadIdx.x & 63u);
+    constexpr bool fy = (DIRS & 12u) != 0;
+    constexpr bool positive = (DIRS & 40u) != 0;
+    const int64_t plane = (int64_t)a.pitch * a.ny;
+    const int64_t rstride = fy ? plane : (int64_t)a.pitch;
+    const int64_t F = (positive ? 1 : -1) * (fy ? (int64_t)a.pitch : plane);
+    const int x = tk.x0 + lane;
+    const int xl = min(max(x, 0), a.pitch - 1);
+    const bool lane_owns = lane >= 3 && lane <= 60 && x == xl;
+    const int row0 = tk.row0, row1 = tk.row1, first = row0 - 2, last = row1 + 1;
+    const uint32_t colb = (uint32_t)xl * (uint32_t)sizeof(Real);
+    auto lane_of = [&](auto* row) -> decltype(row) { return (decltype(row))((const char*)row + colb); };
+    auto at = [&](int r) -> int64_t { return (int64_t)tk.node0 + (int64_t)min(max(r, first - 1), last + 1) * rstride; };
+    auto pos_of = [&](int r) -> uint32_t {
+        const uint32_t p = (a.table + ((size_t)tk.table + (size_t)(min(max(r, first), last) - tk.trow0) * (size_t)a.pitch))[(uint32_t)xl];
+        return x == xl ? p : INVALID_NODE;
+    };
+    auto owned = [&](uint32_t pos, int r) -> bool { return lane_owns && r >= row0 && r < row1 && pos - a.first < a.n; };
+
+    struct RowIn {
+        Real w0p, pv, f0, f1, g1, g2;
+        double m[6];
+        uint32_t ci;
+    };
+    auto load_row = [&](int r, uint32_t pos) -> RowIn {
+        RowIn in;
+        const uint32_t p = pos == INVALID_NODE ? 0u : pos;
+        const bool q = p - a.first < a.n;
+        const double* src = q ? a.q_in + (p - a.q_in_sub) : a.home + p;
+        const size_t stride = q ? (size_t)a.q_in_stride : (size_t)a.n_slots;
+#pragma unroll
+        for (int j = 0; j < 6; ++j) in.m[j] = __builtin_nontemporal_load(src + (size_t)j * stride);
+        in.ci = a.cidx[p];
+        in.w0p = *lane_of(a.cur + at(r + 1));
+        in.pv = *lane_of(a.prev + at(r));
+        in.f0 = *lane_of(a.cur + (at(r) + F));
+        in.f1 = *lane_of(a.o1 + (at(r) + F));
+        in.g1 = *lane_of(a.o1 + (at(r - 1) + 2 * F));
+        in.g2 = *lane_of(a.o2 + (at(r - 2) + 2 * F));
+        return in;
+    };
+    auto wall = [&](Real xm, Real xp, Real rm, Real rp, Real faced, Real prev, double (&m)[1][6], const double* c) -> Real {
+        Real nb[3][2];
+        nb[0][0] = xm;
+        nb[0][1] = xp;
+        nb[1][0] = fy ? faced : rm;
+        nb[1][1] = fy ? faced : rp;
+        nb[2][0] = fy ? rm : faced;
+        nb[2][1] = fy ? rp : faced;
+        const bool off[3][2] = {{false, false}, {false, false}, {false, false}};
+        const double* cf[1] = {c};
+        return boundary_value<Real, 1>(a.courant, a.courant_sq, DIRS, nb, off, prev, m, cf);
+    };
+    auto inner = [&](Real xm, Real xp, Real rm, Real rp, Real w, Real g, Real fprev) -> Real {
+        Real fnb[3][2];
+        const Real lo = positive ? w : g, hi = positive ? g : w;
+        fnb[0][0] = xm;
+        fnb[0][1] = xp;
+        fnb[1][0] = fy ? lo : rm;
+        fnb[1][1] = fy ? hi : rp;
+        fnb[2][0] = fy ? rm : lo;
+        fnb[2][1] = fy ? rp : hi;
+        return faced_value<Real>(fnb, fprev);
+    };
+
+    Real w0m = *lane_of(a.cur + at(first - 1)), w0c = *lane_of(a.cur + at(first));
+    Real f0_1 = 0;
+    Real w1_1 = 0, w1_2 = 0, f1_1 = 0, f1_2 = 0;
+    Real w2_2 = 0, w2_3 = 0, f2_2 = 0, f2_3 = 0;
+    double mb[1][6] = {{0, 0, 0, 0, 0, 0}}, mc[1][6] = {{0, 0, 0, 0, 0, 0}};
+    uint32_t pos_c = pos_of(first), pos_n = pos_of(first + 1), pos_1 = INVALID_NODE, pos_2 = INVALID_NODE;
+    uint32_t ci_1 = 0, ci_2 = 0;
+    RowIn in = load_row(first, pos_c);
+    int bad1 = 0, bad2 = 0, bad3 = 0;
+    for (int i = first; i <= last; ++i) {
+        const uint32_t pos_nn = pos_of(i + 2);
+        const RowIn nxt = load_row(min(i + 1, last), pos_n);
+        double ma[1][6];
+#pragma unroll
+        for (int j = 0; j < 6; ++j) ma[0][j] = in.m[j];
+        const Real w0p = in.w0p, f1_0 = in.f1;
+        const Real w1_0 = wall(lane_from_below(w0c, w0c), lane_from_above(w0c, w0c), w0m, w0p, in.f0, in.pv, ma, coeffs + (size_t)in.ci * 14);
+        if (owned(pos_c, i)) {
+            bad1 |= bad_bits(w1_0);
+            *lane_of(a.o1 + at(i)) = w1_0;
+        }
+        const Real w2_1 = wall(lane_from_below(w1_1, w1_1), lane_from_above(w1_1, w1_1), w1_2, w1_0, f1_1, w0m, mb, coeffs + (size_t)ci_1 * 14);
+        const Real f2_1 = inner(lane_from_below(f1_1, f1_1), lane_from_above(f1_1, f1_1), f1_2, f1_0, w1_1, in.g1, f0_1);
+        if (owned(pos_1, i - 1)) {
+            bad2 |= bad_bits(w2_1) | bad_bits(f2_1);
+            *lane_of(a.o2 + at(i - 1)) = w2_1;
+            *lane_of(a.o2 + (at(i - 1) + F)) = f2_1;
+        }
+        const Real w3_2 = wall(lane_from_below(w2_2, w2_2), lane_from_above(w2_2, w2_2), w2_3, w2_1, f2_2, w1_2, mc, coeffs + (size_t)ci_2 * 14);
+        const Real f3_2 = inner(lane_from_below(f2_2, f2_2), lane_from_above(f2_2, f2_2), f2_3, f2_1, w2_2, in.g2, f1_2);
+        if (owned(pos_2, i - 2)) {
+            bad3 |= bad_bits(w3_2) | bad_bits(f3_2);
+            *lane_of(a.o3 + at(i - 2)) = w3_2;
+            *lane_of(a.o3 + (at(i - 2) + F)) = f3_2;
+            double* dst = a.q_out + (pos_2 - a.q_out_sub);
+#pragma unroll
+            for (int j = 0; j < 6; ++j) __builtin_nontemporal_store(mc[0][j], dst + (size_t)j * (size_t)a.q_out_stride);
+        }
+        w0m = w0c;
+        w0c = w0p;
+        f0_1 = in.f0;
+        w1_2 = w1_1;
+        w1_1 = w1_0;
+        f1_2 = f1_1;
+        f1_1 = f1_0;
+        w2_3 = w2_2;
+        w2_2 = w2_1;
+        f2_3 = f2_2;
+        f2_2 = f2_1;
+#pragma unroll
+        for (int j = 0; j < 6; ++j) {
+            mc[0][j] = mb[0][j];
+            mb[0][j] = ma[0][j];
+        }
+        pos_2 = pos_1;
+        pos_1 = pos_c;
+        pos_c = pos_n;
+        pos_n = pos_nn;
+        ci_2 = ci_1;
+        ci_1 = in.ci;
+        in = nxt;
+    }
+    if (bad1) atomicOr(a.flag1, bad1);
+    if (bad2) atomicOr(a.flag2, bad2);
+    if (bad3) atomicOr(a.flag3, bad3);
+}
+
+template <typename Real, bool LDSC>
+__global__ void __launch_bounds__(256) sheet_kernel(const SheetArgs<Real> a) {
+    __shared__ double s_coeffs[LDSC ? kMaxLdsCoefficientSets * 14 : 1];
+    if (LDSC) {
+        for (uint32_t w = threadIdx.x; w < a.n_coeffs * 14u; w += 256) s_coeffs[w] = a.coeffs[w];
+        __syncthreads();
+    }
+    const double* coeffs = LDSC ? s_coeffs : a.coeffs;
+    const uint32_t task = (uint32_t)__builtin_amdgcn_readfirstlane((int)(blockIdx.x * 4u + threadIdx.x / 64u));
+    if (task >= a.n_tasks) return;
+    const SheetTask tk = a.tasks[task];
+    if (tk.dirs == 4u)
+        sheet_body<Real, 4u>(a, coeffs, tk);
+    else if (tk.dirs == 8u)
+        sheet_body<Real, 8u>(a, coeffs, tk);
+    else if (tk.dirs == 16u)
+        sheet_body<Real, 16u>(a, coeffs, tk);
+    else
+        sheet_body<Real, 32u>(a, coeffs, tk);
+}
+
+struct SheetEligibleArgs {
+    const uint32_t* bnode;
+    const uint8_t* btype;
+    const uint8_t* cls;
+    uint8_t* eligible;
+    uint32_t n1;
+    int nx, ny, nz, pitch, cls_pitch;
+};
+
+__global__ void __launch_bounds__(256) sheet_eligible_kernel(const SheetEligibleArgs a) {
+    const uint32_t e = blockIdx.x * blockDim.x + threadIdx.x;
+    if (e >= a.n1) return;
+    const uint32_t idx = a.bnode[e];
+    const uint32_t dirs = a.btype[e] & 0x3Fu;
+    bool ok = idx != INVALID_NODE && (dirs == 4u || dirs == 8u || dirs == 16u || dirs == 32u);
+    if (ok) {
+        const int x = (int)(idx % (uint32_t)a.pitch);
+        const uint32_t q = idx / (uint32_t)a.pitch;
+        const int y = (int)(q % (uint32_t)a.ny), z = (int)(q / (uint32_t)a.ny);
+        const bool fy = (dirs & 12u) != 0;
+        const int step = (dirs & 40u) ? 1 : -1;
+        const int fdy = fy ? step : 0, fdz = fy ? 0 : step;
+        const int rdy = fy ? 0 : 1, rdz = fy ? 1 : 0;
+        auto cls_at = [&](int xx, int yy, int zz) -> uint32_t {
+            if (xx < 0 || xx >= a.nx || yy < 0 || yy >= a.ny || zz < 0 || zz >= a.nz) return 4u;
+            return (a.cls[cls_byte_index(xx, yy, zz, a.ny, a.cls_pitch)] >> ((xx & 3) * 2)) & 3u;
+        };
+        auto w1 = [&](int xx, int yy, int zz) -> bool {
+            return cls_at(xx, yy, zz) == CLS_BOUNDARY && cls_at(xx, yy + fdy, zz + fdz) == CLS_INSIDE && cls_at(xx - 1, yy, zz) != 4u &&
+                   cls_at(xx + 1, yy, zz) != 4u && cls_at(xx, yy - rdy, zz - rdz) != 4u && cls_at(xx, yy + rdy, zz + rdz) != 4u;
+        };
+        auto g = [&](int xx, int yy, int zz) -> bool {
+            const int gy = yy + 2 * fdy, gz = zz + 2 * fdz;
+            return cls_at(xx, gy, gz) == CLS_INSIDE && cls_at(xx - 1, gy, gz) == CLS_INSIDE && cls_at(xx + 1, gy, gz) == CLS_INSIDE &&
+                   cls_at(xx, gy - 1, gz) == CLS_INSIDE && cls_at(xx, gy + 1, gz) == CLS_INSIDE && cls_at(xx, gy, gz - 1) == CLS_INSIDE &&
+                   cls_at(xx, gy, gz + 1) == CLS_INSIDE;
+        };
+        for (int dr = -2; dr <= 2 && ok; ++dr)
+            for (int dx = -2; dx <= 2 && ok; ++dx) {
+                const int d = (dr < 0 ? -dr : dr) + (dx < 0 ? -dx : dx);
+                if (d > 2) continue;
+                ok = w1(x + dx, y + dr * rdy, z + dr * rdz);
+                if (ok && d <= 1) ok = g(x + dx, y + dr * rdy, z + dr * rdz);
+            }
+    }
+    a.eligible[e] = ok ? 1 : 0;
+}
+
+struct SheetCoverArgs {
+    const uint32_t* bnode;
+    const uint8_t* btype;
+    uint32_t first, n;
+    uint32_t* covered;
+    uint64_t source_node;
+    int* near_source;
+    int ny, pitch;
+};
+
+__global__ void __launch_bounds__(256) sheet_cover_kernel(const SheetCoverArgs a) {
+    const uint32_t t = blockIdx.x * blockDim.x + threadIdx.x;
+    if (t >= a.n) return;
+    const uint32_t idx = a.bnode[a.first + t];
+    const uint32_t dirs = a.btype[a.first + t] & 0x3Fu;
+    const int64_t plane = (int64_t)a.pitch * a.ny;
+    const int64_t F = ((dirs & 40u) ? 1 : -1) * ((dirs & 12u) ? (int64_t)a.pitch : plane);
+    const uint32_t fn = (uint32_t)((int64_t)idx + F);
+    atomicOr(a.covered + (fn >> 5), 1u << (fn & 31u));
+    if (a.source_node != ~0ull) {
+        const int x = (int)(idx % (uint32_t)a.pitch);
+        const uint32_t q = idx / (uint32_t)a.pitch;
+        const int y = (int)(q % (uint32_t)a.ny), z = (int)(q / (uint32_t)a.ny);
+        const int sx = (int)(a.source_node % (uint64_t)a.pitch);
+        const uint64_t sq = a.source_node / (uint64_t)a.pitch;
+        const int sy = (int)(sq % (uint64_t)a.ny), sz = (int)(sq / (uint64_t)a.ny);
+        if (abs(sx - x) <= 4 && abs(sy - y) <= 4 && abs(sz - z) <= 4) *a.near_source = 1;
+    }
 }
 
 template <typename Real>
diff --git a/wayverb_amd/csrc/device_common.hip.h b/wayverb_amd/csrc/device_common.hip.h
--- a/wayverb_amd/csrc/device_common.hip.h
+++ b/wayverb_amd/csrc/device_common.hip.h
@@ -107,6 +107,7 @@
     Real *xw_o2, *xw_f2;
     Real *xw_g2, *xw_h2;
     const uint8_t* xw_gok;
+    uint32_t sh_first, sh_n;
 };
 
 template <typename Real>
diff --git a/wayverb_amd/csrc/engine.hip b/wayverb_amd/csrc/engine.hip
--- a/wayverb_amd/csrc/engine.hip
+++ b/wayverb_amd/csrc/engine.hip
@@ -58,6 +58,7 @@
     t.triple = -1;
     t.triple_chunks = 0;
     t.triple_lanes = 0;
+    t.triple_sheets = -1;
 }
 
 #ifdef WV_DEBUG_ENV
@@ -72,7 +73,7 @@
                           {"WV_PAIR_UNIT_PLANES", &t.pair_unit_planes}, {"WV_PAIR_UNITS_BY_CHUNK", &t.pair_units_by_chunk}, {"WV_TILE_LISTS", &t.tile_lists},
                           {"WV_FUSE_PRE_POST", &t.fuse_pre_post}, {"WV_GRAPH", &t.graph}, {"WV_BOUNDARY_LDS", &t.boundary_lds},
                           {"WV_BOUNDARY_ORDER", &t.boundary_order}, {"WV_BOUNDARY_XWALL", &t.boundary_xwall},
-                          {"WV_SLAB_EARLY", &t.slab_early}, {"WV_PAIR_SPLIT_ROWS", &t.pair_split_rows}, {"WV_FUSE_PLANES", &t.fuse_planes}, {"WV_WHOLE_STEP", &t.whole_step}, {"WV_TRIPLE", &t.triple}, {"WV_TRIPLE_CHUNKS", &t.triple_chunks}, {"WV_TRIPLE_LANES", &t.triple_lanes},
+                          {"WV_SLAB_EARLY", &t.slab_early}, {"WV_PAIR_SPLIT_ROWS", &t.pair_split_rows}, {"WV_FUSE_PLANES", &t.fuse_planes}, {"WV_WHOLE_STEP", &t.whole_step}, {"WV_TRIPLE", &t.triple}, {"WV_TRIPLE_CHUNKS", &t.triple_chunks}, {"WV_TRIPLE_LANES", &t.triple_lanes}, {"WV_TRIPLE_SHEETS", &t.triple_sheets},
                           {"WV_STREAM_VARIANT", &o->stream_variant},
                           {"WV_STREAM_RY", &t.stream_ry}, {"WV_STREAM_NWX", &t.stream_nwx}, {"WV_STREAM_NWY", &t.stream_nwy},
                           {"WV_STREAM_ZCHUNKS", &t.stream_zchunks}};
diff --git a/wayverb_amd/csrc/engine.hip.h b/wayverb_amd/csrc/engine.hip.h
--- a/wayverb_amd/csrc/engine.hip.h
+++ b/wayverb_amd/csrc/engine.hip.h
@@ -74,6 +74,9 @@
     int enqueue_triple_slab(int slot, int part, uint64_t signal_pos, bool source_live);
     int launch_triple_march(int slot, const Real* A, const Real* B, Real* O1, Real* O2, Real* O3);
     int launch_triple_list(int slot, const Real* A, const Real* B, const Real* O1, const Real* O2, Real* O3, bool source_live);
+    int build_sheets(const std::vector<uint32_t>& bnode, const std::vector<uint8_t>& btype);
+    int launch_sheets(int slot, const Real* A, const Real* B, Real* O1, Real* O2, Real* O3);
+    int sheets_home();
     bool time_this_launch();
     int drain_timing();
     int step(int32_t* flag) override;
@@ -240,6 +243,17 @@
     uint32_t triple_unit_start_[9] = {0, 0, 0, 0, 0, 0, 0, 0, 0};
     uint32_t triple_units_longest_ = 0;
     double triple_live_frac_ = 1.0;
+    uint32_t n_sheet_ = 0;
+    uint32_t* sheet_table_ = nullptr;
+    wv::SheetTask* sheet_tasks_ = nullptr;
+    uint32_t sheet_n_tasks_ = 0;
+    uint32_t sheet_min_entries_ = 1u << 20;
+    int sheet_rows_ = 32;
+    double* fmem_alt_ = nullptr;
+    bool sheet_alt_live_ = false;
+    bool sheet_wanted_ = false;
+    bool sheet_active_ = false;
+    bool sheet_pass_ = false;
     bool triple_xw_ = false;
     uint64_t triple_min_nodes_ = sizeof(Real) == 8 ? (12ull << 20) : (24ull << 20);
     int triple_z0_ = 0, triple_z1_ = 0;
diff --git a/wayverb_amd/csrc/engine_batch.hip.h b/wayverb_amd/csrc/engine_batch.hip.h
--- a/wayverb_amd/csrc/engine_batch.hip.h
+++ b/wayverb_amd/csrc/engine_batch.hip.h
@@ -130,6 +130,7 @@
     (void)whole_step_ready();
     batch_source_live_ = source_kind_ != WV_SOURCE_NONE;
     pre_post_done_ = pair_mid_done_ = pair_list_done_ = false;
+    sheet_pass_ = false;
     batch_flags_reset_ = false;
     if (comm_ && batch) {
         static_assert(sizeof(int) == 4, "flag words are 32 bit");
@@ -155,6 +156,10 @@
 int Engine<Real>::collect_batch(uint64_t batch) {
     DeviceGuard guard(device_);
     std::string cerr;
+    {
+        const int rc = sheets_home();
+        if (rc) return rc;
+    }
     if (comm_ && !comm_->join_halo(stream_, &cerr)) return fail(WV_E_COMM, cerr);
     if (comm_ && !comm_->or_flags(stream_, flags_, (int)batch, &cerr)) return fail(WV_E_COMM, cerr);
     WV_HIP(hipMemcpyAsync(flags_host_, flags_, batch * sizeof(int), hipMemcpyDeviceToHost, stream_));
@@ -268,10 +273,12 @@
                     }
                     i += 3;
                 } else if (pair_at(i)) {
+                    if ((rc = sheets_home())) return rc;
                     if ((rc = enqueue_batch_pair(i, 0, 0))) return rc;
                     if ((rc = enqueue_batch_pair(i, 1, kind_at(i + 2)))) return rc;
                     i += 2;
                 } else {
+                    if ((rc = sheets_home())) return rc;
                     if ((rc = enqueue_batch_step(i, batch, kind_at(i + 1)))) return rc;
                     i += 1;
                 }
@@ -351,6 +358,7 @@
         case WV_QUERY_TRIPLE_PARTS_TIMED: *value = std::min(part_n_[2], part_n_[3]); return WV_OK;
         case WV_QUERY_TRIPLE_MARCH_NS: *value = (uint64_t)(part_ms_[4] * 1e6 + 0.5); return WV_OK;
         case WV_QUERY_TRIPLE_MARCH_TIMED: *value = part_n_[4]; return WV_OK;
+        case WV_QUERY_SHEET_ENTRIES: *value = (sheet_active_ && triple_ready_) ? n_sheet_ : 0; return WV_OK;
         default: return fail(WV_E_INVALID_ARGUMENT, "unknown query");
     }
 }
diff --git a/wayverb_amd/csrc/engine_setup.hip.h b/wayverb_amd/csrc/engine_setup.hip.h
--- a/wayverb_amd/csrc/engine_setup.hip.h
+++ b/wayverb_amd/csrc/engine_setup.hip.h
@@ -159,6 +159,45 @@
             for (uint32_t k = 0; k < n1_; ++k) n_xw_ += eligible[k];
             if (n_xw_ >= 0x7FFFFFFFu) n_xw_ = 0;
         }
+        std::vector<uint8_t> sheet(std::max<uint32_t>(n1_, 1), 0);
+        if (n1_ && opt_.tuning.triple_sheets != 0 && opt_.tuning.triple != 0 && !opt_.ghost_lo && !opt_.ghost_hi) {
+            ScopedDevice flags_mem;
+            WV_HIP(hipMalloc(&flags_mem.p, n1_));
+            wv::SheetEligibleArgs x{};
+            x.bnode = bnode_;
+            x.btype = btype_;
+            x.cls = cls_;
+            x.eligible = static_cast<uint8_t*>(flags_mem.p);
+            x.n1 = n1_;
+            x.nx = nx_;
+            x.ny = ny_;
+            x.nz = nz_;
+            x.pitch = pitch_;
+            x.cls_pitch = cls_pitch_;
+            hipLaunchKernelGGL(wv::sheet_eligible_kernel, dim3((n1_ + 255) / 256), dim3(256), 0, stream_, x);
+            WV_HIP(hipGetLastError());
+            WV_HIP(hipMemcpyAsync(sheet.data(), flags_mem.p, n1_, hipMemcpyDeviceToHost, stream_));
+            WV_HIP(hipStreamSynchronize(stream_));
+            std::vector<int> lo(4 * (size_t)std::max(ny_, nz_), INT32_MAX), hi(4 * (size_t)std::max(ny_, nz_), -1);
+            for (uint32_t k = 0; k < n1_; ++k) {
+                if (!sheet[k]) continue;
+                const uint32_t idx = bnode[k], q = idx / (uint32_t)pitch_;
+                const int y = (int)(q % (uint32_t)ny_), z = (int)(q / (uint32_t)ny_);
+                const uint32_t dirs = btype[k] & 0x3Fu;
+                const bool fy = (dirs & 12u) != 0;
+                const size_t s = (size_t)(dirs == 4u ? 0 : dirs == 8u ? 1 : dirs == 16u ? 2 : 3) * (size_t)std::max(ny_, nz_) + (size_t)(fy ? y : z);
+                lo[s] = std::min(lo[s], fy ? z : y);
+                hi[s] = std::max(hi[s], fy ? z : y);
+                ++n_sheet_;
+            }
+            uint64_t words = 0;
+            for (size_t s = 0; s < lo.size(); ++s)
+                if (hi[s] >= 0) words += (uint64_t)(hi[s] - lo[s] + 5) * (uint64_t)pitch_;
+            if (words > (64ull << 20)) {
+                n_sheet_ = 0;
+                std::fill(sheet.begin(), sheet.end(), (uint8_t)0);
+            }
+        }
         const uint64_t bricks_x = ((uint64_t)pitch_ + 63) / 64, bricks_y = ((uint64_t)ny_ + 7) / 8;
         std::vector<std::pair<uint64_t, uint32_t>> keyed(n_entries_);
         std::vector<uint32_t> by_pos(n_entries_);
@@ -173,7 +212,15 @@
                     const uint64_t brick = ((z >> 3) * bricks_y + (y >> 3)) * bricks_x + (x >> 6);
                     kk = (brick << 12) | ((z & 7) << 9) | ((y & 7) << 6) | (x & 63);
                 }
-                if (!(d == 0 && n_xw_ && eligible[k])) kk |= 1ull << 57;
+                if (d == 0 && n_sheet_ && sheet[k]) {
+                    const uint64_t x = idx % (uint32_t)pitch_, q = idx / (uint32_t)pitch_;
+                    const uint64_t y = q % (uint32_t)ny_, z = q / (uint32_t)ny_;
+                    const uint64_t dirs = btype[off + k] & 0x3Fu;
+                    const bool fy = (dirs & 12u) != 0;
+                    kk = 1ull << 57 | dirs << 48 | (fy ? y : z) << 32 | (fy ? z : y) << 16 | x;
+                } else if (!(d == 0 && n_xw_ && eligible[k])) {
+                    kk |= 1ull << 58;
+                }
                 keyed[off + k] = {kk, off + k};
             }
             std::sort(keyed.begin() + off, keyed.begin() + off + nd[d]);
@@ -189,6 +236,10 @@
         }
         WV_HIP(hipMemcpy(bnode_, bnode2.data(), (size_t)n_entries_ * sizeof(uint32_t), hipMemcpyHostToDevice));
         WV_HIP(hipMemcpy(btype_, btype2.data(), (size_t)n_entries_, hipMemcpyHostToDevice));
+        if (n_sheet_) {
+            const int rc = build_sheets(bnode2, btype2);
+            if (rc) return rc;
+        }
     }
     WV_HIP(hipMemcpy(ref_to_pos_, ref_to_pos.data(), ne * sizeof(uint32_t), hipMemcpyHostToDevice));
 
@@ -228,6 +279,115 @@
     const int n_ev = 2 * kRing;
     events_.resize(n_ev);
     for (auto& e : events_) WV_HIP(hipEventCreate(&e));
+    return WV_OK;
+}
+
+template <typename Real>
+int Engine<Real>::build_sheets(const std::vector<uint32_t>& bnode, const std::vector<uint8_t>& btype) {
+    struct Sheet {
+        uint32_t dirs = 0;
+        int c = 0, r0 = INT32_MAX, r1 = -1, x0 = INT32_MAX, x1 = -1;
+        uint64_t table = 0;
+        uint32_t first_task = 0;
+        int windows = 0, chunks = 0;
+    };
+    const size_t span = (size_t)std::max(ny_, nz_);
+    std::vector<int> sheet_of(4 * span, -1);
+    std::vector<Sheet> sheets;
+    auto coords = [&](uint32_t pos, int* c, int* r, int* x) -> size_t {
+        const uint32_t idx = bnode[pos], q = idx / (uint32_t)pitch_, dirs = btype[pos] & 0x3Fu;
+        const int y = (int)(q % (uint32_t)ny_), z = (int)(q / (uint32_t)ny_);
+        const bool fy = (dirs & 12u) != 0;
+        *c = fy ? y : z;
+        *r = fy ? z : y;
+        *x = (int)(idx % (uint32_t)pitch_);
+        return (size_t)(dirs == 4u ? 0 : dirs == 8u ? 1 : dirs == 16u ? 2 : 3) * span + (size_t)*c;
+    };
+    for (uint32_t pos = n_xw_; pos < n_xw_ + n_sheet_; ++pos) {
+        int c, r, x;
+        const size_t s = coords(pos, &c, &r, &x);
+        if (sheet_of[s] < 0) {
+            sheet_of[s] = (int)sheets.size();
+            sheets.emplace_back();
+            sheets.back().dirs = btype[pos] & 0x3Fu;
+            sheets.back().c = c;
+        }
+        Sheet& sh = sheets[(size_t)sheet_of[s]];
+        sh.r0 = std::min(sh.r0, r);
+        sh.r1 = std::max(sh.r1, r);
+        sh.x0 = std::min(sh.x0, x);
+        sh.x1 = std::max(sh.x1, x);
+    }
+    {
+        int cus = 256;
+        if (hipDeviceGetAttribute(&cus, hipDeviceAttributeMultiprocessorCount, device_) != hipSuccess || cus <= 0) {
+            (void)hipGetLastError();
+            cus = 256;
+        }
+        const uint64_t slots = 8ull * (uint64_t)cus;
+        uint64_t best = ~0ull;
+        for (int r = 12; r <= 96; ++r) {
+            uint64_t tasks = 0;
+            for (const Sheet& sh : sheets) tasks += (uint64_t)((sh.x1 - sh.x0) / 58 + 1) * (uint64_t)((sh.r1 - sh.r0) / r + 1);
+            const uint64_t cost = ((tasks + slots - 1) / slots) * (uint64_t)(r + 4);
+            if (cost < best) {
+                best = cost;
+                sheet_rows_ = r;
+            }
+        }
+    }
+    uint64_t words = 0, n_cells = 0;
+    for (Sheet& sh : sheets) {
+        sh.table = words;
+        words += (uint64_t)(sh.r1 - sh.r0 + 5) * (uint64_t)pitch_;
+        sh.windows = (sh.x1 - sh.x0) / 58 + 1;
+        sh.chunks = (sh.r1 - sh.r0) / sheet_rows_ + 1;
+        sh.first_task = (uint32_t)n_cells;
+        n_cells += (uint64_t)sh.windows * (uint64_t)sh.chunks;
+    }
+    if (words >= (1ull << 32) || n_cells >= (1ull << 31)) {
+        n_sheet_ = 0;
+        return WV_OK;
+    }
+    std::vector<uint32_t> table((size_t)words, wv::INVALID_NODE);
+    for (uint32_t pos = 0; pos < n1_; ++pos) {
+        const uint32_t dirs = btype[pos] & 0x3Fu;
+        if (bnode[pos] == wv::INVALID_NODE || !(dirs == 4u || dirs == 8u || dirs == 16u || dirs == 32u)) continue;
+        int c, r, x;
+        const size_t s = coords(pos, &c, &r, &x);
+        if (sheet_of[s] < 0) continue;
+        const Sheet& sh = sheets[(size_t)sheet_of[s]];
+        if (r < sh.r0 - 2 || r > sh.r1 + 2) continue;
+        table[(size_t)sh.table + (size_t)(r - (sh.r0 - 2)) * (size_t)pitch_ + (size_t)x] = pos;
+    }
+    std::vector<uint8_t> live((size_t)n_cells, 0);
+    for (uint32_t pos = n_xw_; pos < n_xw_ + n_sheet_; ++pos) {
+        int c, r, x;
+        const Sheet& sh = sheets[(size_t)sheet_of[coords(pos, &c, &r, &x)]];
+        live[(size_t)sh.first_task + (size_t)((r - sh.r0) / sheet_rows_) * (size_t)sh.windows + (size_t)((x - sh.x0) / 58)] = 1;
+    }
+    std::vector<wv::SheetTask> tasks;
+    const uint64_t plane = (uint64_t)pitch_ * (uint64_t)ny_;
+    for (const Sheet& sh : sheets)
+        for (int ch = 0; ch < sh.chunks; ++ch)
+            for (int w = 0; w < sh.windows; ++w) {
+                if (!live[(size_t)sh.first_task + (size_t)ch * (size_t)sh.windows + (size_t)w]) continue;
+                wv::SheetTask t{};
+                const bool fy = (sh.dirs & 12u) != 0;
+                t.node0 = (uint32_t)(fy ? (uint64_t)sh.c * (uint64_t)pitch_ : (uint64_t)sh.c * plane);
+                t.table = (uint32_t)sh.table;
+                t.x0 = sh.x0 + 58 * w - 3;
+                t.row0 = sh.r0 + ch * sheet_rows_;
+                t.row1 = std::min(t.row0 + sheet_rows_, sh.r1 + 1);
+                t.trow0 = sh.r0 - 2;
+                t.dirs = sh.dirs;
+                tasks.push_back(t);
+            }
+    sheet_n_tasks_ = (uint32_t)tasks.size();
+    WV_HIP(hipMalloc((void**)&sheet_table_, table.size() * sizeof(uint32_t)));
+    WV_HIP(hipMemcpy(sheet_table_, table.data(), table.size() * sizeof(uint32_t), hipMemcpyHostToDevice));
+    WV_HIP(hipMalloc((void**)&sheet_tasks_, tasks.size() * sizeof(wv::SheetTask)));
+    WV_HIP(hipMemcpy(sheet_tasks_, tasks.data(), tasks.size() * sizeof(wv::SheetTask), hipMemcpyHostToDevice));
     return WV_OK;
 }
 
@@ -501,7 +661,7 @@
     for (auto& f : ckpt_.field)
         if (f) (void)hipFree(f);
     if (ckpt_.fmem) (void)hipFree(ckpt_.fmem);
-    void* ptrs[] = {field1_, triple_map_, triple_list_, triple_units_, suspect_, pair_units_, pair_map_, pair_list_, pair_counter_, signal_base_dev_, tile_list_, xw_nbr_, xw_val_, xw_gok_, ref_to_pos_, cls_,   bnode_,      btype_,    fmem_,  cidx_,
+    void* ptrs[] = {sheet_table_, sheet_tasks_, fmem_alt_, field1_, triple_map_, triple_list_, triple_units_, suspect_, pair_units_, pair_map_, pair_list_, pair_counter_, signal_base_dev_, tile_list_, xw_nbr_, xw_val_, xw_gok_, ref_to_pos_, cls_,   bnode_,      btype_,    fmem_,  cidx_,
                     status_,          coeffs_,    flags_,      scratch_, signal_, recv_nodes_, recv_out_, zorder_};
     for (void* p : ptrs)
         if (p) (void)hipFree(p);
diff --git a/wayverb_amd/csrc/engine_single.hip.h b/wayverb_amd/csrc/engine_single.hip.h
--- a/wayverb_amd/csrc/engine_single.hip.h
+++ b/wayverb_amd/csrc/engine_single.hip.h
@@ -164,6 +164,11 @@
         n = b.n_order;
         if (!n && !xw) return WV_OK;
     }
+    if (sheet_pass_ && !b.order) {
+        b.sh_first = n_xw_;
+        b.sh_n = n_sheet_;
+        n -= n_sheet_;
+    }
     if (xw) {
         xwall_args(b);
         n += b.xw_pad;
diff --git a/wayverb_amd/csrc/engine_triple.hip.h b/wayverb_amd/csrc/engine_triple.hip.h
--- a/wayverb_amd/csrc/engine_triple.hip.h
+++ b/wayverb_amd/csrc/engine_triple.hip.h
@@ -56,7 +56,8 @@
         WV_HIP(hipMemsetAsync(suspect_, 0, kRing * sizeof(int), stream_));
     }
     const bool xw = xw_active_ && pair_inner_ok_ > 0 && opt_.tuning.boundary_xwall != 2 && !(comm_ && opt_.tuning.slab_early == 0);
-    if (triple_map_ && triple_source_ == src && triple_io_generation_ == io_generation_ && triple_xw_ == xw) {
+    bool sheets = n_sheet_ && sheet_tasks_ && (opt_.tuning.triple_sheets > 0 || (opt_.tuning.triple_sheets < 0 && n_sheet_ >= sheet_min_entries_)) && !comm_ && !opt_.ghost_lo && !opt_.ghost_hi && pair_inner_ok_ > 0 && !pair_units_;
+    if (triple_map_ && triple_source_ == src && triple_io_generation_ == io_generation_ && triple_xw_ == xw && sheet_wanted_ == sheets) {
         triple_ready_ = !(pair_units_ && !triple_units_);
         return WV_OK;
     }
@@ -80,10 +81,48 @@
     m.z_begin = triple_z0_;
     m.z_end = triple_z1_;
     ScopedDevice covered;
-    if (xw) {
+    sheet_wanted_ = sheets;
+    if (xw || sheets) {
         const size_t words = (size_t)((stored_nodes_ + 31) / 32) + 1;
         WV_HIP(hipMalloc(&covered.p, words * sizeof(uint32_t)));
         WV_HIP(hipMemsetAsync(covered.p, 0, words * sizeof(uint32_t), stream_));
+        m.covered = static_cast<uint32_t*>(covered.p);
+    }
+    if (sheets) {
+        ScopedDevice near;
+        WV_HIP(hipMalloc(&near.p, sizeof(int)));
+        WV_HIP(hipMemsetAsync(near.p, 0, sizeof(int), stream_));
+        wv::SheetCoverArgs c{};
+        c.bnode = bnode_;
+        c.btype = btype_;
+        c.first = n_xw_;
+        c.n = n_sheet_;
+        c.covered = static_cast<uint32_t*>(covered.p);
+        c.source_node = src;
+        c.near_source = static_cast<int*>(near.p);
+        c.ny = ny_;
+        c.pitch = pitch_;
+        hipLaunchKernelGGL(wv::sheet_cover_kernel, dim3((n_sheet_ + 255) / 256), dim3(256), 0, stream_, c);
+        WV_HIP(hipGetLastError());
+        int hit = 0;
+        WV_HIP(hipMemcpyAsync(&hit, near.p, sizeof(int), hipMemcpyDeviceToHost, stream_));
+        WV_HIP(hipStreamSynchronize(stream_));
+        if (hit) {
+            const size_t words = (size_t)((stored_nodes_ + 31) / 32) + 1;
+            WV_HIP(hipMemsetAsync(covered.p, 0, words * sizeof(uint32_t), stream_));
+            if (!xw) m.covered = nullptr;
+            sheets = false;
+        }
+        if (sheets && !fmem_alt_ && hipMalloc((void**)&fmem_alt_, (size_t)n_sheet_ * 6 * sizeof(double)) != hipSuccess) {
+            (void)hipGetLastError();
+            fmem_alt_ = nullptr;
+            WV_HIP(hipMemsetAsync(covered.p, 0, ((size_t)((stored_nodes_ + 31) / 32) + 1) * sizeof(uint32_t), stream_));
+            if (!xw) m.covered = nullptr;
+            sheets = false;
+        }
+    }
+    sheet_active_ = sheets;
+    if (xw) {
         wv::XwCoverArgs c{};
         c.bnode = bnode_;
         c.btype = btype_;
@@ -98,7 +137,6 @@
         c.cls_pitch = cls_pitch_;
         hipLaunchKernelGGL(wv::xwall_cover_kernel, dim3((n_xw_ + 255) / 256), dim3(256), 0, stream_, c);
         WV_HIP(hipGetLastError());
-        m.covered = c.covered;
     }
     triple_xw_ = xw;
     hipLaunchKernelGGL(wv::triple_map_kernel, dim3(blocks), dim3(256), 0, stream_, m);
@@ -424,6 +462,56 @@
 }
 
 template <typename Real>
+int Engine<Real>::launch_sheets(int slot, const Real* A, const Real* B, Real* O1, Real* O2, Real* O3) {
+    wv::SheetArgs<Real> a{};
+    a.prev = A;
+    a.cur = B;
+    a.o1 = O1;
+    a.o2 = O2;
+    a.o3 = O3;
+    a.flag1 = flags_ + slot;
+    a.flag2 = flags_ + slot + 1;
+    a.flag3 = flags_ + slot + 2;
+    a.tasks = sheet_tasks_;
+    a.n_tasks = sheet_n_tasks_;
+    a.table = sheet_table_;
+    a.first = n_xw_;
+    a.n = n_sheet_;
+    a.home = fmem_;
+    const bool to_alt = !sheet_alt_live_;
+    a.q_in = to_alt ? fmem_ : fmem_alt_;
+    a.q_in_stride = to_alt ? n_slots_ : n_sheet_;
+    a.q_in_sub = to_alt ? 0u : n_xw_;
+    a.q_out = to_alt ? fmem_alt_ : fmem_;
+    a.q_out_stride = to_alt ? n_sheet_ : n_slots_;
+    a.q_out_sub = to_alt ? n_xw_ : 0u;
+    a.n_slots = n_slots_;
+    a.cidx = cidx_;
+    a.coeffs = coeffs_;
+    a.n_coeffs = n_coeffs_;
+    a.ny = ny_;
+    a.pitch = pitch_;
+    a.courant = courant_;
+    a.courant_sq = courant_sq_;
+    const dim3 grid((sheet_n_tasks_ + 3) / 4), block(256);
+    if (n_coeffs_ <= wv::kMaxLdsCoefficientSets && opt_.tuning.boundary_lds != 0)
+        hipLaunchKernelGGL((wv::sheet_kernel<Real, true>), grid, block, 0, stream_, a);
+    else
+        hipLaunchKernelGGL((wv::sheet_kernel<Real, false>), grid, block, 0, stream_, a);
+    sheet_alt_live_ = to_alt;
+    return WV_OK;
+}
+
+template <typename Real>
+int Engine<Real>::sheets_home() {
+    if (!sheet_alt_live_) return WV_OK;
+    WV_HIP(hipMemcpy2DAsync(fmem_ + n_xw_, (size_t)n_slots_ * sizeof(double), fmem_alt_, (size_t)n_sheet_ * sizeof(double), (size_t)n_sheet_ * sizeof(double), 6,
+                            hipMemcpyDeviceToDevice, stream_));
+    sheet_alt_live_ = false;
+    return WV_OK;
+}
+
+template <typename Real>
 int Engine<Real>::enqueue_triple(int slot, uint64_t signal_pos, bool source_live, int fuse_next) {
     DeviceGuard guard(device_);
     Real* A = field_[prv_];
@@ -453,6 +541,12 @@
     }
     xw_valid_ = xw;
     int token = begin_part_timing(0);
+    sheet_pass_ = sheet_active_;
+    if (sheet_pass_) {
+        if ((rc = launch_sheets(slot, A, B, O1, O2, O3))) return rc;
+    } else if ((rc = sheets_home())) {
+        return rc;
+    }
     if (fuse && io) {
         wv::PrePostArgs<Real> nx = pre_post_args(O1, slot + 1, true, signal_pos + 1, source_live);
         nx.flag = nullptr;
@@ -507,6 +601,7 @@
     }
     if ((rc = end_part_timing(2, token))) return rc;
     pass_timed_ = false;
+    sheet_pass_ = false;
     WV_HIP(hipGetLastError());
     ++triples_taken_;
     const int a_idx = prv_, b_idx = cur_;
diff --git a/wayverb_amd/engine.py b/wayverb_amd/engine.py
--- a/wayverb_amd/engine.py
+++ b/wayverb_amd/engine.py
@@ -44,7 +44,7 @@
 TUNING_FIELDS = ("pair", "pair_chunks", "pair_inner_fix", "pair_wide", "pair_unit_waves", "pair_unit_planes", "pair_units_by_chunk", "tile_lists",
                  "fuse_pre_post", "graph", "boundary_lds", "boundary_order", "boundary_xwall",
                  "stream_ry", "stream_nwx", "stream_nwy", "stream_zchunks", "slab_early", "pair_split_rows", "fuse_planes", "whole_step", "triple",
-                 "triple_chunks", "triple_lanes")
+                 "triple_chunks", "triple_lanes", "triple_sheets")
 
 
 class WvTuning(C.Structure):
@@ -453,6 +453,7 @@
     QUERY_WHOLE_STEPS = 14
     QUERY_TRIPLE_PASSES = 15
     QUERY_TRIPLE_MARCH_NS, QUERY_TRIPLE_MARCH_TIMED, QUERY_BOUNDARY3_NS, QUERY_FIXUP3_NS, QUERY_TRIPLE_PARTS_TIMED = 16, 17, 18, 19, 20
+    QUERY_SHEET_ENTRIES = 21
 
     def query(self, what):
         self.lib.wv_query.argtypes = [C.c_void_p, C.c_int, C.POINTER(C.c_uint64)]
```

Result: faster. 451.9, median of 6 (+2.2%).
